# whcorkran/mamba-TTS-project

Measured on AMD Instinct MI355X. Metric: audio tokens/sec (teacher-forced fwd+bwd) per GPU; decode_step p50 latency, higher is better.
Workload: dtype bf16; 1 GPU; C2: MambaTTSDecoder 12L d_model=1024 fwd+bwd+clip+Adam, B=8/GPU T_audio=2048 T_text=128; model=MambaTTSDecoder-12L-d1024, global_batch=8, seq_len=2048, parallelism=dp1

## Files before the change

### include/mtts.h

```cpp
#ifndef MTTS_H
#define MTTS_H

#include <stdint.h>

#ifdef __cplusplus
extern "C" {
#endif

#define MTTS_ABI_VERSION 15

enum { MTTS_F32 = 0, MTTS_BF16 = 1 };
enum {
  MTTS_OK = 0,
  MTTS_EINVAL = -22,
  MTTS_EUNSUPPORTED = -95,
  MTTS_ELAUNCH = -5
};

int mtts_abi_version(void);
const char* mtts_last_error(void);

enum {
  MTTS_OVR_AUTO = -1,
  MTTS_OVR_SCAN_PATH = 0,
// ... 14 lines not shown

typedef struct {
  int batch, dim, seqlen, dstate;
  int dtype_io, dtype_bc;
  int delta_softplus;
  int ckpt_chunk;
  int a_is_log;
  int reserved_;
  int64_t u_bs, u_ls;
  int64_t delta_bs, delta_ls;
  int64_t z_bs, z_ls;
  int64_t out_bs, out_ls;
  int64_t B_bs, B_ls;
  int64_t C_bs, C_ls;
  const void* u;
  const void* delta;
  const float* A;
  const void* Bm;
  const void* Cm;
  const float* D;
  const void* z;
  const float* delta_bias;
  const float* h0;
  void* out;
  float* last_state;
  float* ckpt;
  void* workspace;
  const int* seqlens;
} MttsScanFwdArgs;

int64_t mtts_selective_scan_fwd_workspace(int batch, int dim, int seqlen, int dstate);
int mtts_selective_scan_fwd(const MttsScanFwdArgs* a, void* stream);

typedef struct {
  MttsScanFwdArgs f;
  const void* dout;
  int64_t dout_bs, dout_ls;
  void* du;      int64_t du_bs, du_ls;
  void* ddelta;  int64_t ddelta_bs, ddelta_ls;
  void* dz;      int64_t dz_bs, dz_ls;
  float* dB;     int64_t dB_bs, dB_ls;
  float* dC;     int64_t dC_bs, dC_ls;
  float* dA;
  float* dD;
  float* ddelta_bias;
  float* dh0;
  void* workspace;
} MttsScanBwdArgs;

int64_t mtts_selective_scan_bwd_workspace(int batch, int dim, int seqlen, int dstate);
int mtts_selective_scan_bwd(const MttsScanBwdArgs* a, void* stream);

typedef struct {
  int batch, dim, seqlen, width;
  int dtype;
  int silu;
  int64_t x_bs, x_ls, out_bs, out_ls;
  const void* x;
  const float* w;
  const float* bias;
  const float* conv_state_in;
  void* out;
  float* conv_state_out;
  const int* seqlens;
} MttsConvFwdArgs;

int mtts_causal_conv1d_fwd(const MttsConvFwdArgs* a, void* stream);

typedef struct {
  MttsConvFwdArgs f;
  const void* dout; int64_t dout_bs, dout_ls;
  void* dx;         int64_t dx_bs, dx_ls;
  float* dw;
  float* dbias;
  void* workspace;
} MttsConvBwdArgs;

int64_t mtts_causal_conv1d_bwd_workspace(int batch, int dim, int seqlen, int width);
int mtts_causal_conv1d_bwd(const MttsConvBwdArgs* a, void* stream);

typedef struct {
  int batch, dim, width, dtype, silu;
  int64_t x_bs, out_bs;
  const void* x;
  float* conv_state;
  const float* w;
  const float* bias;
  void* out;
} MttsConvUpdateArgs;

int mtts_causal_conv1d_update(const MttsConvUpdateArgs* a, void* stream);

typedef struct {
  int batch, dim, dstate, dtype_io, dtype_bc, dt_softplus;
  int64_t x_bs, dt_bs, z_bs, out_bs, B_bs, C_bs;
  float* state;
  const void* x;
  const void* dt;
  const float* A;
  const void* Bm;
  const void* Cm;
  const float* D;
  const void* z;
  const float* dt_bias;
  void* out;
  int dt_rank;
  const void* dt_w;
  void* out_packed;
} MttsStateUpdateArgs;

int mtts_selective_state_update(const MttsStateUpdateArgs* a, void* stream);


typedef struct {
  int rows, cols, dtype, rows_per_group;
  float eps;
  int64_t x_rs, res_rs, xsum_rs, y_rs, gb_rs;
  const void* x;
  const void* res;
  void* x_sum;
  const float* w;
  const float* b;
  const void* gamma;
  const void* beta;
  int gb_dtype;
  void* y;
  float* mean;
  float* rstd;
} MttsLNArgs;

int mtts_layernorm_fwd(const MttsLNArgs* a, void* stream);

int mtts_layernorm_rows_packed(const MttsLNArgs* a, void* y_packed, void* stream);

typedef struct {
  MttsLNArgs f;
  const void* dy;   int64_t dy_rs;
  const void* dx_acc; int64_t dxacc_rs;
  void* dx;         int64_t dx_rs;
  float* dw;
  float* db;
  float* dgamma;
  float* dbeta;
  void* workspace;
  float* dx_colsum;
  int64_t dgb_rs;
} MttsLNBwdArgs;

int64_t mtts_layernorm_bwd_workspace(int rows, int cols, int rows_per_group);
int mtts_layernorm_bwd(const MttsLNBwdArgs* a, void* stream);

int64_t mtts_colsum_workspace(int rows, int cols, int rows_per_group);
int mtts_colsum(const void* in, int dtype, int rows, int cols, int64_t row_stride, int rows_per_group, float* out,
                int64_t out_gstride, void* workspace, void* stream);

typedef struct {
  int batch, heads, head_dim, q_len, kv_len;
  int dtype;
  float scale;
  int64_t q_bs, q_ls, k_bs, k_ls, v_bs, v_ls, o_bs, o_ls;
  int64_t mask_bs;
  const void* q;
  const void* k;
  const void* v;
  const uint8_t* key_padding_mask;
  void* out;
  float* lse;
  void* out_packed;
  int64_t kv_hs;
} MttsAttnFwdArgs;

int mtts_attention_fwd(const MttsAttnFwdArgs* a, void* stream);

typedef struct {
  MttsAttnFwdArgs f;
  const void* x;
  int64_t x_rs;
  const void* wq;
  const void* bq;
  const float* ln_w;
  const float* ln_b;
  float eps;
  int d_model;
} MttsAttnQProjArgs;
int mtts_attention_decode_qproj(const MttsAttnQProjArgs* a, void* stream);

typedef struct {
  MttsAttnFwdArgs f;
  const void* dout; int64_t do_bs, do_ls;
  void* dq;         int64_t dq_bs, dq_ls;
  void* dk;         int64_t dk_bs, dk_ls;
  void* dv;         int64_t dv_bs, dv_ls;
  void* workspace;
} MttsAttnBwdArgs;

int64_t mtts_attention_bwd_workspace(int batch, int heads, int head_dim, int q_len, int kv_len, int dtype);
int mtts_attention_bwd(const MttsAttnBwdArgs* a, void* stream);

int mtts_length_regulate_lengths(const float* durations, int64_t dur_bs, int batch, int T, int64_t* lengths,
                                 void* stream);
int mtts_length_regulate_fwd(const void* hidden, int dtype, int batch, int T, int D, int64_t h_bs, int64_t h_ls,
                             const float* durations, int64_t dur_bs, int max_len, void* out, int64_t o_bs,
                             int64_t o_ls, void* stream);
int mtts_length_regulate_bwd(const void* dout, int dtype, int batch, int T, int D, int64_t do_bs, int64_t do_ls,
                             const float* durations, int64_t dur_bs, int max_len, void* dhidden, int64_t dh_bs,
                             int64_t dh_ls, void* stream);

// ... 58 lines not shown
  int kgroups;
  float* splitk_slab;
  int* splitk_count;
  int w_packed;
  int x_packed;
  void* y_packed;
  void* u_packed;
} MttsRowsArgs;

int mtts_gemm_rows(const MttsRowsArgs* a, void* stream);

typedef struct {
  int64_t rows;
  int vocab;
  int dtype;
  int64_t ld;
  const void* logits;
  const int64_t* targets;
  int ignore_index;
  float* loss;
  float* lse;
  float* workspace;
} MttsCrossEntropyArgs;

int64_t mtts_cross_entropy_workspace(int64_t rows);
int mtts_cross_entropy_fwd(const MttsCrossEntropyArgs* a, void* stream);
int mtts_cross_entropy_bwd(const MttsCrossEntropyArgs* a, const float* grad_loss, void* dlogits, int64_t ld_dlogits,
                           void* stream);

int64_t mtts_pack_rows_bytes(int N, int K);
int mtts_pack_rows_weight(const void* W, int64_t ldw, int N, int K, void* out, void* stream);


#define MTTS_GEMM_NT 0
#define MTTS_GEMM_TN 1
#define MTTS_GEMM_EPI_BIAS 1
#define MTTS_GEMM_EPI_GELU 2
#define MTTS_GEMM_EPI_DGELU 4
typedef struct {
  int m, n, k;
  int layout;
  int splits;
  int epilogue;
  int out_dtype;
  int bias_dtype;
  int64_t lda, ldb, ldc, ld_aux;
  const void* a;
  const void* b;
  void* c;
  const void* bias;
  void* aux;
  void* workspace;
  float beta;
} MttsGemmArgs;

int64_t mtts_gemm_workspace(const MttsGemmArgs* a);
int mtts_gemm(const MttsGemmArgs* a, void* stream);

int mtts_gemm_grouped(const MttsGemmArgs* probs, int n, void* stream);

int mtts_gemm_grouped_rounds(const MttsGemmArgs* probs, int n, void* stream);

#define MTTS_CONVGEMM_NN 2
#define MTTS_CONVGEMM_BIAS 1
#define MTTS_CONVGEMM_RELU 2
#define MTTS_CONVGEMM_DRELU 4
typedef struct {
  const void* ptr;
  int64_t seg_rows, seg_stride, row_stride;
  int32_t halo_c, halo_p;
} MttsRowMap;
typedef struct {
  int layout;
  int m, n, k;
  MttsRowMap a, b, c, aux;
  const float* bias;
  int epilogue;
  float beta;
  int splits;
  void* workspace;
  float* colsum_a;
} MttsConvGemmArgs;
int64_t mtts_convgemm_workspace(const MttsConvGemmArgs* a);
int mtts_convgemm(const MttsConvGemmArgs* a, void* stream);

#define MTTS_SKINNY_N 0
#define MTTS_SKINNY_SMALL_K 1
#define MTTS_SKINNY_TN 2
typedef struct {
  int mode;
  int m, n, k;
  int c_dtype;
  float beta;
  int64_t lda, ldb, ldc;
  const void* a;
  const void* b;
  void* c;
  void* workspace;
  int trans_c;
  int reserved_;
} MttsSkinnyArgs;

int64_t mtts_gemm_skinny_workspace(const MttsSkinnyArgs* a);
int mtts_gemm_skinny(const MttsSkinnyArgs* a, void* stream);

typedef struct {
// ... 52 lines not shown
```

### mamba-tts-project_amd/mtts/_lib.py

```python
from __future__ import annotations

import contextlib
import ctypes as C
import os

import torch

_HERE = os.path.dirname(os.path.abspath(__file__))
LIB_PATH = os.environ.get("MTTS_LIB", os.path.join(_HERE, "libmtts.so"))
ABI_VERSION = 15

F32, BF16 = 0, 1
i32, i64, f32, vp = C.c_int, C.c_int64, C.c_float, C.c_void_p


class ScanFwdArgs(C.Structure):
    _fields_ = [("batch", i32), ("dim", i32), ("seqlen", i32), ("dstate", i32),
                ("dtype_io", i32), ("dtype_bc", i32), ("delta_softplus", i32), ("ckpt_chunk", i32),
                ("a_is_log", i32), ("reserved_", i32), ("u_bs", i64), ("u_ls", i64), ("delta_bs", i64), ("delta_ls", i64),
                ("z_bs", i64), ("z_ls", i64), ("out_bs", i64), ("out_ls", i64),
                ("B_bs", i64), ("B_ls", i64), ("C_bs", i64), ("C_ls", i64),
                ("u", vp), ("delta", vp), ("A", vp), ("Bm", vp), ("Cm", vp), ("D", vp), ("z", vp),
                ("delta_bias", vp), ("h0", vp), ("out", vp), ("last_state", vp), ("ckpt", vp),
                ("workspace", vp), ("seqlens", vp)]


class ScanBwdArgs(C.Structure):
    _fields_ = [("f", ScanFwdArgs), ("dout", vp), ("dout_bs", i64), ("dout_ls", i64),
                ("du", vp), ("du_bs", i64), ("du_ls", i64),
                ("ddelta", vp), ("ddelta_bs", i64), ("ddelta_ls", i64),
                ("dz", vp), ("dz_bs", i64), ("dz_ls", i64),
                ("dB", vp), ("dB_bs", i64), ("dB_ls", i64),
                ("dC", vp), ("dC_bs", i64), ("dC_ls", i64),
                ("dA", vp), ("dD", vp), ("ddelta_bias", vp), ("dh0", vp), ("workspace", vp)]


class ConvFwdArgs(C.Structure):
    _fields_ = [("batch", i32), ("dim", i32), ("seqlen", i32), ("width", i32), ("dtype", i32), ("silu", i32),
                ("x_bs", i64), ("x_ls", i64), ("out_bs", i64), ("out_ls", i64),
                ("x", vp), ("w", vp), ("bias", vp), ("conv_state_in", vp), ("out", vp), ("conv_state_out", vp),
                ("seqlens", vp)]


class ConvBwdArgs(C.Structure):
    _fields_ = [("f", ConvFwdArgs), ("dout", vp), ("dout_bs", i64), ("dout_ls", i64),
                ("dx", vp), ("dx_bs", i64), ("dx_ls", i64), ("dw", vp), ("dbias", vp), ("workspace", vp)]


class ConvUpdateArgs(C.Structure):
    _fields_ = [("batch", i32), ("dim", i32), ("width", i32), ("dtype", i32), ("silu", i32),
                ("x_bs", i64), ("out_bs", i64), ("x", vp), ("conv_state", vp), ("w", vp), ("bias", vp),
                ("out", vp)]


class StateUpdateArgs(C.Structure):
    _fields_ = [("batch", i32), ("dim", i32), ("dstate", i32), ("dtype_io", i32), ("dtype_bc", i32),
                ("dt_softplus", i32),
                ("x_bs", i64), ("dt_bs", i64), ("z_bs", i64), ("out_bs", i64), ("B_bs", i64), ("C_bs", i64),
                ("state", vp), ("x", vp), ("dt", vp), ("A", vp), ("Bm", vp), ("Cm", vp), ("D", vp), ("z", vp),
                ("dt_bias", vp), ("out", vp), ("dt_rank", i32), ("dt_w", vp), ("out_packed", vp)]


class RowsArgs(C.Structure):
    _fields_ = [("M", i32), ("N", i32), ("K", i32), ("act", i32), ("ldx", i64), ("ldw", i64), ("ldy", i64),
                ("x", vp), ("W", vp), ("bias", vp), ("y", vp),
                ("conv_dim", i32), ("conv_state", vp), ("conv_w", vp), ("conv_b", vp), ("u", vp), ("ldu", i64),
                ("ln_w", vp), ("ln_b", vp), ("ln_eps", f32), ("gamma", vp), ("beta", vp), ("ld_gb", i64),
                ("res", vp), ("ld_res", i64), ("kgroups", i32), ("splitk_slab", vp), ("splitk_count", vp),
                ("w_packed", i32), ("x_packed", i32), ("y_packed", vp), ("u_packed", vp)]


class CrossEntropyArgs(C.Structure):
    _fields_ = [("rows", i64), ("vocab", i32), ("dtype", i32), ("ld", i64), ("logits", vp), ("targets", vp),
                ("ignore_index", i32), ("loss", vp), ("lse", vp), ("workspace", vp)]


class GemmArgs(C.Structure):
    _fields_ = [("m", i32), ("n", i32), ("k", i32), ("layout", i32), ("splits", i32), ("epilogue", i32),
                ("out_dtype", i32), ("bias_dtype", i32), ("lda", i64), ("ldb", i64), ("ldc", i64), ("ld_aux", i64),
                ("a", vp), ("b", vp), ("c", vp), ("bias", vp), ("aux", vp), ("workspace", vp), ("beta", f32)]


class DropoutArgs(C.Structure):
    _fields_ = [("n", i64), ("dtype", i32), ("p", f32), ("seed", C.c_uint64), ("x", vp), ("y", vp), ("pre", vp),
                ("group", i32), ("x_rep", i32), ("x_inner", i32), ("reserved_", i32), ("seed_in", vp),
                ("seed_out", vp)]


class SampleArgs(C.Structure):
    _fields_ = [("rows", i32), ("vocab", i32), ("dtype", i32), ("top_k", i32), ("ld", i64), ("logits", vp),
                ("bias", vp), ("bias_ld", i64), ("temperature", f32), ("top_p", f32), ("seed", vp), ("step", vp),
                ("advance", i32), ("step0", i32), ("pos", vp), ("tokens", vp), ("tok_stride", i64),
                ("history", vp), ("hist_ld", i64), ("hist_cols", i32), ("eos_id", i32), ("pad_id", i32),
                ("pos_rows", i32), ("finished", vp), ("length", vp), ("unfinished", vp)]


class RowMap(C.Structure):
    _fields_ = [("ptr", vp), ("seg_rows", i64), ("seg_stride", i64), ("row_stride", i64), ("halo_c", i32),
                ("halo_p", i32)]


class ConvGemmArgs(C.Structure):
    _fields_ = [("layout", i32), ("m", i32), ("n", i32), ("k", i32), ("a", RowMap), ("b", RowMap), ("c", RowMap),
                ("aux", RowMap), ("bias", vp), ("epilogue", i32), ("beta", f32), ("splits", i32),
                ("workspace", vp), ("colsum_a", vp)]


class SkinnyArgs(C.Structure):
    _fields_ = [("mode", i32), ("m", i32), ("n", i32), ("k", i32), ("c_dtype", i32), ("beta", f32),
                ("lda", i64), ("ldb", i64), ("ldc", i64), ("a", vp), ("b", vp), ("c", vp), ("workspace", vp),
                ("trans_c", i32), ("reserved_", i32)]


class LNArgs(C.Structure):
    _fields_ = [("rows", i32), ("cols", i32), ("dtype", i32), ("rows_per_group", i32), ("eps", f32),
                ("x_rs", i64), ("res_rs", i64), ("xsum_rs", i64), ("y_rs", i64), ("gb_rs", i64),
                ("x", vp), ("res", vp), ("x_sum", vp), ("w", vp), ("b", vp), ("gamma", vp), ("beta", vp),
                ("gb_dtype", i32), ("y", vp), ("mean", vp), ("rstd", vp)]


class LNBwdArgs(C.Structure):
    _fields_ = [("f", LNArgs), ("dy", vp), ("dy_rs", i64), ("dx_acc", vp), ("dxacc_rs", i64),
                ("dx", vp), ("dx_rs", i64), ("dw", vp), ("db", vp), ("dgamma", vp), ("dbeta", vp),
                ("workspace", vp), ("dx_colsum", vp), ("dgb_rs", i64)]


class AttnFwdArgs(C.Structure):
    _fields_ = [("batch", i32), ("heads", i32), ("head_dim", i32), ("q_len", i32), ("kv_len", i32),
                ("dtype", i32), ("scale", f32),
                ("q_bs", i64), ("q_ls", i64), ("k_bs", i64), ("k_ls", i64), ("v_bs", i64), ("v_ls", i64),
                ("o_bs", i64), ("o_ls", i64), ("mask_bs", i64),
                ("q", vp), ("k", vp), ("v", vp), ("key_padding_mask", vp), ("out", vp), ("lse", vp),
                ("out_packed", vp), ("kv_hs", i64)]


class AttnQProjArgs(C.Structure):
    _fields_ = [("f", AttnFwdArgs), ("x", vp), ("x_rs", i64), ("wq", vp), ("bq", vp), ("ln_w", vp), ("ln_b", vp),
                ("eps", f32), ("d_model", i32)]


class AttnBwdArgs(C.Structure):
    _fields_ = [("f", AttnFwdArgs), ("dout", vp), ("do_bs", i64), ("do_ls", i64),
                ("dq", vp), ("dq_bs", i64), ("dq_ls", i64), ("dk", vp), ("dk_bs", i64), ("dk_ls", i64),
                ("dv", vp), ("dv_bs", i64), ("dv_ls", i64), ("workspace", vp)]


class CastDesc(C.Structure):
    _fields_ = [("src", vp), ("dst", vp), ("dstT", vp), ("rows", i32), ("cols", i32), ("tile0", i64)]


class AdamTensor(C.Structure):
    _fields_ = [("p", vp), ("g", vp), ("m", vp), ("v", vp), ("n", i64), ("chunk0", i64)]


_SIGS = {
    "mtts_abi_version": ([], i32),
    "mtts_last_error": ([], C.c_char_p),
    "mtts_set_override": ([i32, i32], i32),
    "mtts_get_override": ([i32], i32),
    "mtts_selective_scan_fwd_workspace": ([i32, i32, i32, i32], i64),
    "mtts_selective_scan_fwd": ([C.POINTER(ScanFwdArgs), vp], i32),
    "mtts_selective_scan_bwd_workspace": ([i32, i32, i32, i32], i64),
    "mtts_selective_scan_bwd": ([C.POINTER(ScanBwdArgs), vp], i32),
    "mtts_causal_conv1d_fwd": ([C.POINTER(ConvFwdArgs), vp], i32),
    "mtts_causal_conv1d_bwd_workspace": ([i32, i32, i32, i32], i64),
    "mtts_causal_conv1d_bwd": ([C.POINTER(ConvBwdArgs), vp], i32),
    "mtts_causal_conv1d_update": ([C.POINTER(ConvUpdateArgs), vp], i32),
    "mtts_selective_state_update": ([C.POINTER(StateUpdateArgs), vp], i32),
    "mtts_layernorm_fwd": ([C.POINTER(LNArgs), vp], i32),
    "mtts_gemm_rows": ([C.POINTER(RowsArgs), vp], i32),
    "mtts_pack_rows_bytes": ([i32, i32], i64),
    "mtts_cross_entropy_workspace": ([i64], i64),
    "mtts_cross_entropy_fwd": ([C.POINTER(CrossEntropyArgs), vp], i32),
    "mtts_cross_entropy_bwd": ([C.POINTER(CrossEntropyArgs), vp, vp, i64, vp], i32),
    "mtts_layernorm_rows_packed": ([C.POINTER(LNArgs), vp, vp], i32),
    "mtts_pack_rows_weight": ([vp, i64, i32, i32, vp, vp], i32),
    "mtts_gemm_workspace": ([C.POINTER(GemmArgs)], i64),
    "mtts_gemm": ([C.POINTER(GemmArgs), vp], i32),
    "mtts_gemm_grouped": ([C.POINTER(GemmArgs), i32, vp], i32),
    "mtts_gemm_grouped_rounds": ([C.POINTER(GemmArgs), i32, vp], i32),
    "mtts_convgemm": ([C.POINTER(ConvGemmArgs), vp], i32),
    "mtts_convgemm_workspace": ([C.POINTER(ConvGemmArgs)], i64),
    "mtts_gemm_skinny": ([C.POINTER(SkinnyArgs), vp], i32),
    "mtts_gemm_skinny_workspace": ([C.POINTER(SkinnyArgs)], i64),
    "mtts_layernorm_bwd_workspace": ([i32, i32, i32], i64),
    "mtts_layernorm_bwd": ([C.POINTER(LNBwdArgs), vp], i32),
    "mtts_colsum_workspace": ([i32, i32, i32], i64),
    "mtts_colsum": ([vp, i32, i32, i32, i64, i32, vp, i64, vp, vp], i32),
    "mtts_attention_fwd": ([C.POINTER(AttnFwdArgs), vp], i32),
    "mtts_attention_decode_qproj": ([C.POINTER(AttnQProjArgs), vp], i32),
    "mtts_attention_bwd_workspace": ([i32, i32, i32, i32, i32, i32], i64),
    "mtts_attention_bwd": ([C.POINTER(AttnBwdArgs), vp], i32),
    "mtts_adam_chunks": ([i64], i64),
    "mtts_adam_workspace": ([i64], i64),
    "mtts_clip_adam": ([vp, i32, i64, vp, f32, f32, f32, f32, f32, f32, vp, vp, vp], i32),
    "mtts_embed_sum": ([vp, i64, vp, vp, vp, vp, vp, i32, i32, i32, i32, vp, i32, i64, vp, vp], i32),
    "mtts_embed_sum_at": ([vp, i64, vp, vp, vp, vp, vp, i32, i32, i32, i32, vp, i32, i64, vp, i64, i32, vp], i32),
    "mtts_embed_table_grad_workspace": ([i64, i32, i32], i64),
    "mtts_embed_table_grad": ([vp, i64, vp, i32, i64, i32, i32, vp, vp, vp], i32),
    "mtts_cast_tiles": ([i32, i32], i64),
    "mtts_cast_bf16_multi": ([vp, i32, i64, vp], i32),
    "mtts_length_regulate_lengths": ([vp, i64, i32, i32, vp, vp], i32),
    "mtts_length_regulate_fwd": ([vp, i32, i32, i32, i32, i64, i64, vp, i64, i32, vp, i64, i64, vp], i32),
    "mtts_length_regulate_bwd": ([vp, i32, i32, i32, i32, i64, i64, vp, i64, i32, vp, i64, i64, vp], i32),
    "mtts_dropout": ([C.POINTER(DropoutArgs), vp], i32),
    "mtts_sample_tokens": ([C.POINTER(SampleArgs), vp], i32),
}

_lib = None


def lib():
    global _lib
    if _lib is None:
        if not os.path.exists(LIB_PATH):
            raise RuntimeError(f"libmtts.so not found at {LIB_PATH}; run __graft_entry__.build() "
                               "(make -C mamba-tts-project_amd/mtts/csrc)")
        L = C.CDLL(LIB_PATH)
        for sym, what in (("mtts_embed_sum_at", "ragged prompts"),
                          ("mtts_gemm_grouped_rounds", "round-filling weight gradients")):
            if not hasattr(L, sym):
                raise RuntimeError(f"{LIB_PATH} is stale: it was built before {sym} ({what}) was "
                                   "added; rebuild it with __graft_entry__.build() "
                                   "(make -C mamba-tts-project_amd/mtts/csrc)")
        for name, (argt, rest) in _SIGS.items():
            fn = getattr(L, name)
            fn.argtypes = argt
            fn.restype = rest
        v = L.mtts_abi_version()
        if v != ABI_VERSION:
            raise RuntimeError(f"libmtts ABI {v} != expected {ABI_VERSION}")
        _lib = L
    return _lib


def exported_symbols():
    return list(_SIGS)


def call(name, args):
    L = lib()
    stream = torch.cuda.current_stream().cuda_stream
    rc = getattr(L, name)(C.byref(args), C.c_void_p(stream))
    if rc != 0:
        raise RuntimeError(f"{name} failed ({rc}): {L.mtts_last_error().decode()}")


def call_raw(name, *args):
    L = lib()
    rc = getattr(L, name)(*args, C.c_void_p(torch.cuda.current_stream().cuda_stream))
    if rc != 0:
        raise RuntimeError(f"{name} failed ({rc}): {L.mtts_last_error().decode()}")


OVERRIDES = {"scan_path": 0, "scan_p": 1, "scan_segs": 2, "scan_bwd_segs": 3, "gemm_narrow": 4,
             "attn_chunks": 5, "attn_bwd": 6, "attn_generic": 7, "conv_untiled": 8, "gemm_tile": 9,
             "attn_dq_dma": 10}
SCAN_C1, SCAN_W2, SCAN_NARROW = 1, 2, 3
ATTN_BWD_FUSED, ATTN_BWD_SPLIT = 1, 2


@contextlib.contextmanager
def override(**paths):
    L = lib()
    old = {}
    try:
        for k, v in paths.items():
            old[k] = L.mtts_set_override(OVERRIDES[k], -1 if v is None else int(v))
        yield
    finally:
        for k, v in old.items():
            L.mtts_set_override(OVERRIDES[k], v)

# ... 12 lines not shown
```

### mamba-tts-project_amd/mtts/attention.py

```python
from __future__ import annotations

import math

import torch
import torch.nn as nn
import torch.nn.functional as F

from . import attn_kernels
from . import wgrad as WG
from .linear import _want_t, cast_scope, cast_weight, cast_weight_t, colsum, linear, proj, wgrad


class InProjFn(torch.autograd.Function):

    @staticmethod
    def forward(ctx, query, key, weight, bias):
        cd = query.dtype
        d = query.shape[-1]
        Wc, bc = cast_weight(weight, cd), cast_weight(bias, cd)
        x2, k2 = query.reshape(-1, d), key.reshape(-1, d)
        q = proj(x2, Wc[:d], bc[:d])
        kv = proj(k2, Wc[d:], bc[d:])
        ctx.save_for_backward(x2, k2, Wc)
        ctx.weight = weight
        ctx.meta = (query.shape, key.shape, weight.dtype, bias.dtype)
        return q.view(*query.shape[:-1], d), kv.view(*key.shape[:-1], 2 * d)

    @staticmethod
    def backward(ctx, dq, dkv):
        x2, k2, Wc = ctx.saved_tensors
        qshape, kshape, wdt, bdt = ctx.meta
        d = x2.shape[1]
        dq2 = dq.reshape(-1, d).to(Wc.dtype)
        dkv2 = dkv.reshape(-1, 2 * d).to(Wc.dtype)
        if Wc.dtype == torch.bfloat16 and _want_t(ctx.weight):
            Wt = cast_weight_t(ctx.weight, Wc.dtype)
            dquery = proj(dq2, Wt[:, :d]).view(qshape) if ctx.needs_input_grad[0] else None
            dkey = proj(dkv2, Wt[:, d:]).view(kshape) if ctx.needs_input_grad[1] else None
        else:
            dquery = (dq2 @ Wc[:d]).view(qshape) if ctx.needs_input_grad[0] else None
            dkey = (dkv2 @ Wc[d:]).view(kshape) if ctx.needs_input_grad[1] else None
        dW = db = None
        if ctx.needs_input_grad[2] and not WG.submit([(dq2, x2, ctx.weight, (0, d)),
                                                      (dkv2, k2, ctx.weight, (d, 3 * d))]):
            dW = torch.empty(3 * d, d, device=x2.device, dtype=torch.float32)
            wgrad(dq2, x2, out=dW[:d])
            wgrad(dkv2, k2, out=dW[d:])
            dW = dW.to(wdt)
        if ctx.needs_input_grad[3]:
            db = torch.empty(3 * d, device=x2.device, dtype=torch.float32)
            colsum(dq2, out=db[:d])
            colsum(dkv2, out=db[d:])
            db = db.to(bdt)
        return dquery, dkey, dW, db


class DkvSink:

    def __init__(self, rows, n_layers, width, shape, device, dtype):
        self.rows, self.L, self.width, self.shape = rows, n_layers, width, shape
        self.device, self.dtype = device, dtype
        self.buf = None
        self.key2 = None
        self.written = [False] * n_layers
        self.taken = [False] * n_layers

    def view(self, layer):
        if self.buf is None:
            self.buf = torch.empty(self.rows, self.L * self.width, device=self.device, dtype=self.dtype)
        self.written[layer] = True
        return self.buf[:, layer * self.width:(layer + 1) * self.width].view(*self.shape, self.width)

    def partner(self, layer):
        sink = self

        class _P:
            @staticmethod
            def take():
                if not sink.written[layer] or sink.buf is None or sink.key2 is None:
                    return None
                sink.taken[layer] = True
                d = sink.width // 2
                return (sink.buf[:, layer * sink.width:(layer + 1) * sink.width], sink.key2, (d, 3 * d))
        return _P()


class KVAllFn(torch.autograd.Function):

    @staticmethod
    def forward(ctx, key, sink, *params):
        cd = key.dtype
        d = key.shape[-1]
        Ws, bs = params[0::2], params[1::2]
        k2 = key.reshape(-1, d)
        Wst = torch.cat([cast_weight(W, cd)[d:] for W in Ws])
        bst = torch.cat([cast_weight(b, cd)[d:] for b in bs])
        kv = proj(k2, Wst, bst)
        ctx.save_for_backward(k2)
        ctx.Ws, ctx.bs, ctx.kshape, ctx.sink = Ws, bs, key.shape, sink
        sink.key2 = k2
        return tuple(kv[:, l * 2 * d:(l + 1) * 2 * d].view(*key.shape[:-1], 2 * d) for l in range(len(Ws)))

    @staticmethod
    def backward(ctx, *dkvs):
        (k2,) = ctx.saved_tensors
        Ws, bs, sink = ctx.Ws, ctx.bs, ctx.sink
        nl, d = len(Ws), k2.shape[1]
        w2 = 2 * d
        cd = k2.dtype
        in_sink = sink.buf is not None and all(
            g is not None and g.data_ptr() == sink.buf.data_ptr() + l * w2 * sink.buf.element_size()
            and g.stride()[-2] == nl * w2 for l, g in enumerate(dkvs))
        if in_sink:
            dkv = sink.buf
        else:
            dkv = torch.zeros(k2.shape[0], nl * w2, device=k2.device, dtype=cd)
            for l, g in enumerate(dkvs):
                if g is not None:
                    dkv[:, l * w2:(l + 1) * w2] = g.reshape(-1, w2)
        sink.buf = None
        dkey = None
        if ctx.needs_input_grad[0]:
            if cd == torch.bfloat16:
                WstT = torch.cat([cast_weight_t(W, cd)[:, d:] for W in Ws], dim=1)
                dkey = proj(dkv, WstT).view(ctx.kshape)
            else:
                dkey = (dkv @ torch.cat([cast_weight(W, cd)[d:] for W in Ws])).view(ctx.kshape)
        grads = [dkey, None]
        for l in range(nl):
            W, b = Ws[l], bs[l]
            dW = db = None
            if not sink.taken[l]:
                dy = dkv[:, l * w2:(l + 1) * w2]
                if ctx.needs_input_grad[2 + 2 * l] and not WG.submit([(dy, k2, W, (d, 3 * d))]):
                    dW = torch.zeros(W.shape, device=W.device, dtype=W.dtype)
                    dW[d:] = wgrad(dy.contiguous(), k2).to(W.dtype)
                if ctx.needs_input_grad[3 + 2 * l]:
                    db = torch.zeros(b.shape, device=b.device, dtype=b.dtype)
                    db[d:] = colsum(dy).to(b.dtype)
            grads += [dW, db]
        sink.written = [False] * nl
        sink.taken = [False] * nl
        return tuple(grads)


def kv_all(key: torch.Tensor, attns) -> list:
    params = []
    for a in attns:
        params += [a.in_proj_weight, a.in_proj_bias]
    d = attns[0].embed_dim
    sink = DkvSink(key.numel() // d, len(attns), 2 * d, tuple(key.shape[:-1]), key.device, key.dtype)
    outs = list(KVAllFn.apply(key, sink, *params))
    for l, o in enumerate(outs):
        o._mtts_dkv_sink = (sink, l)
    return outs


def kv_all_ok(key: torch.Tensor, attns) -> bool:
    a0 = attns[0]
    d = a0.embed_dim
    return (len(attns) >= 2 and key.dim() == 3 and key.shape[-1] == d and key.shape[1] > 1 and key.is_cuda
            and all(a.embed_dim == d and a.in_proj_bias is not None and a.in_proj_weight.dtype == torch.float32
                    and a.in_proj_bias.dtype == torch.float32 and a.in_proj_weight.is_contiguous()
                    and a.dropout == 0.0 for a in attns))


class _KeyTie(torch.autograd.Function):

    @staticmethod
    def forward(ctx, o, key):
        ctx.kmeta = (key.shape, key.dtype, key.device)
        return o.view_as(o)

    @staticmethod
    def backward(ctx, do):
        shape, dt, dev = ctx.kmeta
        return do, torch.zeros(shape, dtype=dt, device=dev)


class CrossAttention(nn.Module):
    def __init__(self, embed_dim, num_heads, dropout=0.0, batch_first=True, bias=True, device=None, dtype=None):
        super().__init__()
        if not batch_first:
            raise ValueError("only batch_first=True is supported (reference usage)")
        fk = {"device": device, "dtype": dtype}
        self.embed_dim = embed_dim
        self.num_heads = num_heads
        self.head_dim = embed_dim // num_heads
        self.dropout = dropout
        self.batch_first = True
# ... 47 lines not shown
```

### mamba-tts-project_amd/mtts/csrc/common.h

```cpp
#pragma once
#include <hip/hip_runtime.h>
#include <stdint.h>
#include <stdio.h>
#include <stdarg.h>

#include "mtts.h"

namespace mtts {

void set_error(const char* fmt, ...);
int override_of(int key);

void colsum(const float* part, int nparts, int ppg, int64_t pstride, int ncols, float* out, int64_t out_gstride,
            hipStream_t st);
struct ColsumJob {
  const float* part;
  float* out;
  int nparts, ppg;
  int64_t out_gstride;
};
void colsum_multi(const ColsumJob* jobs, int n, int ncols, int64_t pstride, hipStream_t st);

#define MTTS_CHECK(cond, ...)                                                 \
  do {                                                                        \
    if (!(cond)) {                                                            \
      ::mtts::set_error(__VA_ARGS__);                                         \
      return MTTS_EINVAL;                                                     \
    }                                                                         \
  } while (0)

#define MTTS_LAUNCH_CHECK(name)                                               \
  do {                                                                        \
    hipError_t e_ = hipGetLastError();                                        \
    if (e_ != hipSuccess) {                                                   \
      ::mtts::set_error("%s: launch failed: %s", name, hipGetErrorString(e_)); \
      return MTTS_ELAUNCH;                                                    \
    }                                                                         \
  } while (0)

int launch_gemv_packed(const MttsRowsArgs* a, hipStream_t st);

__host__ __device__ __forceinline__ int64_t xpk_index(int m, int k) {
  return ((int64_t)((k >> 5) * 2 + (m >> 4)) * 64 + ((k >> 3) & 3) * 16 + (m & 15)) * 8 + (k & 7);
}

typedef uint16_t bf16_t;

__device__ __forceinline__ float bf2f(bf16_t v) { return __uint_as_float(((uint32_t)v) << 16); }
__device__ __forceinline__ bf16_t f2bf(float f) {
  __bf16 h = (__bf16)f;
  return *reinterpret_cast<bf16_t*>(&h);
}

template <typename T> struct IO;
template <> struct IO<float> {
  static __device__ __forceinline__ float ld(const float* p) { return *p; }
  static __device__ __forceinline__ void st(float* p, float v) { *p = v; }
};
template <> struct IO<bf16_t> {
  static __device__ __forceinline__ float ld(const bf16_t* p) { return bf2f(*p); }
  static __device__ __forceinline__ void st(bf16_t* p, float v) { *p = f2bf(v); }
};
template <typename T> __device__ __forceinline__ float ldf(const T* p) { return IO<T>::ld(p); }
template <typename T> __device__ __forceinline__ void stf(T* p, float v) { IO<T>::st(p, v); }

constexpr float kLog2e = 1.4426950408889634f;
constexpr float kLn2 = 0.6931471805599453f;

__device__ __forceinline__ float fast_exp(float x) { return __builtin_amdgcn_exp2f(x * kLog2e); }
__device__ __forceinline__ float fast_rcp(float x) { return __builtin_amdgcn_rcpf(x); }

__device__ __forceinline__ float softplus_f(float x) {
  float e = __builtin_amdgcn_exp2f(fminf(x, 20.f) * kLog2e);
  float lg = __builtin_amdgcn_logf(1.f + e) * kLn2;
// ... 106 lines not shown
```

### mamba-tts-project_amd/mtts/csrc/conv.hip

```cpp
#include "common.h"

#include <type_traits>

namespace mtts {

constexpr int kK = 4;
constexpr int kTT = 32;

template <typename T, int CPT>
__device__ __forceinline__ void ldv(const T* p, float (&o)[CPT]) {
  if constexpr (sizeof(T) * CPT == 16) {
    uint4 v = *reinterpret_cast<const uint4*>(p);
    if constexpr (sizeof(T) == 4) {
      o[0] = __uint_as_float(v.x); o[1] = __uint_as_float(v.y); o[2] = __uint_as_float(v.z); o[3] = __uint_as_float(v.w);
    } else {
      const uint32_t w[4] = {v.x, v.y, v.z, v.w};
#pragma unroll
      for (int q = 0; q < 4; ++q) { o[2 * q] = __uint_as_float(w[q] << 16); o[2 * q + 1] = __uint_as_float(w[q] & 0xffff0000u); }
    }
  } else {
#pragma unroll
    for (int q = 0; q < CPT; ++q) o[q] = ldf(p + q);
  }
}
// ... 425 lines not shown
}

}

using namespace mtts;

extern "C" int mtts_causal_conv1d_fwd(const MttsConvFwdArgs* a, void* stream) {
  int rc = check_conv(a);
  if (rc) return rc;
  hipStream_t st = (hipStream_t)stream;
  if (a->seqlen > 0) {
    if (a->dtype == MTTS_F32) {
      if (vec_ok<float>(a, 4) && (uintptr_t)a->w % 16 == 0) launch_fwd<float, 4>(a, st);
      else launch_fwd<float, 1>(a, st);
    } else {
      if (vec_ok<bf16_t>(a, 8) && (uintptr_t)a->w % 16 == 0) launch_fwd<bf16_t, 8>(a, st);
      else launch_fwd<bf16_t, 1>(a, st);
    }
    MTTS_LAUNCH_CHECK("causal_conv1d_fwd");
  }
  if (a->conv_state_out) {
    const int64_t n = (int64_t)a->batch * a->dim * kK;
    if (a->dtype == MTTS_F32) hipLaunchKernelGGL(conv_state_kernel<float>, dim3((n + 255) / 256), dim3(256), 0, st, *a);
    else hipLaunchKernelGGL(conv_state_kernel<bf16_t>, dim3((n + 255) / 256), dim3(256), 0, st, *a);
    MTTS_LAUNCH_CHECK("causal_conv1d_state");
  }
  return MTTS_OK;
}

extern "C" int64_t mtts_causal_conv1d_bwd_workspace(int batch, int dim, int seqlen, int width) {
  (void)width;
  const int64_t ntile = (seqlen + kTT - 1) / kTT;
  return ((int64_t)batch * ntile + 1) * dim * (kK + 1) * 4 + 256;
}

template <typename T, int CPT>
static int launch_bwd(const MttsConvBwdArgs* a, hipStream_t st, float* part, bool tiled) {
  if constexpr (sizeof(T) * CPT >= 8) {
   if (tiled) {
    dim3 grid((a->f.dim / CPT + 63) / 64, (a->f.seqlen + 8 * kBwdTT - 1) / (8 * kBwdTT), a->f.batch);
    hipLaunchKernelGGL((conv_bwd_tile_kernel<T, CPT, kBwdTT>), grid, dim3(512), 0, st, *a, part);
    return (int)(grid.y * grid.z);
   }
  }
  dim3 grid((a->f.dim / CPT + 255) / 256, (a->f.seqlen + kTT - 1) / kTT, a->f.batch);
  hipLaunchKernelGGL((conv_bwd_kernel<T, CPT>), grid, dim3(256), 0, st, *a, part);
  return (int)(grid.y * grid.z);
}

extern "C" int mtts_causal_conv1d_bwd(const MttsConvBwdArgs* a, void* stream) {
  MTTS_CHECK(a, "conv1d_bwd: null args");
  int rc = check_conv(&a->f);
  if (rc) return rc;
  MTTS_CHECK(a->dout && a->dx && a->dw && a->workspace, "conv1d_bwd: null tensor");
  MTTS_CHECK(!a->f.seqlens, "conv1d_bwd: seqlens is inference only");
  const MttsConvFwdArgs& f = a->f;
  if (f.seqlen == 0) return MTTS_OK;
  hipStream_t st = (hipStream_t)stream;
  float* part = (float*)a->workspace;
  const int es = f.dtype == MTTS_F32 ? 4 : 2;
  const int cpt = f.dtype == MTTS_F32 ? 4 : 8;
  const bool vec = f.dim % cpt == 0 && (uintptr_t)f.x % 16 == 0 && (uintptr_t)a->dout % 16 == 0 &&
                   (uintptr_t)a->dx % 16 == 0 && (f.x_ls * es) % 16 == 0 && (f.x_bs * es) % 16 == 0 &&
                   (a->dout_ls * es) % 16 == 0 && (a->dout_bs * es) % 16 == 0 && (a->dx_ls * es) % 16 == 0 &&
                   (a->dx_bs * es) % 16 == 0;
  auto fits = [&](int64_t ls) { return (int64_t)(f.seqlen + 16) * ls * es < (1ll << 31); };
  const bool tiled = vec && (uintptr_t)f.w % 16 == 0 && !tiled_off() && fits(f.x_ls) && fits(a->dout_ls);
  int nparts;
  if (f.dtype == MTTS_F32) {
    if (vec) nparts = launch_bwd<float, 4>(a, st, part, tiled);
    else nparts = launch_bwd<float, 1>(a, st, part, false);
  } else {
    if (tiled) nparts = launch_bwd<bf16_t, 4>(a, st, part, true);
    else if (vec) nparts = launch_bwd<bf16_t, 8>(a, st, part, false);
    else nparts = launch_bwd<bf16_t, 1>(a, st, part, false);
  }
  MTTS_LAUNCH_CHECK("causal_conv1d_bwd");
  float* sums = part + (int64_t)nparts * f.dim * (kK + 1);
  colsum(part, nparts, nparts, (int64_t)f.dim * (kK + 1), f.dim * (kK + 1), sums, 0, st);
  hipLaunchKernelGGL(conv_bwd_split, dim3((f.dim * (kK + 1) + 255) / 256), dim3(256), 0, st, sums, f.dim, a->dw,
                     a->dbias);
  MTTS_LAUNCH_CHECK("causal_conv1d_bwd_reduce");
  return MTTS_OK;
}
```

### mamba-tts-project_amd/mtts/csrc/gemm.hip

```cpp
#include "common.h"

#include <algorithm>
#include <cstddef>
#include <type_traits>

namespace mtts {
namespace {

typedef short s16x8 __attribute__((ext_vector_type(8)));
typedef short s16x4 __attribute__((ext_vector_type(4)));
typedef __bf16 bf16x8 __attribute__((ext_vector_type(8)));
typedef float f32x4 __attribute__((ext_vector_type(4)));
typedef __attribute__((address_space(3))) s16x4 lds_s16x4;
typedef __attribute__((address_space(3))) s16x8 lds_s16x8;

constexpr int kThreads = 512;
constexpr int kTile = 256;
constexpr int kBK = 64;
constexpr int kRegion = 16384;
constexpr int kBuf = 4 * kRegion;
constexpr int kLds = 2 * kBuf;

enum { R_A0 = 0, R_A1 = 1, R_B0 = 2, R_B1 = 3 };

struct GemmParams {
  const bf16_t* a;
  const bf16_t* b;
  void* c;
  const void* bias;
  void* aux;
  int64_t lda, ldb, ldc, ld_aux;
  int64_t split_stride;
  int m, n, k;
  int tiles_m, tiles_n, splits;
  int group;
  int epi;
  int bias_bf16;
  int wide_out;
  float beta;
};

__device__ __forceinline__ int a_map(int rr, int s) { return (rr >> 6) * 128 + s * 64 + (rr & 63); }
__device__ __forceinline__ int b_map(int rr, int s) { return (rr >> 5) * 64 + s * 32 + (rr & 31); }
template <bool IS_A>
__device__ __forceinline__ int rmap(int rr, int s) { return IS_A ? a_map(rr, s) : b_map(rr, s); }

__device__ __forceinline__ void glds16(const void* base, uint32_t voff, uint32_t lds_base) {
#if defined(__HIP_DEVICE_COMPILE__)
  asm volatile("s_mov_b32 m0, %2\n\ts_nop 0\n\tglobal_load_lds_dwordx4 %0, %1" ::"v"(voff), "s"(base), "s"(lds_base)
               : "memory", "m0");
#endif
}
template <int N>
__device__ __forceinline__ void wait_vm() {
#if defined(__HIP_DEVICE_COMPILE__)
  static_assert(N >= 0 && N < 64, "vmcnt range");
  __builtin_amdgcn_s_waitcnt((N & 15) | (7 << 4) | (15 << 8) | ((N >> 4) << 14));
#endif
}
__device__ __forceinline__ void barrier() {
#if defined(__HIP_DEVICE_COMPILE__)
  __builtin_amdgcn_s_waitcnt(0xC07F);
#ifndef MTTS_GEMM_DIAG_NOBAR
  __builtin_amdgcn_s_barrier();
#endif
  asm volatile("" ::: "memory");
#endif
}

__device__ __forceinline__ f32x4 mfma(s16x8 a, s16x8 b, f32x4 c) {
  return __builtin_amdgcn_mfma_f32_16x16x32_bf16(__builtin_bit_cast(bf16x8, a), __builtin_bit_cast(bf16x8, b), c, 0,
                                                 0, 0);
}

__device__ __forceinline__ float gelu_tail_s(float a) {
  float s = -1.7774024116e-08f;
  s = fmaf(s, a, 5.6194854933e-07f);
  s = fmaf(s, a, -7.6223902631e-06f);
  s = fmaf(s, a, 5.5893204013e-05f);
  s = fmaf(s, a, -2.0454518331e-04f);
  s = fmaf(s, a, -1.6655060660e-04f);
  s = fmaf(s, a, 7.1668288485e-03f);
  s = fmaf(s, a, -5.2604280745e-02f);
  s = fmaf(s, a, 2.6218665810e-01f);
  s = fmaf(s, a, -1.1511125488e+00f);
  s = fmaf(s, a, -9.9999981719e-01f);
  return s;
}
__device__ __forceinline__ float gelu_f(float x) {
  const float a = fminf(fabsf(x), 5.5f);
  const float h = __builtin_amdgcn_exp2f(fmaf(x * (-0.5f * kLog2e), x, gelu_tail_s(a)));
  return x * (x >= 0.f ? 1.f - h : h);
// ... 397 lines not shown
  static_assert(N >= 0 && N < 64, "vmcnt range");
  wait_vm<N>();
}
template <int BASE>
__device__ __forceinline__ void wait_ops_rt(int n) {
  if (n == BASE) { wait_ops<BASE>(); return; }
  switch (n) {
#define W_(k) case k: wait_ops<k>(); break;
    W_(0) W_(1) W_(2) W_(3) W_(4) W_(5) W_(6) W_(7) W_(8) W_(9) W_(10) W_(11) W_(12) W_(13) W_(14) W_(15)
    W_(16) W_(17) W_(18) W_(19) W_(20) W_(21) W_(22) W_(23) W_(24) W_(25) W_(26) W_(27) W_(28) W_(29) W_(30)
    W_(31) W_(32) W_(33) W_(34) W_(35) W_(36) W_(37) W_(38) W_(39) W_(40) W_(41) W_(42) W_(43) W_(44) W_(45)
    W_(46) W_(47) W_(48) W_(49) W_(50) W_(51) W_(52) W_(53) W_(54) W_(55) W_(56) W_(57) W_(58) W_(59) W_(60)
    W_(61) W_(62)
#undef W_
    default: wait_ops<0>(); break;
  }
}
__device__ __forceinline__ void sbar() {
#if defined(__HIP_DEVICE_COMPILE__)
  __builtin_amdgcn_s_barrier();
  asm volatile("" ::: "memory");
#endif
}

typedef int i32x4 __attribute__((ext_vector_type(4)));
typedef int i32x2 __attribute__((ext_vector_type(2)));
constexpr uint32_t kOOB = 0xFFFFFFF0u;

__device__ __forceinline__ __amdgpu_buffer_rsrc_t brsrc(const void* p, uint32_t bytes) {
  return __builtin_amdgcn_make_buffer_rsrc(const_cast<void*>(p), 0, (int)bytes, 0x00020000);
}

template <int EPI>
__device__ __forceinline__ void load_bias(const GemmParams& p, int n0, int wc, int lane, f32x4 (&bias)[4]) {
  if constexpr ((EPI & MTTS_GEMM_EPI_BIAS) != 0) {
    const int cl = 4 * (lane >> 4);
    const int es = p.bias_bf16 ? 2 : 4;
    const __amdgpu_buffer_rsrc_t r = brsrc(p.bias, (uint32_t)p.n * es);
#pragma unroll
    for (int NB = 0; NB < 4; ++NB) {
      const int col = n0 + wc * 64 + NB * 16 + cl;
      const uint32_t off = col < p.n ? (uint32_t)col * es : kOOB;
      if (p.bias_bf16) {
        const i32x2 raw = __builtin_amdgcn_raw_buffer_load_b64(r, off, 0, 0);
        bias[NB] = f32x4{__uint_as_float((uint32_t)raw.x << 16), __uint_as_float((uint32_t)raw.x & 0xffff0000u),
                         __uint_as_float((uint32_t)raw.y << 16), __uint_as_float((uint32_t)raw.y & 0xffff0000u)};
      } else {
        bias[NB] = __builtin_bit_cast(f32x4, __builtin_amdgcn_raw_buffer_load_b128(r, off, 0, 0));
      }
    }
  }
}

template <int EPI, bool OUT_F32>
__device__ __forceinline__ void store_tile_buf(const GemmParams& p, f32x4 (&acc)[8][4], const f32x4 (&bias)[4],
                                               int m0, int n0, int wr, int wc, int lane, int split) {
  const int rl = lane & 15, cl = 4 * (lane >> 4);
  if constexpr (OUT_F32) {
    const __amdgpu_buffer_rsrc_t r = brsrc((const float*)p.c + (int64_t)split * p.split_stride,
                                           (uint32_t)((int64_t)p.m * p.ldc * 4));
    const bool acc_old = p.beta != 0.f;
#pragma unroll
    for (int MB = 0; MB < 8; ++MB) {
      const int row = m0 + wr * 128 + MB * 16 + rl;
      f32x4 old[4];
      if (acc_old) {
#pragma unroll
        for (int NB = 0; NB < 4; ++NB) {
          const int col = n0 + wc * 64 + NB * 16 + cl;
          const uint32_t off = (row < p.m && col < p.n) ? (uint32_t)((row * p.ldc + col) * 4) : kOOB;
          old[NB] = __builtin_bit_cast(f32x4, __builtin_amdgcn_raw_buffer_load_b128(r, off, 0, 0));
        }
      }
#pragma unroll
      for (int NB = 0; NB < 4; ++NB) {
        const int col = n0 + wc * 64 + NB * 16 + cl;
        const uint32_t off = (row < p.m && col < p.n) ? (uint32_t)((row * p.ldc + col) * 4) : kOOB;
        f32x4 v = acc[MB][NB];
        if (acc_old) v += p.beta * old[NB];
        __builtin_amdgcn_raw_buffer_store_b128(__builtin_bit_cast(i32x4, v), r, off, 0, 0);
      }
    }
  } else {
    const int g = lane >> 4;
    const int cw0 = n0 + wc * 64 + (g & 1) * 16 + 8 * (g >> 1);
    const __amdgpu_buffer_rsrc_t rc = brsrc(p.c, (uint32_t)((int64_t)p.m * p.ldc * 2));
    const __amdgpu_buffer_rsrc_t ra = brsrc(p.aux, (uint32_t)((int64_t)p.m * p.ld_aux * 2));
#pragma unroll
    for (int MB = 0; MB < 8; ++MB) {
      const int row = m0 + wr * 128 + MB * 16 + rl;
      const bool rok = row < p.m;
      uint32_t o2[4][2], h2[4][2];
      i32x2 auxv[4];
      if constexpr ((EPI & MTTS_GEMM_EPI_DGELU) != 0) {
#pragma unroll
        for (int NB = 0; NB < 4; ++NB) {
          const int col = n0 + wc * 64 + NB * 16 + cl;
          const uint32_t off = (rok && col < p.n) ? (uint32_t)((row * p.ld_aux + col) * 2) : kOOB;
          auxv[NB] = __builtin_amdgcn_raw_buffer_load_b64(ra, off, 0, 0);
        }
      }
#pragma unroll
      for (int NB = 0; NB < 4; ++NB) {
        f32x4 v = acc[MB][NB];
        if constexpr ((EPI & MTTS_GEMM_EPI_BIAS) != 0) v += bias[NB];
        bf16_t o[4];
        if constexpr ((EPI & MTTS_GEMM_EPI_GELU) != 0) {
          bf16_t hpre[4];
#pragma unroll
          for (int j = 0; j < 4; ++j) hpre[j] = f2bf(v[j]);
#pragma unroll
          for (int j = 0; j < 4; j += 2) {
            const f32x2 g = gelu_f2(f32x2{bf2f(hpre[j]), bf2f(hpre[j + 1])});
            o[j] = f2bf(g[0]);
            o[j + 1] = f2bf(g[1]);
          }
          h2[NB][0] = hpre[0] | ((uint32_t)hpre[1] << 16);
          h2[NB][1] = hpre[2] | ((uint32_t)hpre[3] << 16);
        } else if constexpr ((EPI & MTTS_GEMM_EPI_DGELU) != 0) {
          const uint32_t x = (uint32_t)auxv[NB].x, y = (uint32_t)auxv[NB].y;
          const float h[4] = {__uint_as_float(x << 16), __uint_as_float(x & 0xffff0000u), __uint_as_float(y << 16),
                              __uint_as_float(y & 0xffff0000u)};
#pragma unroll
          for (int j = 0; j < 4; j += 2) {
            const f32x2 gg = gelu_grad_f2(f32x2{h[j], h[j + 1]});
            o[j] = f2bf(bf2f(f2bf(v[j])) * gg[0]);
            o[j + 1] = f2bf(bf2f(f2bf(v[j + 1])) * gg[1]);
          }
        } else {
#pragma unroll
          for (int j = 0; j < 4; ++j) o[j] = f2bf(v[j]);
        }
        o2[NB][0] = o[0] | ((uint32_t)o[1] << 16);
        o2[NB][1] = o[2] | ((uint32_t)o[3] << 16);
      }
#pragma unroll
      for (int pr = 0; pr < 2; ++pr) {
        uint32_t w[4];
#pragma unroll
        for (int d = 0; d < 2; ++d) {
          const auto r = __builtin_amdgcn_permlane16_swap(o2[2 * pr][d], o2[2 * pr + 1][d], false, false);
          w[d] = r[0];
          w[2 + d] = r[1];
        }
        const int cw = cw0 + pr * 32;
        const bool ok = rok && cw < p.n;
        __builtin_amdgcn_raw_buffer_store_b128(i32x4{(int)w[0], (int)w[1], (int)w[2], (int)w[3]}, rc,
                                               ok ? (uint32_t)((row * p.ldc + cw) * 2) : kOOB, 0, 0);
        if constexpr ((EPI & MTTS_GEMM_EPI_GELU) != 0) {
#pragma unroll
          for (int d = 0; d < 2; ++d) {
            const auto r = __builtin_amdgcn_permlane16_swap(h2[2 * pr][d], h2[2 * pr + 1][d], false, false);
            w[d] = r[0];
            w[2 + d] = r[1];
          }
          __builtin_amdgcn_raw_buffer_store_b128(i32x4{(int)w[0], (int)w[1], (int)w[2], (int)w[3]}, ra,
                                                 ok ? (uint32_t)((row * p.ld_aux + cw) * 2) : kOOB, 0, 0);
        }
      }
    }
  }
}

struct WorkItem {
  int m0, n0, split;
};
__device__ __forceinline__ WorkItem work_item(const GemmParams& p, int id) {
  const int tiles = p.tiles_m * p.tiles_n;
  const int split = id / tiles;
  const int tile = id % tiles;
  const int gsz = p.group * p.tiles_n;
  const int g0 = (tile / gsz) * p.group;
  const int gr = min(p.group, p.tiles_m - g0);
  const int tm = g0 + (tile % gsz) % gr, tn = (tile % gsz) / gr;
  return WorkItem{tm * kTile, tn * kTile, split};
}

template <bool KMAJ, bool IS_A>
struct PLoader {
  uint32_t fixed[2];
  int rm[2][2];
  __device__ void init(int tid, int64_t ld) {
#pragma unroll
    for (int i = 0; i < 2; ++i) {
      if constexpr (KMAJ) {
        const int rr = i * 64 + (tid >> 3), pp = tid & 7;
        fixed[i] = (uint32_t)(((pp ^ ((rr >> 1) & 7)) * 8) * 2);
#pragma unroll
        for (int s = 0; s < 2; ++s) rm[s][i] = rmap<IS_A>(rr, s);
      } else {
        const int kr = i * 32 + (tid >> 4), pp = tid & 15;
        const int f = (kr & 3) | (((kr >> 3) & 1) << 2);
        const int c = pp ^ (f << 1);
        fixed[i] = (uint32_t)(kr * ld * 2);
#pragma unroll
        for (int s = 0; s < 2; ++s) rm[s][i] = rmap<IS_A>(c * 8, s);
      }
    }
  }
  __device__ __forceinline__ uint32_t off(int row0, int nrows, int64_t ld, int s, int i) const {
    if constexpr (KMAJ) {
      int row = row0 + rm[s][i];
      row = row < nrows ? row : nrows - 1;
      return (uint32_t)(row * ld * 2) + fixed[i];
    } else {
      int col = row0 + rm[s][i];
      col = col + 8 <= nrows ? col : ((nrows - 8) & ~7);
      return fixed[i] + (uint32_t)col * 2;
    }
  }
};

__device__ __forceinline__ int xcd_work_id() {
  const int nwg = gridDim.x;
  const int bid = blockIdx.x;
  const int q8 = nwg / 8, r8 = nwg % 8, xcd = bid % 8;
  return (xcd < r8 ? xcd * (q8 + 1) : r8 * (q8 + 1) + (xcd - r8) * q8) + bid / 8;
}

template <bool AK, bool BKM, int EPI, bool OUT_F32>
__device__ __forceinline__ void gemm_pp_body(const GemmParams& p, const int wid) {
  __shared__ __attribute__((aligned(16))) char lds[kLds];
  const int tid = threadIdx.x, lane = tid & 63, wave = __builtin_amdgcn_readfirstlane(tid >> 6);
  const int wr = wave >> 2, wc = wave & 3;
  const int nk = p.k / kBK;
  const int G = nk;

  PLoader<AK, true> la;
  PLoader<BKM, false> lb;
  la.init(tid, p.lda);
  lb.init(tid, p.ldb);
  const int64_t astep = AK ? kBK * 2 : kBK * p.lda * 2;
  const int64_t bstep = BKM ? kBK * 2 : kBK * p.ldb * 2;
  const uint32_t lds0 = (uint32_t)(uintptr_t)(__attribute__((address_space(3))) char*)lds;

  struct Src {
    const char* a;
    const char* b;
    uint32_t o[8];
  };
  auto source = [&](const WorkItem& it, Src& sr) {
    const int64_t k0 = (int64_t)it.split * p.k;
    sr.a = (const char*)(AK ? p.a + k0 : p.a + k0 * p.lda);
    sr.b = (const char*)(BKM ? p.b + k0 : p.b + k0 * p.ldb);
#pragma unroll
    for (int s = 0; s < 2; ++s)
#pragma unroll
      for (int i = 0; i < 2; ++i) {
        sr.o[s * 2 + i] = la.off(it.m0, p.m, p.lda, s, i);
        sr.o[4 + s * 2 + i] = lb.off(it.n0, p.n, p.ldb, s, i);
      }
  };
  const WorkItem cur = work_item(p, wid);
  Src scur;
  source(cur, scur);
  auto stage = [&](int kt, int r) {
    const uint32_t reg = lds0 + (kt & 1) * kBuf + r * kRegion;
    const int oi = (r == R_A0 ? 0 : r == R_A1 ? 2 : r == R_B0 ? 4 : 6);
    const bool isa = r == R_A0 || r == R_A1;
    const char* base = isa ? scur.a + kt * astep : scur.b + kt * bstep;
    glds16(base, scur.o[oi], reg + wave * 1024);
    glds16(base, scur.o[oi + 1], reg + 8192 + wave * 1024);
  };

  f32x4 bias[4] = {};
  load_bias<EPI>(p, cur.n0, wc, lane, bias);

  f32x4 acc[8][4];
#pragma unroll
  for (int i = 0; i < 8; ++i)
#pragma unroll
    for (int j = 0; j < 4; ++j) acc[i][j] = f32x4{0.f, 0.f, 0.f, 0.f};

// ... 7 lines not shown
  s16x8 af[2][4], b0f[2][2], b1f[2][2];
#define PP_MFMA(BF, MO, NO)                                                                   \
  __builtin_amdgcn_sched_barrier(0);                                                        \
  __builtin_amdgcn_s_waitcnt(0xC07F);                                                        \
  __builtin_amdgcn_sched_barrier(0);                                                        \
  __builtin_amdgcn_s_setprio(1);                                                            \
  _Pragma("unroll") for (int ks_ = 0; ks_ < 2; ++ks_)                                        \
  _Pragma("unroll") for (int mb_ = 0; mb_ < 4; ++mb_)                                        \
  _Pragma("unroll") for (int nb_ = 0; nb_ < 2; ++nb_)                                        \
      acc[(MO) + mb_][(NO) + nb_] = mfma(BF[ks_][nb_], af[ks_][mb_], acc[(MO) + mb_][(NO) + nb_]); \
  __builtin_amdgcn_s_setprio(0);                                                            \
  __builtin_amdgcn_sched_barrier(0);                                                        \
  sbar();
  for (int g = 0; g < G; ++g) {
    const bool steady = g > 0 && g + 2 < G;
    const bool n1 = g + 1 < G, n2 = g + 2 < G;
    const char* bufp = lbase + (g & 1) * kBuf;
#pragma unroll
    for (int ks = 0; ks < 2; ++ks) {
#pragma unroll
      for (int nb = 0; nb < 2; ++nb) b0f[ks][nb] = frag<BKM>(bufp + R_B0 * kRegion, wc * 32 + nb * 16, ks, lane);
#pragma unroll
      for (int mb = 0; mb < 4; ++mb) af[ks][mb] = frag<AK>(bufp + R_A0 * kRegion, wr * 64 + mb * 16, ks, lane);
    }
    if (n1) stage(g + 1, R_A1);
    if (steady) wait_ops<6>();
    else wait_ops_rt<6>(g == 0 ? (n1 ? 8 : 2) : (n1 ? 6 : 0));
    sbar();
    PP_MFMA(b0f, 0, 0)
#pragma unroll
    for (int ks = 0; ks < 2; ++ks)
#pragma unroll
      for (int nb = 0; nb < 2; ++nb) b1f[ks][nb] = frag<BKM>(bufp + R_B1 * kRegion, wc * 32 + nb * 16, ks, lane);
    if (n1) stage(g + 1, R_B1);
    if (steady) wait_ops<10>();
    else wait_ops_rt<10>(g == 0 ? (n1 ? 8 : 0) : (n1 ? 10 : 2));
    sbar();
    PP_MFMA(b1f, 0, 2)
#pragma unroll
    for (int ks = 0; ks < 2; ++ks)
#pragma unroll
      for (int mb = 0; mb < 4; ++mb) af[ks][mb] = frag<AK>(bufp + R_A1 * kRegion, wr * 64 + mb * 16, ks, lane);
    if (n2) stage(g + 2, R_A0);
    sbar();
    PP_MFMA(b1f, 4, 2)
    if (n2) stage(g + 2, R_B0);
    if (steady) wait_ops<8>();
    else if (n1) wait_ops_rt<8>((n2 ? 8 : 4));
    sbar();
    PP_MFMA(b0f, 4, 0)
  }
#undef PP_MFMA
  if (wr == 0) sbar();
  store_tile_buf<EPI, OUT_F32>(p, acc, bias, cur.m0, cur.n0, wr, wc, lane, cur.split);
}

template <bool AK, bool BKM, int EPI, bool OUT_F32>
__global__ __launch_bounds__(kThreads, 1) void gemm_pp_kernel(GemmParams p) {
  gemm_pp_body<AK, BKM, EPI, OUT_F32>(p, xcd_work_id());
}

constexpr int kGroupMax = 24;
struct GroupParams {
  GemmParams p[kGroupMax];
  int tile_end[kGroupMax];
  int n;
};

template <bool AK, bool BKM, int EPI, bool OUT_F32>
__global__ __launch_bounds__(kThreads, 1) void gemm_pp_grouped_kernel(const GroupParams G) {
  const int wid = xcd_work_id();
  int i = 0, t0 = 0;
#pragma unroll
  for (int j = 0; j + 1 < kGroupMax; ++j)
    if (j + 1 < G.n && wid >= G.tile_end[j]) { i = j + 1; t0 = G.tile_end[j]; }
  GemmParams q = G.p[0];
#pragma unroll
  for (int j = 1; j < kGroupMax; ++j)
    if (i == j) q = G.p[j];
  gemm_pp_body<AK, BKM, EPI, OUT_F32>(q, wid - t0);
}

constexpr int kRoundsMax = 64;
struct RoundProb {
  const bf16_t* a;
  const bf16_t* b;
  void* c;
  int lda, ldb, ldc;
  int m, n, k;
  float beta;
  int pad_;
};
struct RoundParams {
  RoundProb p[kRoundsMax];
  int tile_end[kRoundsMax];
  int n;
  int round;
};
static_assert(sizeof(RoundProb) == 56 && offsetof(RoundParams, p) == 0 && sizeof(RoundParams) <= 4096,
              "round-filling problem table must fit the kernel arguments");
static_assert(offsetof(RoundProb, lda) == 24 && offsetof(RoundProb, ldc) == 32 && offsetof(RoundProb, n) == 40 &&
              offsetof(RoundProb, beta) == 48, "gemm_pp_rounds_kernel reads RoundProb as qwords");

__device__ __forceinline__ int round_work_id(int round) {
  const int bid = blockIdx.x;
  const int b = bid % round, r0 = bid - b;
  const int nwg = min(round, (int)gridDim.x - r0);
  const int q8 = nwg / 8, r8 = nwg % 8, xcd = b % 8;
  return r0 + (xcd < r8 ? xcd * (q8 + 1) : r8 * (q8 + 1) + (xcd - r8) * q8) + b / 8;
}

__global__ __launch_bounds__(kThreads, 1) void gemm_pp_rounds_kernel(const RoundParams G) {
// ... 100 lines not shown
    __builtin_amdgcn_sched_barrier(0);
  };
  for (int g = 0; g < nk; g += 2) {
    step(g, std::integral_constant<int, 0>{});
    step(g + 1, std::integral_constant<int, 1>{});
  }
  wait_ops<0>();
#pragma unroll
  for (int h = 0; h < 2; ++h)
#pragma unroll
    for (int i = 0; i < 8; ++i)
#pragma unroll
      for (int j = 0; j < 4; ++j) asm volatile("" : "+a"(acc[h][i][j]));
#pragma unroll
  for (int h = 0; h < 2; ++h) {
    f32x4 bias[4] = {};
    load_bias<EPI>(p, it.n0, 2 * wc + h, lane, bias);
    store_tile_buf<EPI, false>(p, acc[h], bias, it.m0, it.n0, wr, 2 * wc + h, lane, 0);
  }
}

__global__ __launch_bounds__(256) void split_reduce_kernel(const float* __restrict__ slabs, int64_t sstride, int splits,
                                                           int rows, int cols, int64_t lds_, float* out, int64_t ldo,
                                                           float beta) {
  const int c4 = cols / 4;
  const int64_t total = (int64_t)rows * c4;
  for (int64_t i = (int64_t)blockIdx.x * blockDim.x + threadIdx.x; i < total; i += (int64_t)gridDim.x * blockDim.x) {
    const int r = (int)(i / c4), c = (int)(i % c4) * 4;
    f32x4 s = *(const f32x4*)(slabs + (int64_t)r * lds_ + c);
    for (int k = 1; k < splits; ++k) s += *(const f32x4*)(slabs + k * sstride + (int64_t)r * lds_ + c);
    float* op = out + (int64_t)r * ldo + c;
    if (beta != 0.f) s += beta * *(const f32x4*)op;
    *(f32x4*)op = s;
  }
}

template <bool AK, bool BKM, int EPI, bool F32>
void launch(const GemmParams& p, int nwg, hipStream_t st) {
  const int64_t cbytes = F32 ? (int64_t)p.m * p.ldc * 4 : (int64_t)p.m * p.ldc * 2;
  const int64_t abytes = (EPI & (MTTS_GEMM_EPI_GELU | MTTS_GEMM_EPI_DGELU)) ? (int64_t)p.m * p.ld_aux * 2 : 0;
  const bool pp_ok = (F32 || p.wide_out) && cbytes < (1ll << 31) && abytes < (1ll << 31) &&
                     (!F32 || p.beta == 0.f || p.splits == 1) && override_of(MTTS_OVR_GEMM_NARROW) != 1;
  if (!pp_ok) {
    hipLaunchKernelGGL((gemm_kernel<AK, BKM, EPI, F32>), dim3(nwg), dim3(kThreads), 0, st, p);
    return;
  }
  if constexpr (AK && BKM && !F32) {
    if (override_of(MTTS_OVR_GEMM_TILE) == 2) {
      hipLaunchKernelGGL((gemm_w4_kernel<EPI>), dim3(nwg), dim3(kW4Threads), 0, st, p);
      return;
    }
  }
  hipLaunchKernelGGL((gemm_pp_kernel<AK, BKM, EPI, F32>), dim3(nwg), dim3(kThreads), 0, st, p);
}

}
}

using namespace mtts;

extern "C" int64_t mtts_gemm_workspace(const MttsGemmArgs* a) {
  if (!a || a->layout != MTTS_GEMM_TN || a->splits <= 1) return 0;
  return (int64_t)a->splits * a->m * a->n * 4;
}

extern "C" int mtts_gemm(const MttsGemmArgs* a, void* stream) {
  MTTS_CHECK(a && a->a && a->b && a->c, "gemm: null pointer");
  const int M = a->m, N = a->n, K = a->k;
  MTTS_CHECK(M > 0 && N > 0 && K > 0, "gemm: m=%d n=%d k=%d must be positive", M, N, K);
  MTTS_CHECK(a->layout == MTTS_GEMM_NT || a->layout == MTTS_GEMM_TN, "gemm: layout must be NT (0) or TN (1)");
  const bool nt = a->layout == MTTS_GEMM_NT;
  const int splits = a->splits > 0 ? a->splits : 1;
  MTTS_CHECK(K % (kBK * splits) == 0, "gemm: k=%d must be a multiple of 64*splits (splits=%d)", K, splits);
  MTTS_CHECK(N % 8 == 0, "gemm: n=%d must be a multiple of 8", N);
  MTTS_CHECK(nt || M % 8 == 0, "gemm: TN needs m=%d a multiple of 8", M);
  MTTS_CHECK(((uintptr_t)a->a | (uintptr_t)a->b) % 16 == 0 && a->lda % 8 == 0 && a->ldb % 8 == 0,
             "gemm: A / B must be 16-byte aligned with row strides a multiple of 8 elements");
  MTTS_CHECK(a->ldc % 4 == 0 && (uintptr_t)a->c % 16 == 0, "gemm: C must be 16-byte aligned, ldc a multiple of 4");
  MTTS_CHECK(nt ? (a->lda >= K && a->ldb >= K) : (a->lda >= M && a->ldb >= N), "gemm: leading dimension too small");
  const int64_t aspan = nt ? (int64_t)(M - 1) * a->lda + K : (int64_t)(kBK - 1) * a->lda + M;
  const int64_t bspan = nt ? (int64_t)(N - 1) * a->ldb + K : (int64_t)(kBK - 1) * a->ldb + N;
  MTTS_CHECK(aspan * 2 < (1ll << 32) && bspan * 2 < (1ll << 32), "gemm: operand span exceeds 4 GiB");
  const int epi = a->epilogue;
  const bool f32out = a->out_dtype == 0;
  MTTS_CHECK(a->out_dtype == 0 || a->out_dtype == 1, "gemm: out_dtype must be 0 (f32) or 1 (bf16)");
  MTTS_CHECK(!f32out || epi == 0, "gemm: epilogues apply to bf16 output only");
  MTTS_CHECK(f32out || splits == 1, "gemm: split-K needs fp32 output");
  MTTS_CHECK(!(epi & MTTS_GEMM_EPI_BIAS) || a->bias, "gemm: bias epilogue without bias");
  MTTS_CHECK(!(epi & MTTS_GEMM_EPI_BIAS) || (uintptr_t)a->bias % (a->bias_dtype == 1 ? 8 : 16) == 0,
             "gemm: bias must be %d-byte aligned", a->bias_dtype == 1 ? 8 : 16);
  MTTS_CHECK(!(epi & (MTTS_GEMM_EPI_GELU | MTTS_GEMM_EPI_DGELU)) || (uintptr_t)a->aux % 8 == 0,
             "gemm: aux must be 8-byte aligned");
  MTTS_CHECK(!(epi & (MTTS_GEMM_EPI_GELU | MTTS_GEMM_EPI_DGELU)) || (a->aux && a->ld_aux % 4 == 0),
             "gemm: GELU epilogues need aux (ld_aux multiple of 4)");
  MTTS_CHECK((epi & (MTTS_GEMM_EPI_GELU | MTTS_GEMM_EPI_DGELU)) != (MTTS_GEMM_EPI_GELU | MTTS_GEMM_EPI_DGELU),
             "gemm: GELU and DGELU are exclusive");
  MTTS_CHECK(nt || (epi == 0 && f32out), "gemm: TN (weight gradient) runs fp32 out, no epilogue");
  MTTS_CHECK(splits == 1 || a->workspace, "gemm: split-K needs the workspace (mtts_gemm_workspace bytes)");

  GemmParams p{};
  p.a = (const bf16_t*)a->a; p.b = (const bf16_t*)a->b;
  p.bias = a->bias; p.aux = a->aux; p.bias_bf16 = a->bias_dtype == 1;
  p.lda = a->lda; p.ldb = a->ldb; p.ld_aux = a->ld_aux;
  p.m = M; p.n = N; p.k = K / splits;
  p.tiles_m = (M + kTile - 1) / kTile; p.tiles_n = (N + kTile - 1) / kTile;
  p.splits = splits; p.epi = epi;
  p.group = std::min(p.tiles_m, 4);
  if (splits > 1) {
    p.c = a->workspace; p.ldc = N; p.split_stride = (int64_t)M * N; p.beta = 0.f;
  } else {
    p.c = a->c; p.ldc = a->ldc; p.split_stride = 0; p.beta = a->beta;
  }
  p.wide_out = !f32out && a->ldc % 8 == 0 && (!(epi & (MTTS_GEMM_EPI_GELU | MTTS_GEMM_EPI_DGELU)) || a->ld_aux % 8 == 0) &&
               (!a->aux || (uintptr_t)a->aux % 16 == 0) && override_of(MTTS_OVR_GEMM_NARROW) != 1;
  const int nwg = p.tiles_m * p.tiles_n * splits;
  hipStream_t st = (hipStream_t)stream;
  if (!nt) {
    launch<false, false, 0, true>(p, nwg, st);
  } else if (f32out) {
    launch<true, true, 0, true>(p, nwg, st);
  } else {
    switch (epi) {
      case 0: launch<true, true, 0, false>(p, nwg, st); break;
      case MTTS_GEMM_EPI_BIAS: launch<true, true, MTTS_GEMM_EPI_BIAS, false>(p, nwg, st); break;
      case MTTS_GEMM_EPI_GELU: launch<true, true, MTTS_GEMM_EPI_GELU, false>(p, nwg, st); break;
      case MTTS_GEMM_EPI_BIAS | MTTS_GEMM_EPI_GELU:
        launch<true, true, MTTS_GEMM_EPI_BIAS | MTTS_GEMM_EPI_GELU, false>(p, nwg, st); break;
      case MTTS_GEMM_EPI_DGELU: launch<true, true, MTTS_GEMM_EPI_DGELU, false>(p, nwg, st); break;
      default: MTTS_CHECK(false, "gemm: unsupported epilogue combination %d", epi);
    }
  }
  MTTS_LAUNCH_CHECK("gemm");
  if (splits > 1) {
    const int64_t total = (int64_t)M * (N / 4);
    const int blocks = (int)std::min<int64_t>((total + 255) / 256, 2048);
    hipLaunchKernelGGL(split_reduce_kernel, dim3(blocks), dim3(256), 0, st, (const float*)a->workspace,
                       (int64_t)M * N, splits, M, N, (int64_t)N, (float*)a->c, a->ldc, a->beta);
    MTTS_LAUNCH_CHECK("gemm split reduce");
  }
  return MTTS_OK;
}

extern "C" int mtts_gemm_grouped(const MttsGemmArgs* probs, int n, void* stream) {
  using namespace mtts;
  MTTS_CHECK(probs && n >= 1 && n <= kGroupMax, "gemm_grouped: 1 <= n <= %d problems", kGroupMax);
  GroupParams G{};
  int tiles = 0;
  for (int i = 0; i < n; ++i) {
    const MttsGemmArgs* a = probs + i;
    MTTS_CHECK(a->a && a->b && a->c, "gemm_grouped[%d]: null pointer", i);
    const int M = a->m, N = a->n, K = a->k;
    MTTS_CHECK(a->layout == MTTS_GEMM_TN && a->out_dtype == 0 && a->epilogue == 0 && a->splits <= 1,
               "gemm_grouped[%d]: TN, fp32 out, no epilogue, no split-K only", i);
    MTTS_CHECK(M > 0 && N > 0 && K > 0 && K % kBK == 0, "gemm_grouped[%d]: m=%d n=%d k=%d (k %% 64 == 0)", i, M, N, K);
    MTTS_CHECK(N % 8 == 0 && M % 8 == 0, "gemm_grouped[%d]: m, n must be multiples of 8", i);
    MTTS_CHECK(((uintptr_t)a->a | (uintptr_t)a->b) % 16 == 0 && a->lda % 8 == 0 && a->ldb % 8 == 0 &&
               a->lda >= M && a->ldb >= N, "gemm_grouped[%d]: A / B alignment or leading dimension", i);
    MTTS_CHECK(a->ldc % 4 == 0 && (uintptr_t)a->c % 16 == 0 && a->ldc >= N, "gemm_grouped[%d]: C alignment / ldc", i);
    MTTS_CHECK(a->beta == 0.f || a->beta == 1.f, "gemm_grouped[%d]: beta must be 0 or 1", i);
    MTTS_CHECK((int64_t)(kBK - 1) * a->lda + M < (1ll << 31) && (int64_t)(kBK - 1) * a->ldb + N < (1ll << 31) &&
               (int64_t)M * a->ldc * 4 < (1ll << 31), "gemm_grouped[%d]: operand / C span exceeds the 32-bit offsets", i);
    GemmParams& p = G.p[i];
    p.a = (const bf16_t*)a->a; p.b = (const bf16_t*)a->b; p.c = a->c;
    p.lda = a->lda; p.ldb = a->ldb; p.ldc = a->ldc;
    p.m = M; p.n = N; p.k = K;
    p.tiles_m = (M + kTile - 1) / kTile; p.tiles_n = (N + kTile - 1) / kTile;
    p.splits = 1; p.split_stride = 0; p.beta = a->beta;
    p.group = std::min(p.tiles_m, 4);
    tiles += p.tiles_m * p.tiles_n;
// ... 53 lines not shown
```

### mamba-tts-project_amd/mtts/csrc/ln.hip

```cpp
#include "common.h"

namespace mtts {

constexpr int kLnWaves = 4;
constexpr int kMaxVec = 8;


template <typename T, typename TG, int VEC, int NV>
__global__ __launch_bounds__(64 * kLnWaves) void ln_fwd_kernel(const MttsLNArgs a) {
  const int lane = threadIdx.x & 63;
  const int row = blockIdx.x * kLnWaves + (threadIdx.x >> 6);
  if (row >= a.rows) return;
  const int n = a.cols;
  float v[NV][VEC];
  const T* x = (const T*)a.x + (int64_t)row * a.x_rs;
#pragma unroll
  for (int k = 0; k < NV; ++k) ld_vec<T, VEC>(x + (k * 64 + lane) * VEC, v[k]);
  if (a.res) {
    const T* r = (const T*)a.res + (int64_t)row * a.res_rs;
#pragma unroll
    for (int k = 0; k < NV; ++k) {
      float t[VEC];
      ld_vec<T, VEC>(r + (k * 64 + lane) * VEC, t);
#pragma unroll
// ... 249 lines not shown
  const bool gf = !a->gamma || a->gb_dtype == MTTS_F32;
  if (a->dtype == MTTS_F32) return gf ? go(F32{}, F32{}) : go(F32{}, BF{});
  return gf ? go(BF{}, F32{}) : go(BF{}, BF{});
}

template <typename T, typename TG, int VEC, int NV>
struct FwdRunner {
  static void run(const MttsLNArgs* a, hipStream_t st) { launch_fwd<T, TG, VEC, NV>(a, st); }
};
template <typename T, typename TG, int VEC, int NV>
struct BwdRunner {
  static void run(const MttsLNArgs* a, const MttsLNBwdArgs* b, int rb, float* part, hipStream_t st) {
    (void)a;
    launch_bwd<T, TG, VEC, NV>(b, rb, part, st);
  }
};

static int check_ln(const MttsLNArgs* a) {
  MTTS_CHECK(a && a->x && a->w && a->b && a->y && a->mean && a->rstd, "layernorm: null tensor");
  MTTS_CHECK(a->rows >= 0 && a->cols > 0, "layernorm: bad sizes");
  MTTS_CHECK(a->dtype == MTTS_F32 || a->dtype == MTTS_BF16, "layernorm: bad dtype");
  MTTS_CHECK(!a->gamma || (a->beta && a->rows_per_group > 0), "layernorm: FiLM needs beta and rows_per_group");
  return MTTS_OK;
}

}

using namespace mtts;

extern "C" int mtts_layernorm_fwd(const MttsLNArgs* a, void* stream) {
  int rc = check_ln(a);
  if (rc) return rc;
  if (a->rows == 0) return MTTS_OK;
  rc = dispatch_ln<FwdRunner>(a, (hipStream_t)stream);
  if (rc) return rc;
  MTTS_LAUNCH_CHECK("layernorm_fwd");
  return MTTS_OK;
}

extern "C" int64_t mtts_layernorm_bwd_workspace(int rows, int cols, int rows_per_group) {
  MttsLNArgs t{};
  t.gamma = rows_per_group > 0 ? (const void*)1 : nullptr;
  t.rows_per_group = rows_per_group;
  t.rows = rows;
  const int rb = ln_rb(&t);
  const int64_t nblk = (rows + rb - 1) / rb;
  return 5 * nblk * cols * 4 + 256;
}

extern "C" int mtts_layernorm_bwd(const MttsLNBwdArgs* a, void* stream) {
  MTTS_CHECK(a, "layernorm_bwd: null args");
  int rc = check_ln(&a->f);
  if (rc) return rc;
  MTTS_CHECK(a->dy && a->dx && a->dw && a->db && a->workspace, "layernorm_bwd: null tensor");
  MTTS_CHECK(!a->f.gamma || (a->dgamma && a->dbeta), "layernorm_bwd: FiLM needs dgamma/dbeta");
  const MttsLNArgs& f = a->f;
  hipStream_t st = (hipStream_t)stream;
  MTTS_CHECK(a->dgb_rs == 0 || a->dgb_rs >= f.cols, "layernorm_bwd: dgb_rs < cols");
  if (f.rows == 0) {
    (void)hipMemsetAsync(a->dw, 0, f.cols * 4, st);
    (void)hipMemsetAsync(a->db, 0, f.cols * 4, st);
    if (a->dx_colsum) (void)hipMemsetAsync(a->dx_colsum, 0, f.cols * 4, st);
    return MTTS_OK;
  }
  const int rb = ln_rb(&f);
  float* part = (float*)a->workspace;
  rc = dispatch_ln<BwdRunner>(&f, a, rb, part, st);
  if (rc) return rc;
  MTTS_LAUNCH_CHECK("layernorm_bwd");
  const int nblk = (f.rows + rb - 1) / rb;
  const int64_t slab = (int64_t)nblk * f.cols;
  ColsumJob jobs[5] = {{part, a->dw, nblk, nblk, 0}, {part + slab, a->db, nblk, nblk, 0}};
  int nj = 2;
  if (f.gamma) {
    const int bpg = f.rows_per_group / rb;
    const int64_t gs = a->dgb_rs > 0 ? a->dgb_rs : (int64_t)f.cols;
    jobs[nj++] = {part + 2 * slab, a->dgamma, nblk, bpg, gs};
    jobs[nj++] = {part + 3 * slab, a->dbeta, nblk, bpg, gs};
  }
  if (a->dx_colsum) jobs[nj++] = {part + 4 * slab, a->dx_colsum, nblk, nblk, 0};
  colsum_multi(jobs, nj, f.cols, f.cols, st);
  MTTS_LAUNCH_CHECK("layernorm_bwd_reduce");
  return MTTS_OK;
}
```

### mamba-tts-project_amd/mtts/csrc/reduce.hip

```cpp
#include "common.h"

namespace mtts {

template <typename T, int W = 4>
__global__ __launch_bounds__(64 * W) void colsum_kernel(const T* __restrict__ part, int nparts, int ppg,
                                                        int64_t pstride, int ncols, float* __restrict__ out,
                                                        int64_t out_gstride, int outer = 0) {
  __shared__ float red[W][64];
  const int lane = threadIdx.x & 63, w = threadIdx.x >> 6;
  const int c = blockIdx.x * 64 + lane;
  const int g = blockIdx.y;
  int p0 = g * ppg, p1 = min(nparts, p0 + ppg);
  if (outer > 0) {
    const int cpg = (outer + ppg - 1) / ppg;
    const int og = g / cpg;
    p0 = og * outer + (g % cpg) * ppg;
    p1 = min(min(nparts, p0 + ppg), (og + 1) * outer);
  }
  float acc[8];
#pragma unroll
  for (int q = 0; q < 8; ++q) acc[q] = 0.f;
  if (c < ncols) {
    int p = p0 + w;
    for (; p + 7 * W < p1; p += 8 * W) {
#pragma unroll
      for (int q = 0; q < 8; ++q) acc[q] += ldf(part + (int64_t)(p + W * q) * pstride + c);
    }
    for (; p < p1; p += W) acc[0] += ldf(part + (int64_t)p * pstride + c);
  }
  float s = ((acc[0] + acc[1]) + (acc[2] + acc[3])) + ((acc[4] + acc[5]) + (acc[6] + acc[7]));
  red[w][lane] = s;
  block_sync();
  if (w == 0 && c < ncols) {
    float t = 0.f;
#pragma unroll
    for (int i = 0; i < W; i += 4) t += (red[i][lane] + red[i + 1][lane]) + (red[i + 2][lane] + red[i + 3][lane]);
    out[(int64_t)g * out_gstride + c] = t;
  }
}

void colsum(const float* part, int nparts, int ppg, int64_t pstride, int ncols, float* out, int64_t out_gstride,
            hipStream_t st) {
  const int ngroups = (nparts + ppg - 1) / ppg;
  if (ngroups * ((ncols + 63) / 64) < 128 && ppg >= 64) {
    hipLaunchKernelGGL((colsum_kernel<float, 16>), dim3((ncols + 63) / 64, ngroups), dim3(1024), 0, st, part, nparts,
                       ppg, pstride, ncols, out, out_gstride);
    return;
  }
  hipLaunchKernelGGL((colsum_kernel<float, 4>), dim3((ncols + 63) / 64, ngroups), dim3(256), 0, st, part, nparts, ppg,
                     pstride, ncols, out, out_gstride);
}

struct ColsumJobs {
  ColsumJob j[5];
  int ncols;
  int64_t pstride;
};
template <int W>
__global__ __launch_bounds__(64 * W) void colsum_multi_kernel(const ColsumJobs J) {
  const ColsumJob& jb = J.j[blockIdx.z];
  const int g = blockIdx.y;
  const int p0 = g * jb.ppg;
  if (p0 >= jb.nparts) return;
  __shared__ float red[W][64];
  const int lane = threadIdx.x & 63, w = threadIdx.x >> 6;
  const int c = blockIdx.x * 64 + lane;
  const int p1 = min(jb.nparts, p0 + jb.ppg);
  float acc[8];
#pragma unroll
  for (int q = 0; q < 8; ++q) acc[q] = 0.f;
  if (c < J.ncols) {
    int p = p0 + w;
    for (; p + 7 * W < p1; p += 8 * W) {
#pragma unroll
      for (int q = 0; q < 8; ++q) acc[q] += jb.part[(int64_t)(p + W * q) * J.pstride + c];
    }
    for (; p < p1; p += W) acc[0] += jb.part[(int64_t)p * J.pstride + c];
  }
  const float s = ((acc[0] + acc[1]) + (acc[2] + acc[3])) + ((acc[4] + acc[5]) + (acc[6] + acc[7]));
  red[w][lane] = s;
  block_sync();
  if (w == 0 && c < J.ncols) {
    float t = 0.f;
#pragma unroll
    for (int i = 0; i < W; i += 4) t += (red[i][lane] + red[i + 1][lane]) + (red[i + 2][lane] + red[i + 3][lane]);
    jb.out[(int64_t)g * jb.out_gstride + c] = t;
  }
}

void colsum_multi(const ColsumJob* jobs, int n, int ncols, int64_t pstride, hipStream_t st) {
  ColsumJobs J{};
  int gmax = 1, pmax = 0;
  for (int i = 0; i < n; ++i) {
    J.j[i] = jobs[i];
    gmax = std::max(gmax, (jobs[i].nparts + jobs[i].ppg - 1) / jobs[i].ppg);
    pmax = std::max(pmax, std::min(jobs[i].ppg, jobs[i].nparts));
  }
  J.ncols = ncols;
  J.pstride = pstride;
  const dim3 grid((ncols + 63) / 64, gmax, n);
  if ((int)(grid.x * grid.y * grid.z) < 128 && pmax >= 64)
    hipLaunchKernelGGL(colsum_multi_kernel<16>, grid, dim3(1024), 0, st, J);
  else
    hipLaunchKernelGGL(colsum_multi_kernel<4>, grid, dim3(256), 0, st, J);
}

template <typename T>
__global__ __launch_bounds__(256) void colsum_rows_kernel(const T* __restrict__ in, int rows, int cols,
                                                          int64_t ld, int rchunk, float* __restrict__ part) {
  constexpr int EPL = 16 / (int)sizeof(T);
  constexpr int CB = 64 * EPL;
  __shared__ float red[4][CB];
  const int lane = threadIdx.x & 63, w = threadIdx.x >> 6;
  const int c = blockIdx.x * CB + lane * EPL;
  const int r0 = blockIdx.y * rchunk, r1 = min(rows, r0 + rchunk);
  float acc[EPL];
#pragma unroll
  for (int e = 0; e < EPL; ++e) acc[e] = 0.f;
  auto add = [&](const uint4 v) {
    if constexpr (sizeof(T) == 2) {
      const uint32_t x[4] = {v.x, v.y, v.z, v.w};
#pragma unroll
      for (int q = 0; q < 4; ++q) {
        acc[2 * q] += __uint_as_float(x[q] << 16);
        acc[2 * q + 1] += __uint_as_float(x[q] & 0xffff0000u);
      }
    } else {
      acc[0] += __uint_as_float(v.x); acc[1] += __uint_as_float(v.y);
      acc[2] += __uint_as_float(v.z); acc[3] += __uint_as_float(v.w);
    }
  };
  if (c < cols) {
    int r = r0 + w;
    for (; r + 60 < r1; r += 64) {
      uint4 v[16];
#pragma unroll
      for (int q = 0; q < 16; ++q) v[q] = *reinterpret_cast<const uint4*>(in + (int64_t)(r + 4 * q) * ld + c);
#pragma unroll
      for (int q = 0; q < 16; ++q) add(v[q]);
    }
    for (; r + 12 < r1; r += 16) {
      uint4 v[4];
#pragma unroll
      for (int q = 0; q < 4; ++q) v[q] = *reinterpret_cast<const uint4*>(in + (int64_t)(r + 4 * q) * ld + c);
#pragma unroll
      for (int q = 0; q < 4; ++q) add(v[q]);
    }
    for (; r < r1; r += 4) add(*reinterpret_cast<const uint4*>(in + (int64_t)r * ld + c));
  }
#pragma unroll
  for (int e = 0; e < EPL; ++e) red[w][lane * EPL + e] = acc[e];
  block_sync();
  for (int q = threadIdx.x; q < CB; q += 256) {
    const int cc = blockIdx.x * CB + q;
    if (cc < cols) part[(int64_t)blockIdx.y * cols + cc] = (red[0][q] + red[1][q]) + (red[2][q] + red[3][q]);
  }
}

}

extern "C" int64_t mtts_colsum_workspace(int rows, int cols, int rows_per_group) {
  if (rows_per_group <= 1024 && !(rows_per_group >= rows && rows >= 256)) return 0;
  const int64_t chunks = (int64_t)(rows + 15) / 16;
  return chunks * cols * 4 + 256;
}

extern "C" int mtts_colsum(const void* in, int dtype, int rows, int cols, int64_t row_stride, int rows_per_group,
                           float* out, int64_t out_gstride, void* workspace, void* stream) {
  using namespace mtts;
  MTTS_CHECK(in && out && rows >= 0 && cols > 0 && rows_per_group > 0, "colsum: bad args");
  MTTS_CHECK(dtype == MTTS_F32 || dtype == MTTS_BF16, "colsum: bad dtype");
  hipStream_t st = (hipStream_t)stream;
  if (rows == 0) {
    (void)hipMemsetAsync(out, 0, (size_t)cols * 4, st);
    return MTTS_OK;
  }
  const int es = dtype == MTTS_F32 ? 4 : 2;
  if (rows_per_group >= rows && rows >= 256 && cols % (16 / es) == 0 && row_stride % (16 / es) == 0 &&
      (uintptr_t)in % 16 == 0) {
    MTTS_CHECK(workspace, "colsum: workspace required (mtts_colsum_workspace)");
    int rchunk = 128;
    if (rows <= 1024) {
      const int cblocks = (cols + 64 * (16 / es) - 1) / (64 * (16 / es));
      const int want = (256 + cblocks - 1) / cblocks;
      rchunk = std::min(128, std::max(16, ((rows + want - 1) / want + 15) / 16 * 16));
    }
    const int chunks = (rows + rchunk - 1) / rchunk;
    float* part = (float*)workspace;
    if (dtype == MTTS_F32)
      hipLaunchKernelGGL(colsum_rows_kernel<float>, dim3((cols + 255) / 256, chunks), dim3(256), 0, st,
                         (const float*)in, rows, cols, row_stride, rchunk, part);
    else
      hipLaunchKernelGGL(colsum_rows_kernel<bf16_t>, dim3((cols + 511) / 512, chunks), dim3(256), 0, st,
                         (const bf16_t*)in, rows, cols, row_stride, rchunk, part);
    MTTS_LAUNCH_CHECK("colsum rows");
    colsum(part, chunks, chunks, cols, cols, out, out_gstride, st);
    MTTS_LAUNCH_CHECK("colsum chunks");
    return MTTS_OK;
  }
  if (rows_per_group > 1024) {
    MTTS_CHECK(workspace, "colsum: workspace required (mtts_colsum_workspace)");
    const int rpg = std::min(rows_per_group, rows);
    const bool ragged = rpg % 256 != 0 && rpg < rows;
    const int cpg = (rpg + 255) / 256;
    const int chunks = ragged ? ((rows + rpg - 1) / rpg) * cpg : (rows + 255) / 256;
    float* part = (float*)workspace;
    dim3 g1((cols + 63) / 64, chunks);
    if (dtype == MTTS_F32)
      hipLaunchKernelGGL((colsum_kernel<float, 4>), g1, dim3(256), 0, st, (const float*)in, rows, 256, row_stride, cols,
                         part, (int64_t)cols, ragged ? rpg : 0);
    else
      hipLaunchKernelGGL((colsum_kernel<bf16_t, 4>), g1, dim3(256), 0, st, (const bf16_t*)in, rows, 256, row_stride,
                         cols, part, (int64_t)cols, ragged ? rpg : 0);
    MTTS_LAUNCH_CHECK("colsum stage 1");
    colsum(part, chunks, rows_per_group >= rows ? chunks : cpg, cols, cols, out, out_gstride, st);
    MTTS_LAUNCH_CHECK("colsum stage 2");
    return MTTS_OK;
  }
  const int ngroups = (rows + rows_per_group - 1) / rows_per_group;
  dim3 grid((cols + 63) / 64, ngroups);
  if (dtype == MTTS_F32)
    hipLaunchKernelGGL((colsum_kernel<float, 4>), grid, dim3(256), 0, st, (const float*)in, rows, rows_per_group,
                       row_stride, cols, out, out_gstride);
  else
    hipLaunchKernelGGL((colsum_kernel<bf16_t, 4>), grid, dim3(256), 0, st, (const bf16_t*)in, rows, rows_per_group,
                       row_stride, cols, out, out_gstride);
  MTTS_LAUNCH_CHECK("colsum");
  return MTTS_OK;
}

namespace mtts {

}
```

### mamba-tts-project_amd/mtts/dp.py

```python
from __future__ import annotations

import torch
import torch.distributed as dist

from . import wgrad

DEFER_LISTENER_LAUNCH = True


class GradAllReduce:
    def __init__(self, params, bucket_mb: float = 128.0, group=None, first_bucket_mb: float = 8.0,
                 comm_dtype: torch.dtype = None):
        self.group = group
        self.world = dist.get_world_size(group)
        self.bucket_mb, self.first_bucket_mb = bucket_mb, first_bucket_mb
        self.params = [p for p in params if p.requires_grad]
        order = list(reversed(self.params))
        dev = order[0].device
        dtype = order[0].dtype
        al = max(1, 256 // torch.empty(0, dtype=dtype).element_size())
        pad = lambda n: -(-n // al) * al
        total = sum(pad(p.numel()) for p in order)
        self.flat = torch.zeros(total, device=dev, dtype=dtype)
        cap_rest = max(1, int(bucket_mb * 1024 * 1024 // self.flat.element_size()))
        cap = max(1, int(min(first_bucket_mb, bucket_mb) * 1024 * 1024 // self.flat.element_size()))
        if comm_dtype is not None and comm_dtype not in (torch.bfloat16, dtype):
            raise TypeError("GradAllReduce: comm_dtype must be None, the parameter dtype or torch.bfloat16")
        self.comm_dtype = None if comm_dtype in (None, dtype) else comm_dtype
        self.buckets = []
        self.bucket_of = {}
        off, start, count = 0, 0, 0
        self.views = {}
        for p in order:
            if p.dtype != dtype or dtype not in (torch.float32, torch.float64):
                raise TypeError("GradAllReduce expects fp32 (or, for tests, fp64) master parameters of one dtype")
            n = p.numel()
            self.views[p] = self.flat[off:off + n].as_strided(p.shape, p.stride())
            p.grad = self.views[p]
            self.bucket_of[p] = len(self.buckets)
            off += pad(n)
            count += 1
            if off - start >= cap:
                self.buckets.append([start, off, count])
                start, count = off, 0
                cap = cap_rest
        if count:
            self.buckets.append([start, off, count])
        self.cbuf = None if self.comm_dtype is None else torch.empty(total, device=dev, dtype=self.comm_dtype)
        self.pending = [0] * len(self.buckets)
        self.handles = [None] * len(self.buckets)
        self.counted = set()
        self.ready = []
        self.hooks = [p.register_post_accumulate_grad_hook(self._hook) for p in self.params]
        for p, v in self.views.items():
            p._mtts_grad_view = v
        wgrad.add_listener(self._deferred_ready)

    def _deferred_ready(self, p):
        if p in self.views:
            self._hook(p, from_listener=True)

    def zero_grad(self):
        for p in self.views:
            p.grad = None
        self.pending = [0] * len(self.buckets)
        self.handles = [None] * len(self.buckets)
        self.counted = set()

    def _hook(self, p, from_listener=False):
        if p.grad is None:
            return
        if not from_listener and wgrad.owns(p):
            return
        if id(p) in self.counted:
            return
        self.counted.add(id(p))
        v = self.views[p]
        if p.grad is not v and p.grad.data_ptr() != v.data_ptr():
            v.copy_(p.grad)
            p.grad = v
        b = self.bucket_of[p]
        self.pending[b] += 1
        if self.pending[b] == self.buckets[b][2]:
            if from_listener and DEFER_LISTENER_LAUNCH:
                self.ready.append(b)
            else:
                self._launch_ready()
                self._launch(b)
        elif not from_listener:
            self._launch_ready()

    def _launch_ready(self):
        while self.ready:
            self._launch(self.ready.pop(0))

    def _avg_op(self):
        if not hasattr(self, "_avg"):
            self._avg = dist.get_backend(self.group) == "nccl"
        return self._avg

    def _launch(self, b):
        s, e, _ = self.buckets[b]
        buf = self.flat[s:e]
        if self.cbuf is not None:
            self.cbuf[s:e].copy_(buf)
            buf = self.cbuf[s:e]
        if self._avg_op():
            try:
                self.handles[b] = dist.all_reduce(buf, op=dist.ReduceOp.AVG, group=self.group, async_op=True)
# ... 47 lines not shown
```

### mamba-tts-project_amd/mtts/gemm.py

```python
from __future__ import annotations

import torch

from . import _lib as L

EPI_BIAS, EPI_GELU, EPI_DGELU = 1, 2, 4
NT, TN = 0, 1
TILE = 256
ENABLED = True
FFN_FUSED = True


def _rowmajor(t):
    return t.dim() == 2 and t.stride(1) == 1 and t.stride(0) % 8 == 0 and t.data_ptr() % 16 == 0


def nt_ok(a: torch.Tensor, b: torch.Tensor) -> bool:
    return (ENABLED and a.dtype == torch.bfloat16 and b.dtype == torch.bfloat16 and a.is_cuda
            and _rowmajor(a) and _rowmajor(b)
            and a.shape[1] == b.shape[1] and a.shape[1] % 64 == 0 and b.shape[0] % 8 == 0 and a.shape[0] > 0)


def epi_ok(bias: torch.Tensor = None, aux: torch.Tensor = None) -> bool:
    if bias is not None and bias.data_ptr() % (16 if bias.dtype == torch.float32 else 8) != 0:
        return False
    if aux is not None and (aux.data_ptr() % 8 != 0 or aux.stride(0) % 4 != 0 or aux.stride(-1) != 1):
        return False
    return True


def tn_ok(a: torch.Tensor, b: torch.Tensor) -> bool:
    return (ENABLED and a.dtype == torch.bfloat16 and b.dtype == torch.bfloat16 and a.is_cuda
            and _rowmajor(a) and _rowmajor(b)
            and a.shape[0] == b.shape[0] and a.shape[0] % 64 == 0 and a.shape[1] % 8 == 0 and b.shape[1] % 8 == 0)


def mm_nt(a: torch.Tensor, b: torch.Tensor, bias: torch.Tensor = None, gelu_aux: torch.Tensor = None,
          dgelu_aux: torch.Tensor = None, out: torch.Tensor = None) -> torch.Tensor:
    m, k = a.shape
    n = b.shape[0]
    if not epi_ok(bias, gelu_aux if gelu_aux is not None else dgelu_aux):
        raise ValueError("mm_nt: bias / aux not aligned for the epilogue's vector accesses (gemm.epi_ok)")
    if out is None:
        out = torch.empty(m, n, device=a.device, dtype=torch.bfloat16)
    args = L.GemmArgs()
    args.m, args.n, args.k, args.layout, args.splits, args.out_dtype = m, n, k, NT, 1, 1
    epi = 0
    if bias is not None:
        epi |= EPI_BIAS
        args.bias, args.bias_dtype = bias.data_ptr(), L.dtype_code(bias)
    aux = gelu_aux if gelu_aux is not None else dgelu_aux
    if gelu_aux is not None:
        epi |= EPI_GELU
    if dgelu_aux is not None:
        epi |= EPI_DGELU
    if aux is not None:
        args.aux, args.ld_aux = aux.data_ptr(), aux.stride(0)
    args.epilogue = epi
    args.lda, args.ldb, args.ldc = a.stride(0), b.stride(0), out.stride(0)
    args.a, args.b, args.c = a.data_ptr(), b.data_ptr(), out.data_ptr()
    L.call("mtts_gemm", args)
    return out


def tn_splits(m: int, n: int, k: int) -> int:
    tiles = -(-m // TILE) * -(-n // TILE)
    min_k = 1024 if tiles >= 64 else 256
    s = 1
    while tiles * s < 256 and k % (64 * s * 2) == 0 and k // (s * 2) >= min_k:
        s *= 2
    return s


def mm_tn(a: torch.Tensor, b: torch.Tensor, out: torch.Tensor = None, beta: float = 0.0,
          splits: int = None) -> torch.Tensor:
    k, m = a.shape
    n = b.shape[1]
    if out is None:
        out = torch.empty(m, n, device=a.device, dtype=torch.float32)
    args = L.GemmArgs()
    s = tn_splits(m, n, k) if splits is None else splits
    args.m, args.n, args.k, args.layout, args.splits, args.out_dtype = m, n, k, TN, s, 0
    args.lda, args.ldb, args.ldc = a.stride(0), b.stride(0), out.stride(0)
    args.a, args.b, args.c = a.data_ptr(), b.data_ptr(), out.data_ptr()
    args.beta = beta
    ws = None
    if s > 1:
        ws = torch.empty(L.lib().mtts_gemm_workspace(args), device=a.device, dtype=torch.uint8)
        args.workspace = ws.data_ptr()
    L.call("mtts_gemm", args)
    return out


SKINNY_N, SKINNY_SMALL_K = 0, 1
SKINNY = True
SKINNY_TN_KERNEL = True
WGRAD_SKINNY_ON_TN = False
SKINNY_XPROJ = False
SKINNY_DTPROJ = True
SKINNY_DU = True


def _skinny_operand(t):
    return (t.dim() == 2 and t.dtype == torch.bfloat16 and t.is_cuda and t.stride(1) == 1 and t.stride(0) % 8 == 0
            and t.data_ptr() % 16 == 0)


def skinny_ok(a: torch.Tensor, b: torch.Tensor, out_dtype=torch.bfloat16, out: torch.Tensor = None) -> bool:
    if not (SKINNY and _skinny_operand(a) and _skinny_operand(b) and a.shape[1] == b.shape[1]):
        return False
    m, k = a.shape
    n = b.shape[0]
    if m == 0 or k % 32 or n % 4 or not (n <= 128 or k <= 128):
        return False
    if out is not None:
# ... 50 lines not shown
```

### mamba-tts-project_amd/mtts/linear.py

```python
from __future__ import annotations

import contextlib

import torch

from . import _lib as L
from . import gemm as G
from . import wgrad as WG

_scope = {"token": 0, "depth": 0}
_cast_plans = {}
TRANSPOSE_MIN = 512


def _want_t(p):
    return p.dim() == 2 and (min(p.shape) >= TRANSPOSE_MIN or getattr(p, "_mtts_want_t", False))


def _cast_multi_bf16(params):
    key = tuple((p.data_ptr(), tuple(p.shape)) for p in params)
    plan = _cast_plans.get(key)
    if plan is None:
        descs = (L.CastDesc * len(params))()
        bufs = []
# ... 43 lines not shown
                    torch.empty(p.shape, device=p.device, dtype=dtype)
                dst.append(buf)
            if src:
                with torch.no_grad():
                    torch._foreach_copy_(dst, [p.detach() for p in src])
                for p, b in zip(src, dst):
                    p._mtts_cast = (_scope["token"], b)
    _scope["depth"] += 1
    try:
        yield
    finally:
        _scope["depth"] -= 1


def cast_weight(w: torch.Tensor, dtype: torch.dtype) -> torch.Tensor:
    if w.dtype == dtype:
        return w.detach()
    ent = getattr(w, "_mtts_cast", None)
    if ent is not None and ent[0] == _scope["token"] and ent[1].dtype == dtype and ent[1].device == w.device:
        return ent[1]
    if ent is not None and ent[1].dtype == dtype and ent[1].shape == w.shape:
        t = ent[1]
        with torch.no_grad():
            t.copy_(w.detach())
    else:
        t = w.detach().to(dtype)
    w._mtts_cast = (_scope["token"], t)
    return t


def cast_weight_t(w: torch.Tensor, dtype: torch.dtype) -> torch.Tensor:
    ent = getattr(w, "_mtts_castT", None)
    if ent is not None and ent[0] == _scope["token"] and ent[1].dtype == dtype:
        return ent[1]
    t = cast_weight(w, dtype).t().contiguous()
    w._mtts_castT = (_scope["token"], t)
    return t


def colsum(x2d: torch.Tensor, out: torch.Tensor = None) -> torch.Tensor:
    if x2d.stride(-1) != 1:
        x2d = x2d.contiguous()
    rows, cols = x2d.shape
    if out is None:
        out = torch.empty(cols, device=x2d.device, dtype=torch.float32)
    rpg = max(rows, 1)
    wsz = L.lib().mtts_colsum_workspace(rows, cols, rpg)
    ws = torch.empty(wsz, device=x2d.device, dtype=torch.uint8) if wsz > 0 else None
    L.call_raw("mtts_colsum", x2d.data_ptr(), L.dtype_code(x2d), rows, cols, x2d.stride(0), rpg,
               out.data_ptr(), 0, L.ptr(ws))
    return out


def colsum_groups(x2d: torch.Tensor, rows_per_group: int) -> torch.Tensor:
    if x2d.stride(-1) != 1:
        x2d = x2d.contiguous()
    rows, cols = x2d.shape
    if rows % rows_per_group:
        raise ValueError(f"colsum_groups: rows={rows} not a multiple of {rows_per_group}")
    out = torch.empty(rows // rows_per_group, cols, device=x2d.device, dtype=torch.float32)
    wsz = L.lib().mtts_colsum_workspace(rows, cols, rows_per_group)
    ws = torch.empty(wsz, device=x2d.device, dtype=torch.uint8) if wsz > 0 else None
    L.call_raw("mtts_colsum", x2d.data_ptr(), L.dtype_code(x2d), rows, cols, x2d.stride(0), rows_per_group,
               out.data_ptr(), cols, L.ptr(ws))
    return out


HIP_WGRAD_MIN = 256


NT_MIN = 256
NT_MIN_TILES = 128


def _nt_route(x2, w, bias=None):
    m, k = x2.shape
    n = w.shape[0]
    return (n >= NT_MIN and k >= NT_MIN and -(-m // G.TILE) * -(-n // G.TILE) >= NT_MIN_TILES and G.nt_ok(x2, w)
            and (bias is None or (bias.dtype in (torch.float32, torch.bfloat16) and bias.stride(-1) == 1
                                  and G.epi_ok(bias))))


def proj(x2: torch.Tensor, w: torch.Tensor, bias: torch.Tensor = None) -> torch.Tensor:
    if _nt_route(x2, w, bias):
        return G.mm_nt(x2, w, bias=bias)
    return torch.addmm(bias, x2, w.t()) if bias is not None else x2 @ w.t()


def wgrad(dy: torch.Tensor, x: torch.Tensor, splits: int = 4, out: torch.Tensor = None) -> torch.Tensor:
    M = dy.shape[0]
    if dy.dtype == torch.float32:
        return torch.mm(dy.t(), x, out=out) if out is not None else dy.t() @ x
    big = dy.shape[1] >= HIP_WGRAD_MIN and x.shape[1] >= HIP_WGRAD_MIN
    skinny = G.WGRAD_SKINNY_ON_TN and min(dy.shape[1], x.shape[1]) >= 64 and max(dy.shape[1], x.shape[1]) >= HIP_WGRAD_MIN
    out_ok = out is None or (out.stride(1) == 1 and out.stride(0) % 4 == 0 and out.data_ptr() % 16 == 0)
    if (big or skinny) and G.tn_ok(dy, x) and out_ok:
        return G.mm_tn(dy, x, out=out)
    M64 = M // 64 * 64
    if (big or skinny) and M64 >= 1024 and M != M64 and out_ok and G.tn_ok(dy[:M64], x[:M64]):
        tail = torch.mm(dy[M64:].t(), x[M64:], out_dtype=torch.float32)
        if out is None:
            out = tail
        else:
            out.copy_(tail)
        return G.mm_tn(dy[:M64], x[:M64], out=out, beta=1.0)
    if splits > 1 and M % splits == 0 and M >= 2048:
        m = M // splits
        part = torch.bmm(dy.reshape(splits, m, -1).transpose(1, 2), x.reshape(splits, m, -1),
                         out_dtype=torch.float32)
        return torch.sum(part, 0, out=out) if out is not None else part.sum(0)
    r = torch.mm(dy.t(), x, out_dtype=torch.float32)
    if out is not None:
        out.copy_(r)
        return out
    return r


class BiasGradSlot:
    __slots__ = ("value",)

    def __init__(self):
        self.value = None

    def take(self, n):
        v, self.value = self.value, None
        return v if (v is not None and v.numel() == n) else None


class LinearFn(torch.autograd.Function):

    @staticmethod
    def forward(ctx, x, weight, bias, r0, r1, slot=None, partner=None):
        cd = x.dtype
        ctx.slot = slot
        ctx.partner = partner
        w = cast_weight(weight, cd)
        if r0 is not None:
            w = w[r0:r1]
        x2 = x.reshape(-1, x.shape[-1])
        b = None
        if bias is not None:
            b = cast_weight(bias, cd)
            if r0 is not None:
                b = b[r0:r1]
        y = proj(x2, w, b)
        ctx.save_for_backward(x2, w)
        ctx.weight = weight
        ctx.meta = (x.shape, weight.shape, weight.dtype, None if bias is None else bias.dtype, r0, r1)
        return y.view(*x.shape[:-1], w.shape[0])

    @staticmethod
    def backward(ctx, dy):
        x2, w = ctx.saved_tensors
        xshape, wshape, wdt, bdt, r0, r1 = ctx.meta
        dy2 = dy.reshape(-1, dy.shape[-1])
        if dy2.dtype != w.dtype:
            dy2 = dy2.to(w.dtype)
        dx = None
        if ctx.needs_input_grad[0]:
            if w.dtype == torch.bfloat16 and _want_t(ctx.weight):
                wt = cast_weight_t(ctx.weight, w.dtype)
                if r0 is not None:
                    wt = wt[:, r0:r1]
                dx = proj(dy2, wt).view(xshape)
            else:
                dx = (dy2 @ w).view(xshape)
        dW = db = None
        rest = ctx.partner.take() if ctx.partner is not None else None
        if rest is not None and r0 is not None:
            dyr, xr, (q0, q1) = rest
            if ctx.needs_input_grad[1] and not WG.submit([(dy2, x2, ctx.weight, (r0, r1)),
                                                          (dyr, xr, ctx.weight, (q0, q1))]):
                dW = torch.empty(wshape, device=dy2.device, dtype=torch.float32)
                wgrad(dy2, x2, out=dW[r0:r1])
                wgrad(dyr.contiguous(), xr, out=dW[q0:q1])
                if r1 - r0 + q1 - q0 < wshape[0]:
                    for a, b in ((0, min(r0, q0)), (max(r1, q1), wshape[0])):
                        if b > a:
                            dW[a:b].zero_()
                dW = dW.to(wdt)
            if bdt is not None and ctx.needs_input_grad[2]:
                db = torch.empty(wshape[0], device=dy2.device, dtype=torch.float32)
                colsum(dy2, out=db[r0:r1])
                colsum(dyr, out=db[q0:q1])
                if r1 - r0 + q1 - q0 < wshape[0]:
                    for a, b in ((0, min(r0, q0)), (max(r1, q1), wshape[0])):
                        if b > a:
                            db[a:b].zero_()
                db = db.to(bdt)
            return dx, dW, db, None, None, None, None
        if ctx.needs_input_grad[1] and not WG.submit([(dy2, x2, ctx.weight, None if r0 is None else (r0, r1))]):
            g = wgrad(dy2, x2).to(wdt)
            if r0 is not None:
                full = torch.zeros(wshape, device=g.device, dtype=wdt)
                full[r0:r1] = g
                g = full
            dW = g
        if bdt is not None and ctx.needs_input_grad[2]:
            gb = ctx.slot.take(dy2.shape[1]) if ctx.slot is not None else None
            gb = (gb if gb is not None else colsum(dy2)).to(bdt)
            if r0 is not None:
                full = torch.zeros(wshape[0], device=gb.device, dtype=bdt)
                full[r0:r1] = gb
                gb = full
            db = gb
        return dx, dW, db, None, None, None, None


def linear(x, weight, bias=None, rows=None, dbias_slot=None, partner=None):
    r0, r1 = (None, None) if rows is None else rows
    return LinearFn.apply(x, weight, bias, r0, r1, dbias_slot, partner)


class FFNFn(torch.autograd.Function):

    @staticmethod
    def forward(ctx, h, w1, b1, w2, b2, slot=None, p=0.0):
        from . import dropout as DO
        cd = h.dtype
        ctx.slot = slot
        W1, B1, W2, B2 = cast_weight(w1, cd), cast_weight(b1, cd), cast_weight(w2, cd), cast_weight(b2, cd)
        h2 = h.reshape(-1, h.shape[-1])
        pre = torch.empty(h2.shape[0], W1.shape[0], device=h.device, dtype=cd)
        a = G.mm_nt(h2, W1, bias=B1, gelu_aux=pre)
        ctx.p, ctx.seed = p, None
        if p > 0.0:
            ctx.seed = DO.new_seed()
            base, ctx.used = DO._slot(a)
            a = DO.apply_mask(a, p, ctx.seed, seed_in=base, seed_out=ctx.used)
        y = proj(a, W2, B2)
        ctx.save_for_backward(h2, pre, a, W1, W2)
        ctx.ws = (w1, w2)
        ctx.meta = (h.shape, w1.dtype, b1.dtype, w2.dtype, b2.dtype)
        return y.view(*h.shape[:-1], W2.shape[0])

    @staticmethod
    def backward(ctx, dy):
        h2, pre, a, W1, W2 = ctx.saved_tensors
        hshape, w1dt, b1dt, w2dt, b2dt = ctx.meta
        w1, w2 = ctx.ws
        dy2 = dy.reshape(-1, dy.shape[-1]).to(W2.dtype)
        W2t = cast_weight_t(w2, W2.dtype) if _want_t(w2) else W2.t().contiguous()
        if ctx.p > 0.0:
            from . import dropout as DO
            dpre = DO.apply_mask(G.mm_nt(dy2, W2t), ctx.p, ctx.seed, pre=pre, seed_in=ctx.used)
        else:
            dpre = G.mm_nt(dy2, W2t, dgelu_aux=pre)
        dh = None
        if ctx.needs_input_grad[0]:
            if _want_t(w1):
                dh = proj(dpre, cast_weight_t(w1, W1.dtype))
            else:
                dh = dpre @ W1
            dh = dh.view(hshape)
        dW1 = dW2 = None
        if ctx.needs_input_grad[1] and not WG.submit([(dpre, h2, w1, None)]):
            dW1 = wgrad(dpre, h2).to(w1dt)
        db1 = colsum(dpre).to(b1dt) if ctx.needs_input_grad[2] else None
        if ctx.needs_input_grad[3] and not WG.submit([(dy2, a, w2, None)]):
            dW2 = wgrad(dy2, a).to(w2dt)
        db2 = None
        if ctx.needs_input_grad[4]:
            db2 = ctx.slot.take(dy2.shape[1]) if ctx.slot is not None else None
            db2 = (db2 if db2 is not None else colsum(dy2)).to(b2dt)
        return dh, dW1, db1, dW2, db2, None, None


def ffn(h, w1, b1, w2, b2, dbias_slot=None, p=0.0):
    if (G.ENABLED and G.FFN_FUSED and h.dtype == torch.bfloat16 and h.is_cuda and h.shape[-1] % 64 == 0 and w1.shape[0] % 64 == 0
            and h.stride(-1) == 1 and h.is_contiguous()):
        return FFNFn.apply(h, w1, b1, w2, b2, dbias_slot, p)
    from . import dropout as DO
    a = DO.dropout(torch.nn.functional.gelu(linear(h, w1, b1)), p, p > 0.0)
    return linear(a, w2, b2, dbias_slot=dbias_slot)
```

### mamba-tts-project_amd/mtts/mamba.py

```python
from __future__ import annotations

import math

import torch
import torch.nn as nn
import torch.nn.functional as F

from . import gemm as G
from . import ops
from . import wgrad as WG
from .linear import cast_scope, cast_weight, cast_weight_t, linear, wgrad


class MambaInnerFn(torch.autograd.Function):

    @staticmethod
    def forward(ctx, xz, conv_w, conv_b, W_x, W_dt, A_log, D, dt_bias, conv_state_in, h0, seq_lens=None):
        ctx.ragged = seq_lens is not None
        need = any(ctx.needs_input_grad) and not ctx.ragged
        cd = xz.dtype
        di = xz.shape[-1] // 2
        N = A_log.shape[1]
        r = W_dt.shape[1]
        Wx, Wdt = cast_weight(W_x, cd), cast_weight(W_dt, cd)
# ... 12 lines not shown
        y, last, ckpt = ops.scan_fwd(u, delta, A_log32, Bm, Cm, D, z, dt_bias, True, h0, want_last=True,
                                     want_ckpt=need, out=y0, a_is_log=True, seq_lens=seq_lens)
        if need:
            ctx.save_for_backward(xz, conv_w, conv_b, W_x, W_dt, A_log, D, dt_bias, u, x_dbl, delta, ckpt,
                                  conv_state_in, h0, A_log32)
        ctx.mark_non_differentiable(conv_state, last)
        ctx.set_materialize_grads(False)
        return y, conv_state, last

    @staticmethod
    def backward(ctx, dy, _dconv, _dlast):
        if ctx.ragged:
            raise RuntimeError("Mamba: seq_lens (a ragged batch) is inference only: there is no backward")
        (xz, conv_w, conv_b, W_x, W_dt, A_log, D, dt_bias, u, x_dbl, delta, ckpt,
         conv_state_in, h0, A_log32) = ctx.saved_tensors
        if dy is None:
            dy = torch.zeros(xz.shape[:-1] + (xz.shape[-1] // 2,), device=xz.device, dtype=xz.dtype)
        cd = u.dtype
        Wx, Wdt = cast_weight(W_x, cd), cast_weight(W_dt, cd)
        di = xz.shape[-1] // 2
        N = A_log.shape[1]
        r = W_dt.shape[1]
        Bsz, Ln, _ = xz.shape
        x, z = xz[..., :di], xz[..., di:]
        dt, Bm, Cm = x_dbl[..., :r], x_dbl[..., r:r + N], x_dbl[..., r + N:]
        dxz = torch.empty_like(xz)
        dx_dbl = torch.empty(Bsz, Ln, r + 2 * N, device=xz.device, dtype=torch.float32)
        need_dh0 = h0 is not None and ctx.needs_input_grad[9]
        du, ddelta, _, _, _, dA_log, dD, dbias, dh0 = ops.scan_bwd(
            u, delta, A_log32, Bm, Cm, D, z, dt_bias, True, h0, ckpt, dy,
            dz=dxz[..., di:], dB=dx_dbl[..., r:r + N], dC=dx_dbl[..., r + N:], need_dh0=need_dh0, a_is_log=True)
        dd2 = ddelta.reshape(-1, di)
        dxd2 = dx_dbl.view(-1, r + 2 * N)
        WdtT = cast_weight_t(W_dt, cd) if cd == torch.bfloat16 else None
        if WdtT is not None and G.skinny_ok(dd2, WdtT, out_dtype=torch.float32, out=dxd2[:, :r]):
            G.mm_skinny(dd2, WdtT, out=dxd2[:, :r])
        else:
            dx_dbl[..., :r] = (ddelta @ Wdt).float()
        dt2 = x_dbl.view(-1, r + 2 * N)[:, :r]
        dW_dt = None
        if not WG.submit([(dd2, dt2, W_dt, None)], narrow=True):
            dW_dt = G.mm_skinny_tn(dd2, dt2) if G.skinny_tn_ok(dd2, dt2) else wgrad(dd2, dt2)
        gx = dx_dbl.to(cd).view(-1, r + 2 * N)
        du2 = du.view(-1, di)
        WxT = cast_weight_t(W_x, cd) if cd == torch.bfloat16 else None
        if WxT is not None and G.SKINNY_DU and G.skinny_ok(gx, WxT, out=du2):
            G.mm_skinny(gx, WxT, out=du2, beta=1.0)
        else:
            du2.addmm_(gx, Wx)
        u2 = u.reshape(-1, di)
        dW_x = None
        if not WG.submit([(gx, u2, W_x, None)], narrow=True):
            dW_x = G.mm_skinny_tn(u2, gx, trans_c=True) if G.skinny_tn_ok(u2, gx) else wgrad(gx, u2)
        _, dw, db = ops.conv_bwd(x, conv_w, conv_b, du, True, dx=dxz[..., :di], state_in=conv_state_in)
        dstate = None
        if conv_state_in is not None and ctx.needs_input_grad[8]:
            dstate = _conv_state_grad(x, conv_w, conv_b, conv_state_in, du)
        dA_log = dA_log.to(A_log.dtype)
        return (dxz, dw.reshape(conv_w.shape).to(conv_w.dtype), db.to(conv_b.dtype),
                None if dW_x is None else dW_x.to(W_x.dtype), None if dW_dt is None else dW_dt.to(W_dt.dtype),
                dA_log, dD.to(D.dtype), dbias.to(dt_bias.dtype), dstate,
                None if dh0 is None else dh0.to(h0.dtype), None)


def _conv_state_grad(x, conv_w, conv_b, state, du):
    K = state.shape[-1]
    di = state.shape[1]
    w = conv_w.reshape(di, K).float()
    L = x.shape[1]
    n = min(K - 1, L)
    full = torch.cat([state.float(), x[:, :n].transpose(1, 2).float()], dim=-1)
    pre = torch.stack([(full[:, :, 1 + t:1 + t + K] * w).sum(-1) for t in range(n)], dim=-1)
    if conv_b is not None:
        pre = pre + conv_b.float()[None, :, None]
    s = torch.sigmoid(pre)
    g = du[:, :n].transpose(1, 2).float() * s * (1 + pre * (1 - s))
    ds = torch.zeros_like(state, dtype=torch.float32)
    for j in range(1, K):
        for t in range(min(j, n)):
            ds[:, :, j] += w[:, j - 1 - t] * g[:, :, t]
    return ds.to(state.dtype)


class Mamba(nn.Module):
    def __init__(self, d_model, d_state=16, d_conv=4, expand=2, dt_rank="auto", dt_min=0.001, dt_max=0.1,
                 dt_init="random", dt_scale=1.0, dt_init_floor=1e-4, conv_bias=True, bias=False,
                 device=None, dtype=None):
        super().__init__()
        fk = {"device": device, "dtype": dtype}
        self.d_model = d_model
        self.d_state = d_state
        self.d_conv = d_conv
        self.expand = expand
        self.d_inner = int(expand * d_model)
        self.dt_rank = math.ceil(d_model / 16) if dt_rank == "auto" else dt_rank
        di = self.d_inner
        self.in_proj = nn.Linear(d_model, di * 2, bias=bias, **fk)
        self.conv1d = nn.Conv1d(di, di, kernel_size=d_conv, groups=di, padding=d_conv - 1, bias=conv_bias, **fk)
        self.x_proj = nn.Linear(di, self.dt_rank + d_state * 2, bias=False, **fk)
        self.dt_proj = nn.Linear(self.dt_rank, di, bias=True, **fk)
        self.x_proj.weight._mtts_want_t = True
        self.dt_proj.weight._mtts_want_t = True
        dt_init_std = self.dt_rank ** -0.5 * dt_scale
        with torch.no_grad():
            if dt_init == "constant":
                self.dt_proj.weight.fill_(dt_init_std)
            else:
                self.dt_proj.weight.uniform_(-dt_init_std, dt_init_std)
            dt = torch.exp(torch.rand(di, **fk) * (math.log(dt_max) - math.log(dt_min)) + math.log(dt_min))
            dt = dt.clamp(min=dt_init_floor)
            self.dt_proj.bias.copy_(dt + torch.log(-torch.expm1(-dt)))
        self.dt_proj.bias._no_reinit = True
# ... 53 lines not shown
```

### mamba-tts-project_amd/mtts/ops.py

```python
from __future__ import annotations

import ctypes as C

import torch

from . import _lib as L

SCAN_CKPT = 16


def _check_cuda(*ts):
    for t in ts:
        if t is not None and not t.is_cuda:
            raise RuntimeError("libmtts ops need CUDA (HIP) tensors; there is no CPU path")


def _f32c(t):
    return None if t is None else t.detach().to(torch.float32).contiguous()


def _bc_ok(t):
    es = t.element_size()
    return (t.stride(-1) == 1 and t.data_ptr() % 16 == 0 and (t.stride(0) * es) % 16 == 0
            and (t.stride(1) * es) % 16 == 0)


def _bc(t):
    return t if _bc_ok(t) else t.contiguous()


def _seq_lens(seq_lens, batch, dev, what):
    if seq_lens is None:
        return None
    t = torch.as_tensor(seq_lens)
    if t.dim() != 1 or t.shape[0] != batch or t.dtype.is_floating_point or t.dtype == torch.bool:
        raise ValueError(f"{what}: seq_lens must be {batch} integers, one per batch row")
    return t.to(device=dev, dtype=torch.int32).contiguous()


def _scan_args(u, delta, A, Bm, Cm, D, z, delta_bias, softplus, h0, out, last, ckpt, a_is_log=False):
    Bsz, Ln, Dm = u.shape
    for t in (u, delta, out) + ((z,) if z is not None else ()):
        if t.stride(-1) != 1:
            raise ValueError("scan: channel stride must be 1")
    a = L.ScanFwdArgs()
    a.batch, a.seqlen, a.dim, a.dstate = Bsz, Ln, Dm, A.shape[1]
    a.dtype_io, a.dtype_bc = L.dtype_code(u), L.dtype_code(Bm)
    a.delta_softplus = int(bool(softplus))
    a.ckpt_chunk = SCAN_CKPT if ckpt is not None else 0
    a.a_is_log = int(bool(a_is_log))
    a.u_bs, a.u_ls = u.stride(0), u.stride(1)
    a.delta_bs, a.delta_ls = delta.stride(0), delta.stride(1)
    if z is not None:
        a.z_bs, a.z_ls = z.stride(0), z.stride(1)
    a.out_bs, a.out_ls = out.stride(0), out.stride(1)
    a.B_bs, a.B_ls = Bm.stride(0), Bm.stride(1)
    a.C_bs, a.C_ls = Cm.stride(0), Cm.stride(1)
    a.u, a.delta, a.A, a.Bm, a.Cm = u.data_ptr(), delta.data_ptr(), A.data_ptr(), Bm.data_ptr(), Cm.data_ptr()
    a.D, a.z, a.delta_bias, a.h0 = L.ptr(D), L.ptr(z), L.ptr(delta_bias), L.ptr(h0)
# ... 74 lines not shown
        out, last, ckpt = scan_fwd(u, delta, A, Bm, Cm, D, z, delta_bias, softplus, want_last=True, want_ckpt=True)
        ctx.softplus = softplus
        ctx.has = (D is not None, z is not None, delta_bias is not None)
        ctx.bc_dtype = Bm.dtype
        ctx.save_for_backward(u, delta, A, Bm, Cm, D, z, delta_bias, ckpt)
        ctx.mark_non_differentiable(last)
        return out, last

    @staticmethod
    def backward(ctx, dout, dlast):
        u, delta, A, Bm, Cm, D, z, delta_bias, ckpt = ctx.saved_tensors
        du, ddelta, dz, dB, dC, dA, dD, dbias, _ = scan_bwd(u, delta, A, Bm, Cm, D, z, delta_bias, ctx.softplus,
                                                            None, ckpt, dout)
        hasD, hasz, hasb = ctx.has
        return (du, ddelta, dA.to(A.dtype), dB.to(Bm.dtype), dC.to(Cm.dtype), dD.to(D.dtype) if hasD else None,
                dz if hasz else None, dbias.to(delta_bias.dtype) if hasb else None, None, None)


def selective_scan_fn(u, delta, A, B, C, D=None, z=None, delta_bias=None, delta_softplus=False,
                      return_last_state=False):
    cl = lambda t: None if t is None else t.transpose(1, 2).contiguous()
    out, last = SelectiveScanFn.apply(cl(u), cl(delta), A, cl(B), cl(C), D, cl(z), delta_bias, delta_softplus,
                                      return_last_state)
    out = out.transpose(1, 2)
    return (out, last) if return_last_state else out


def _conv_args(x, w, bias, silu, state_in, out, state_out):
    Bsz, Ln, Dm = x.shape
    a = L.ConvFwdArgs()
    a.batch, a.dim, a.seqlen, a.width, a.dtype, a.silu = Bsz, Dm, Ln, w.shape[-1], L.dtype_code(x), int(silu)
    a.x_bs, a.x_ls = x.stride(0), x.stride(1)
    a.out_bs, a.out_ls = out.stride(0), out.stride(1)
    a.x, a.w, a.bias, a.conv_state_in = x.data_ptr(), w.data_ptr(), L.ptr(bias), L.ptr(state_in)
    a.out, a.conv_state_out = out.data_ptr(), L.ptr(state_out)
    return a


def conv_fwd(x, w, bias=None, silu=True, state_in=None, want_state=False, out=None, seq_lens=None):
    _check_cuda(x, w, bias, state_in)
    if x.stride(-1) != 1:
        x = x.contiguous()
    Bsz, Ln, Dm = x.shape
    w = _f32c(w.reshape(Dm, -1))
    bias, state_in = _f32c(bias), _f32c(state_in)
    out = torch.empty(Bsz, Ln, Dm, device=x.device, dtype=x.dtype) if out is None else out
    st = torch.empty(Bsz, Dm, w.shape[1], device=x.device, dtype=torch.float32) if want_state else None
    a = _conv_args(x, w, bias, silu, state_in, out, st)
    a.seqlens = L.ptr(_seq_lens(seq_lens, Bsz, x.device, "conv"))
    L.call("mtts_causal_conv1d_fwd", a)
    return out, st


def conv_bwd(x, w, bias, dout, silu=True, dx=None, state_in=None):
    Bsz, Ln, Dm = x.shape
    w = _f32c(w.reshape(Dm, -1))
    bias, state_in = _f32c(bias), _f32c(state_in)
    dout = dout if dout.stride(-1) == 1 else dout.contiguous()
    if dout.dtype != x.dtype:
        dout = dout.to(x.dtype)
    dx = torch.empty(Bsz, Ln, Dm, device=x.device, dtype=x.dtype) if dx is None else dx
    dw = torch.empty(Dm, w.shape[1], device=x.device, dtype=torch.float32)
    db = torch.empty(Dm, device=x.device, dtype=torch.float32)
    ws = torch.empty(L.lib().mtts_causal_conv1d_bwd_workspace(Bsz, Dm, Ln, w.shape[1]), device=x.device,
                     dtype=torch.uint8)
    b = L.ConvBwdArgs()
    b.f = _conv_args(x, w, bias, silu, state_in, dout, None)
    b.dout, b.dout_bs, b.dout_ls = dout.data_ptr(), dout.stride(0), dout.stride(1)
    b.dx, b.dx_bs, b.dx_ls = dx.data_ptr(), dx.stride(0), dx.stride(1)
    b.dw, b.dbias, b.workspace = dw.data_ptr(), db.data_ptr(), ws.data_ptr()
    L.call("mtts_causal_conv1d_bwd", b)
    return dx, dw, db


class CausalConv1dFn(torch.autograd.Function):
    @staticmethod
    def forward(ctx, x, w, bias, silu):
        out, _ = conv_fwd(x, w, bias, silu)
        ctx.silu = silu
        ctx.save_for_backward(x, w, bias)
        return out

    @staticmethod
    def backward(ctx, dout):
        x, w, bias = ctx.saved_tensors
        if x.stride(-1) != 1:
            x = x.contiguous()
        dx, dw, db = conv_bwd(x, w, bias, dout, ctx.silu)
        return dx, dw.reshape(w.shape).to(w.dtype), (db.to(bias.dtype) if bias is not None else None), None


def causal_conv1d_fn(x, weight, bias=None, activation=None):
    silu = activation in ("silu", "swish")
    out = CausalConv1dFn.apply(x.transpose(1, 2), weight, bias, silu)
    return out.transpose(1, 2)


def conv_update(x, conv_state, w, bias=None, silu=True, out=None):
    _check_cuda(x, conv_state, w)
    Bsz, Dm = x.shape
    if x.stride(-1) != 1:
        x = x.contiguous()
    out = torch.empty(Bsz, Dm, device=x.device, dtype=x.dtype) if out is None else out
    a = L.ConvUpdateArgs()
    a.batch, a.dim, a.width, a.dtype, a.silu = Bsz, Dm, conv_state.shape[-1], L.dtype_code(x), int(silu)
    a.x_bs, a.out_bs = x.stride(0), out.stride(0)
    a.x, a.conv_state, a.w, a.bias, a.out = x.data_ptr(), conv_state.data_ptr(), w.data_ptr(), L.ptr(bias), out.data_ptr()
    L.call("mtts_causal_conv1d_update", a)
    return out


def state_update(state, x, dt, A, Bm, Cm, D=None, z=None, dt_bias=None, softplus=True, out=None, dt_w=None,
                 packed_out=False):
    _check_cuda(state, x, dt, A, Bm, Cm, dt_w)
    for t in (Bm, Cm, dt):
        if t.stride(-1) != 1:
            raise ValueError("state_update: B / C / dt need unit element stride")
    Bsz, Dm = x.shape
    yp = PackedAct.empty(Bsz, Dm, x.device) if packed_out else None
    if not packed_out:
        out = torch.empty(Bsz, Dm, device=x.device, dtype=x.dtype) if out is None else out
    a = L.StateUpdateArgs()
    a.batch, a.dim, a.dstate = Bsz, Dm, state.shape[-1]
# ... 36 lines not shown
        if t.shape[d] > 1 and t.stride(d) != st * _prod(t.shape[d + 1:-1]):
            raise ValueError("layernorm: leading dims must be collapsible")
    return rows, st


def _prod(s):
    p = 1
    for v in s:
        p *= v
    return p


def _ln_args(x, w, b, eps, res, x_sum, gamma, beta, rows_per_group, y, mean, rstd):
    rows, xrs = _rows(x)
    a = L.LNArgs()
    a.rows, a.cols, a.dtype, a.eps = rows, x.shape[-1], L.dtype_code(x), float(eps)
    a.rows_per_group = int(rows_per_group) if gamma is not None else 0
    a.x_rs, a.y_rs = xrs, _rows(y)[1]
    a.x, a.w, a.b, a.y, a.mean, a.rstd = x.data_ptr(), w.data_ptr(), b.data_ptr(), y.data_ptr(), mean.data_ptr(), rstd.data_ptr()
    if res is not None:
        a.res, a.res_rs = res.data_ptr(), _rows(res)[1]
        if x_sum is not None:
            a.x_sum, a.xsum_rs = x_sum.data_ptr(), _rows(x_sum)[1]
    if gamma is not None:
        a.gamma, a.beta, a.gb_rs, a.gb_dtype = gamma.data_ptr(), beta.data_ptr(), gamma.stride(0), L.dtype_code(gamma)
    return a


def layernorm_fwd(x, w, b, eps=1e-5, res=None, gamma=None, beta=None, rows_per_group=1, want_sum=True):
    _check_cuda(x, w, b, res, gamma, beta)
    if x.stride(-1) != 1:
        x = x.contiguous()
    if res is not None and (res.shape != x.shape):
        raise ValueError("layernorm: res shape mismatch")
    if res is not None and res.dtype != x.dtype:
        res = res.to(x.dtype)
    w, b = _f32c(w), _f32c(b)
    if gamma is not None:
        gamma = gamma if gamma.stride(-1) == 1 else gamma.contiguous()
        beta = beta if beta.stride(-1) == 1 else beta.contiguous()
        if beta.stride(0) != gamma.stride(0):
            beta = beta.contiguous()
            gamma = gamma.contiguous()
    rows = x.numel() // x.shape[-1]
    y = torch.empty(x.shape, device=x.device, dtype=x.dtype)
    mean = torch.empty(rows, device=x.device, dtype=torch.float32)
    rstd = torch.empty(rows, device=x.device, dtype=torch.float32)
    x_sum = torch.empty(x.shape, device=x.device, dtype=x.dtype) if (res is not None and want_sum) else None
    L.call("mtts_layernorm_fwd", _ln_args(x, w, b, eps, res, x_sum, gamma, beta, rows_per_group, y, mean, rstd))
    return y, mean, rstd, x_sum


def layernorm_bwd(xn, w, b, eps, gamma, beta, rows_per_group, mean, rstd, dy, dx_acc=None, dgb=None,
                  dx_colsum=None):
    dy = dy if dy.stride(-1) == 1 else dy.contiguous()
    if dy.dtype != xn.dtype:
        dy = dy.to(xn.dtype)
    w, b = _f32c(w), _f32c(b)
    rows, cols = mean.numel(), xn.shape[-1]
    dx = torch.empty(xn.shape, device=xn.device, dtype=xn.dtype)
    dw = torch.empty(cols, device=xn.device, dtype=torch.float32)
    db = torch.empty(cols, device=xn.device, dtype=torch.float32)
    film = gamma is not None
    G = rows // rows_per_group if film else 0
    if film and dgb is not None:
        dg, dbe = dgb[:, :cols], dgb[:, cols:]
    else:
        dg = torch.empty(G, cols, device=xn.device, dtype=torch.float32) if film else None
        dbe = torch.empty(G, cols, device=xn.device, dtype=torch.float32) if film else None
    ws = torch.empty(L.lib().mtts_layernorm_bwd_workspace(rows, cols, rows_per_group if film else 0),
                     device=xn.device, dtype=torch.uint8)
    bb = L.LNBwdArgs()
    bb.f = _ln_args(xn, w, b, eps, None, None, gamma, beta, rows_per_group, xn, mean, rstd)
    bb.dy, bb.dy_rs = dy.data_ptr(), _rows(dy)[1]
    if dx_acc is not None:
        dx_acc = dx_acc if dx_acc.stride(-1) == 1 else dx_acc.contiguous()
        if dx_acc.dtype != xn.dtype:
            dx_acc = dx_acc.to(xn.dtype)
        bb.dx_acc, bb.dxacc_rs = dx_acc.data_ptr(), _rows(dx_acc)[1]
    bb.dx, bb.dx_rs = dx.data_ptr(), _rows(dx)[1]
    bb.dw, bb.db, bb.dgamma, bb.dbeta, bb.workspace = dw.data_ptr(), db.data_ptr(), L.ptr(dg), L.ptr(dbe), ws.data_ptr()
    bb.dgb_rs = dg.stride(0) if film else 0
    bb.dx_colsum = L.ptr(dx_colsum)
    L.call("mtts_layernorm_bwd", bb)
    return dx, dw, db, dg, dbe


class LayerNormFn(torch.autograd.Function):

    @staticmethod
    def forward(ctx, x, res, w, b, gamma, beta, eps, rows_per_group, film, colsum_slot):
        if film is not None:
            n = x.shape[-1]
            gamma, beta = film[:, :n], film[:, n:]
        y, mean, rstd, x_sum = layernorm_fwd(x, w, b, eps, res, gamma, beta, rows_per_group)
        xn = x_sum if res is not None else x
        ctx.set_materialize_grads(False)
        ctx.eps, ctx.rpg = eps, rows_per_group
        ctx.has_res = res is not None
        ctx.has_film = film is not None
        ctx.slot = colsum_slot
        ctx.dtypes = (w.dtype, b.dtype, None if gamma is None else gamma.dtype)
        ctx.save_for_backward(xn, w, b, gamma, beta, mean, rstd)
        if res is None:
            x_sum = x.new_empty(0)
            ctx.mark_non_differentiable(x_sum)
        return y, x_sum

    @staticmethod
    def backward(ctx, dy, dsum):
        xn, w, b, gamma, beta, mean, rstd = ctx.saved_tensors
        if dsum is not None and dsum.numel() == 0:
            dsum = None
        if dy is None:
            dy = torch.zeros_like(xn)
        n = xn.shape[-1]
        dgb = None
        if ctx.has_film:
            dgb = torch.empty(gamma.shape[0], 2 * n, device=xn.device, dtype=torch.float32)
        csum = None
        if ctx.slot is not None:
            csum = torch.empty(n, device=xn.device, dtype=torch.float32)
        dx, dw, db, dg, dbe = layernorm_bwd(xn, w, b, ctx.eps, gamma, beta, ctx.rpg, mean, rstd, dy, dx_acc=dsum,
                                            dgb=dgb, dx_colsum=csum)
        if csum is not None:
            ctx.slot.value = csum
        wd, bd, gd = ctx.dtypes
        dres = dx if ctx.has_res else None
        if ctx.has_film:
            return (dx, dres, dw.to(wd), db.to(bd), None, None, None, None, dgb.to(gd), None)
        return (dx, dres, dw.to(wd), db.to(bd), None if dg is None else dg.to(gd),
                None if dbe is None else dbe.to(gd), None, None, None, None)


def layer_norm(x, w, b, eps=1e-5, res=None, gamma=None, beta=None, rows_per_group=1, film=None, colsum_slot=None):
    return LayerNormFn.apply(x, res, w, b, gamma, beta, eps, rows_per_group, film, colsum_slot)



def _dur_f32(durations):
    d = durations.detach()
    if d.dtype != torch.float32:
        d = d.to(torch.float32)
    return d if d.stride(-1) == 1 else d.contiguous()


def length_regulate_lengths(durations):
    _check_cuda(durations)
    d = _dur_f32(durations)
    B, T = d.shape
    out = torch.empty(B, device=d.device, dtype=torch.int64)
    L.call_raw("mtts_length_regulate_lengths", d.data_ptr(), d.stride(0), B, T, out.data_ptr())
    return out


class LengthRegulateFn(torch.autograd.Function):

    @staticmethod
    def forward(ctx, hidden, durations, max_len):
        _check_cuda(hidden, durations)
        h = hidden if hidden.stride(-1) == 1 else hidden.contiguous()
        d = _dur_f32(durations)
        B, T, D = h.shape
        out = torch.empty(B, max_len, D, device=h.device, dtype=h.dtype)
        L.call_raw("mtts_length_regulate_fwd", h.data_ptr(), L.dtype_code(h), B, T, D, h.stride(0), h.stride(1),
                   d.data_ptr(), d.stride(0), max_len, out.data_ptr(), out.stride(0), out.stride(1))
        ctx.save_for_backward(d)
        ctx.meta = (T, max_len)
        return out

    @staticmethod
    def backward(ctx, dout):
        (d,) = ctx.saved_tensors
        T, max_len = ctx.meta
        g = dout if dout.stride(-1) == 1 else dout.contiguous()
        B, _, D = g.shape
        dh = torch.empty(B, T, D, device=g.device, dtype=g.dtype)
        L.call_raw("mtts_length_regulate_bwd", g.data_ptr(), L.dtype_code(g), B, T, D, g.stride(0), g.stride(1),
                   d.data_ptr(), d.stride(0), max_len, dh.data_ptr(), dh.stride(0), dh.stride(1))
        return dh, None, None
# ... 273 lines not shown
```

### mamba-tts-project_amd/mtts/wgrad.py

```python
from __future__ import annotations

import contextlib
import ctypes as C
import heapq

import torch

from . import _lib as L
from . import gemm as G

GROUP_TILES = 192
MAX_PROBLEMS = 64
LAYER_PROBLEMS = 24
FILL_ROUNDS = True
FILL = 0.95
HOLD_BYTES = 6 << 30
_LAYER_TILES = GROUP_TILES
_BK = 64
MIN_GROUP_TILES = 128
SIDE_STREAM = False

_depth = 0


class _Job:
    __slots__ = ("dy", "x", "param", "rows")

    def __init__(self, dy, x, param, rows):
        self.dy, self.x, self.param, self.rows = dy, x, param, rows

    def tiles(self):
        m, n = self.dy.shape[1], self.x.shape[1]
        return -(-m // G.TILE) * -(-n // G.TILE)

    def nbytes(self):
        return self.dy.numel() * self.dy.element_size() + self.x.numel() * self.x.element_size()


def makespan(work, cus):
    by_k = {}
    for t, k in work:
        if t > 0 and k > 0:
            by_k[k] = by_k.get(k, 0) + t
    loads = [0] * cus
    for k in sorted(by_k, reverse=True):
        t = by_k[k]
        if loads[-1] - loads[0] > k:
            heapq.heapify(loads)
            top = max(loads)
            while t and top - loads[0] > k:
                new = loads[0] + k
                heapq.heapreplace(loads, new)
                top = max(top, new)
                t -= 1
            loads.sort()
        q, r = divmod(t, cus)
        if q:
            loads = [v + q * k for v in loads]
        if r:
            loads[:r] = [v + k for v in loads[:r]]
            loads.sort()
    return loads[-1]


def utilisation(work, cus):
    total = sum(t * k for t, k in work if t > 0 and k > 0)
    return total / (cus * makespan(work, cus)) if total else 0.0


def plan_groups(work, nbytes, cus):
    n = 1
    while n * len(work) <= MAX_PROBLEMS - 2 and n * nbytes <= HOLD_BYTES:
        if utilisation(work * n, cus) >= FILL:
            return n
        n += 1
    return 1


class RoundQueue:

    def __init__(self):
        self.clear()

    def clear(self):
        self.work = []
        self.held = 0
        self.tiles = 0
        self.jobs = 0
        self.groups = 0
        self.plan = 1

    def add(self, tiles, ktiles, nbytes):
        self.work.append((tiles, ktiles))
        self.held += nbytes
        self.tiles += tiles
        self.jobs += 1

    def full(self, cus):
        if len(self.work) >= MAX_PROBLEMS - 2:
            return True
        if self.tiles < GROUP_TILES and self.jobs < LAYER_PROBLEMS - 2:
            return False
        self.tiles = self.jobs = 0
        self.groups += 1
        if self.groups == 1:
            self.plan = plan_groups(self.work, self.held, cus)
        return self.groups >= self.plan or self.held >= HOLD_BYTES


_cus = {}


def cu_count(dev):
    i = dev.index if dev.index is not None else torch.cuda.current_device()
    if i not in _cus:
        _cus[i] = torch.cuda.get_device_properties(i).multi_processor_count
    return _cus[i]


class _Engine:
    def __init__(self):
        self.jobs = []
        self.tiles = 0
        self.queue = RoundQueue()
        self.callback_queued = False
        self.done = set()
        self.covered = {}
        self.listeners = []
        self.side = {}
        self.used_side = None

    def reset_pass(self):
        self.callback_queued = False
        self.done = set()
        self.covered = {}
        self.used_side = None


_E = _Engine()


def active() -> bool:
    return _depth > 0


@contextlib.contextmanager
def deferred(enable: bool = True):
    global _depth
    if not enable:
        yield
        return
    _depth += 1
    try:
        yield
    finally:
        _depth -= 1
        if _depth == 0 and (_E.jobs or _E.used_side is not None):
            _end_of_backward()


def owns(p) -> bool:
    if id(p) in _E.done:
        return False
    return id(p) in _E.covered or any(j.param is p for j in _E.jobs)


def add_listener(fn):
    _E.listeners.append(fn)


def remove_listener(fn):
    if fn in _E.listeners:
        _E.listeners.remove(fn)


def _eligible(dy, x, param, narrow=False):
    return (active() and param is not None and param.requires_grad and param.dtype == torch.float32
            and param.dim() == 2 and (narrow or (dy.shape[1] >= 256 and x.shape[1] >= 256)) and G.tn_ok(dy, x))


def _end_of_backward():
    flush()
    if _E.used_side is not None:
        main, side = _E.used_side
        main.wait_stream(side)
    for key, (p, _, _) in list(_E.covered.items()):
        if key not in _E.done:
            _announce(p)
    _E.reset_pass()


def _announce(p):
    _E.done.add(id(p))
    for fn in _E.listeners:
        fn(p)


def _cover(p, rows):
    r0, r1 = rows if rows is not None else (0, p.shape[0])
    _, ivs, overlap = _E.covered.get(id(p), (p, [], False))
    overlap = overlap or any(a < r1 and r0 < b for a, b in ivs)
    ivs = ivs + [(r0, r1)]
    _E.covered[id(p)] = (p, ivs, overlap)
    if overlap:
        return False
    return sum(b - a for a, b in ivs) >= p.shape[0]


def _side_stream(dev):
    i = dev.index if dev.index is not None else torch.cuda.current_device()
    st = _E.side.get(i)
    if st is None:
        st = _E.side[i] = torch.cuda.Stream(device=i)
    return st


def submit(jobs, narrow=False) -> bool:
    if not jobs or not all(_eligible(dy, x, p, narrow) for dy, x, p, _ in jobs):
        return False
    param = jobs[0][2]
    for dy, x, p, rows in jobs:
        r0, r1 = rows if rows is not None else (0, p.shape[0])
        if p is not param or p.shape[1] != x.shape[1] or r1 - r0 != dy.shape[1]:
            return False
    if id(param) in _E.done and _E.listeners:
        raise RuntimeError("wgrad: a parameter's weight gradient was submitted after its gradient was announced "
                           "complete to a listener (a weight used again later in the backward under GradAllReduce); "
                           "run this backward outside mtts.wgrad.deferred()")
    if any(j.param is param for j in _E.jobs):
        flush()
    if not _E.callback_queued:
        torch.autograd.Variable._execution_engine.queue_callback(_end_of_backward)
        _E.callback_queued = True
    for dy, x, p, rows in jobs:
        j = _Job(dy, x, p, rows)
        _E.jobs.append(j)
        _E.tiles += j.tiles()
        _E.queue.add(j.tiles(), dy.shape[0] // _BK, j.nbytes())
    if not FILL_ROUNDS or _E.listeners or GROUP_TILES < _LAYER_TILES:
        if _E.tiles >= GROUP_TILES or len(_E.jobs) >= LAYER_PROBLEMS - 2:
            flush()
    elif _E.queue.full(cu_count(dy.device)):
        flush()
    return True


def flush():
    jobs, _E.jobs, _E.tiles = _E.jobs, [], 0
    _E.queue.clear()
    if not jobs:
        return
    if not (SIDE_STREAM and _E.callback_queued):
        _flush(jobs)
        return
    main = torch.cuda.current_stream()
    side = _side_stream(jobs[0].dy.device)
    side.wait_stream(main)
    _E.used_side = (main, side)
    for j in jobs:
        j.dy.record_stream(side)
        j.x.record_stream(side)
    with torch.cuda.stream(side):
        _flush(jobs, side)


def _flush(jobs, side=None):
    dest, covered = {}, {}
    for j in jobs:
        covered[id(j.param)] = covered.get(id(j.param), 0) + ((j.rows[1] - j.rows[0]) if j.rows else j.param.shape[0])
    for j in jobs:
        p = j.param
        if id(p) in dest:
            continue
        if p.grad is not None:
            dest[id(p)] = (p.grad, 1.0, False)
            continue
        cover = covered[id(p)]
        view = getattr(p, "_mtts_grad_view", None)
        full = cover >= p.shape[0]
        if view is not None:
            if not full:
                view.zero_()
            g = view
        else:
            g = torch.empty(p.shape, device=p.device, dtype=torch.float32) if full else \
                torch.zeros(p.shape, device=p.device, dtype=torch.float32)
        if side is not None:
            g.record_stream(side)
        dest[id(p)] = (g, 0.0 if full else 1.0, True)
    probs, fixups = [], []
    for j in jobs:
        g, beta, _ = dest[id(j.param)]
        out = g if j.rows is None else g[j.rows[0]:j.rows[1]]
        if not _addressable(out):
            tmp = torch.empty(out.shape, device=out.device, dtype=torch.float32)
            if side is not None:
                tmp.record_stream(side)
            fixups.append((out, tmp, beta))
            out, beta = tmp, 0.0
        probs.append((j.dy, j.x, out, beta))
# ... 44 lines not shown
```

Baseline: 552,500 tokens/s.

## Defer and batch bias/LN/conv parameter-gradient reductions into one launch

Bias, LayerNorm and conv weight-gradient partial sums are no longer reduced by a separate kernel per op. Their reduce jobs are recorded and later launched together through a new mtts_reduce_batch call, which writes straight into the parameter .grad buffers (accumulating when a gradient already exists). A GEMM epilogue variant that emits per-tile column sums is also added so bias gradients can come out of the dgrad GEMM. The aim is fewer small launches and less memory traffic in backward, at the cost of holding partial buffers longer and a more complex gradient-ownership and announcement path.

```diff
diff --git a/include/mtts.h b/include/mtts.h
--- a/include/mtts.h
+++ b/include/mtts.h
@@ -90,6 +90,18 @@
 int mtts_selective_scan_bwd(const MttsScanBwdArgs* a, void* stream);
 
 typedef struct {
+  const float* part;
+  float* out;
+  float* out2;
+  int64_t pstride, out_gstride;
+  int nparts, ppg, ncols, split;
+  int waves;
+  float beta;
+} MttsReduceJob;
+
+int mtts_reduce_batch(const MttsReduceJob* jobs, int n, void* stream);
+
+typedef struct {
   int batch, dim, seqlen, width;
   int dtype;
   int silu;
@@ -112,6 +124,7 @@
   float* dw;
   float* dbias;
   void* workspace;
+  MttsReduceJob* defer_job;
 } MttsConvBwdArgs;
 
 int64_t mtts_causal_conv1d_bwd_workspace(int batch, int dim, int seqlen, int width);
@@ -183,6 +196,7 @@
   void* workspace;
   float* dx_colsum;
   int64_t dgb_rs;
+  MttsReduceJob* defer_jobs;
 } MttsLNBwdArgs;
 
 int64_t mtts_layernorm_bwd_workspace(int rows, int cols, int rows_per_group);
@@ -191,6 +205,8 @@
 int64_t mtts_colsum_workspace(int rows, int cols, int rows_per_group);
 int mtts_colsum(const void* in, int dtype, int rows, int cols, int64_t row_stride, int rows_per_group, float* out,
                 int64_t out_gstride, void* workspace, void* stream);
+int mtts_colsum_partials(const void* in, int dtype, int rows, int cols, int64_t row_stride, void* workspace,
+                         MttsReduceJob* job, void* stream);
 
 typedef struct {
   int batch, heads, head_dim, q_len, kv_len;
@@ -355,6 +371,7 @@
   void* aux;
   void* workspace;
   float beta;
+  float* colsum_c;
 } MttsGemmArgs;
 
 int64_t mtts_gemm_workspace(const MttsGemmArgs* a);
diff --git a/mamba-tts-project_amd/mtts/_lib.py b/mamba-tts-project_amd/mtts/_lib.py
--- a/mamba-tts-project_amd/mtts/_lib.py
+++ b/mamba-tts-project_amd/mtts/_lib.py
@@ -44,7 +44,8 @@
 
 class ConvBwdArgs(C.Structure):
     _fields_ = [("f", ConvFwdArgs), ("dout", vp), ("dout_bs", i64), ("dout_ls", i64),
-                ("dx", vp), ("dx_bs", i64), ("dx_ls", i64), ("dw", vp), ("dbias", vp), ("workspace", vp)]
+                ("dx", vp), ("dx_bs", i64), ("dx_ls", i64), ("dw", vp), ("dbias", vp), ("workspace", vp),
+                ("defer_job", vp)]
 
 
 class ConvUpdateArgs(C.Structure):
@@ -78,7 +79,8 @@
 class GemmArgs(C.Structure):
     _fields_ = [("m", i32), ("n", i32), ("k", i32), ("layout", i32), ("splits", i32), ("epilogue", i32),
                 ("out_dtype", i32), ("bias_dtype", i32), ("lda", i64), ("ldb", i64), ("ldc", i64), ("ld_aux", i64),
-                ("a", vp), ("b", vp), ("c", vp), ("bias", vp), ("aux", vp), ("workspace", vp), ("beta", f32)]
+                ("a", vp), ("b", vp), ("c", vp), ("bias", vp), ("aux", vp), ("workspace", vp), ("beta", f32),
+                ("colsum_c", vp)]
 
 
 class DropoutArgs(C.Structure):
@@ -122,7 +124,7 @@
 class LNBwdArgs(C.Structure):
     _fields_ = [("f", LNArgs), ("dy", vp), ("dy_rs", i64), ("dx_acc", vp), ("dxacc_rs", i64),
                 ("dx", vp), ("dx_rs", i64), ("dw", vp), ("db", vp), ("dgamma", vp), ("dbeta", vp),
-                ("workspace", vp), ("dx_colsum", vp), ("dgb_rs", i64)]
+                ("workspace", vp), ("dx_colsum", vp), ("dgb_rs", i64), ("defer_jobs", vp)]
 
 
 class AttnFwdArgs(C.Structure):
@@ -143,6 +145,11 @@
     _fields_ = [("f", AttnFwdArgs), ("dout", vp), ("do_bs", i64), ("do_ls", i64),
                 ("dq", vp), ("dq_bs", i64), ("dq_ls", i64), ("dk", vp), ("dk_bs", i64), ("dk_ls", i64),
                 ("dv", vp), ("dv_bs", i64), ("dv_ls", i64), ("workspace", vp)]
+
+
+class ReduceJob(C.Structure):
+    _fields_ = [("part", vp), ("out", vp), ("out2", vp), ("pstride", i64), ("out_gstride", i64),
+                ("nparts", i32), ("ppg", i32), ("ncols", i32), ("split", i32), ("waves", i32), ("beta", f32)]
 
 
 class CastDesc(C.Structure):
@@ -187,6 +194,8 @@
     "mtts_layernorm_bwd": ([C.POINTER(LNBwdArgs), vp], i32),
     "mtts_colsum_workspace": ([i32, i32, i32], i64),
     "mtts_colsum": ([vp, i32, i32, i32, i64, i32, vp, i64, vp, vp], i32),
+    "mtts_colsum_partials": ([vp, i32, i32, i32, i64, vp, C.POINTER(ReduceJob), vp], i32),
+    "mtts_reduce_batch": ([C.POINTER(ReduceJob), i32, vp], i32),
     "mtts_attention_fwd": ([C.POINTER(AttnFwdArgs), vp], i32),
     "mtts_attention_decode_qproj": ([C.POINTER(AttnQProjArgs), vp], i32),
     "mtts_attention_bwd_workspace": ([i32, i32, i32, i32, i32, i32], i64),
@@ -218,7 +227,8 @@
                                "(make -C mamba-tts-project_amd/mtts/csrc)")
         L = C.CDLL(LIB_PATH)
         for sym, what in (("mtts_embed_sum_at", "ragged prompts"),
-                          ("mtts_gemm_grouped_rounds", "round-filling weight gradients")):
+                          ("mtts_gemm_grouped_rounds", "round-filling weight gradients"),
+                          ("mtts_reduce_batch", "batched parameter-gradient reductions")):
             if not hasattr(L, sym):
                 raise RuntimeError(f"{LIB_PATH} is stale: it was built before {sym} ({what}) was "
                                    "added; rebuild it with __graft_entry__.build() "
diff --git a/mamba-tts-project_amd/mtts/attention.py b/mamba-tts-project_amd/mtts/attention.py
--- a/mamba-tts-project_amd/mtts/attention.py
+++ b/mamba-tts-project_amd/mtts/attention.py
@@ -8,7 +8,7 @@
 
 from . import attn_kernels
 from . import wgrad as WG
-from .linear import _want_t, cast_scope, cast_weight, cast_weight_t, colsum, linear, proj, wgrad
+from .linear import _want_t, cast_scope, cast_weight, cast_weight_t, colsum, defer_bias, linear, proj, wgrad
 
 
 class InProjFn(torch.autograd.Function):
@@ -23,6 +23,7 @@
         kv = proj(k2, Wc[d:], bc[d:])
         ctx.save_for_backward(x2, k2, Wc)
         ctx.weight = weight
+        ctx.bias_p = bias
         ctx.meta = (query.shape, key.shape, weight.dtype, bias.dtype)
         return q.view(*query.shape[:-1], d), kv.view(*key.shape[:-1], 2 * d)
 
@@ -47,7 +48,7 @@
             wgrad(dq2, x2, out=dW[:d])
             wgrad(dkv2, k2, out=dW[d:])
             dW = dW.to(wdt)
-        if ctx.needs_input_grad[3]:
+        if ctx.needs_input_grad[3] and not defer_bias([(dq2, (0, d)), (dkv2, (d, 3 * d))], ctx.bias_p):
             db = torch.empty(3 * d, device=x2.device, dtype=torch.float32)
             colsum(dq2, out=db[:d])
             colsum(dkv2, out=db[d:])
@@ -135,7 +136,7 @@
                 if ctx.needs_input_grad[2 + 2 * l] and not WG.submit([(dy, k2, W, (d, 3 * d))]):
                     dW = torch.zeros(W.shape, device=W.device, dtype=W.dtype)
                     dW[d:] = wgrad(dy.contiguous(), k2).to(W.dtype)
-                if ctx.needs_input_grad[3 + 2 * l]:
+                if ctx.needs_input_grad[3 + 2 * l] and not defer_bias([(dy, (d, 3 * d))], b):
                     db = torch.zeros(b.shape, device=b.device, dtype=b.dtype)
                     db[d:] = colsum(dy).to(b.dtype)
             grads += [dW, db]
diff --git a/mamba-tts-project_amd/mtts/csrc/common.h b/mamba-tts-project_amd/mtts/csrc/common.h
--- a/mamba-tts-project_amd/mtts/csrc/common.h
+++ b/mamba-tts-project_amd/mtts/csrc/common.h
@@ -19,7 +19,9 @@
   int nparts, ppg;
   int64_t out_gstride;
 };
-void colsum_multi(const ColsumJob* jobs, int n, int ncols, int64_t pstride, hipStream_t st);
+void colsum_multi(const ColsumJob* jobs, int n, int ncols, int64_t pstride, hipStream_t st, int waves = 0);
+int colsum_waves(int nparts, int ppg, int ncols);
+int colsum_multi_waves(const ColsumJob* jobs, int n, int ncols);
 
 #define MTTS_CHECK(cond, ...)                                                 \
   do {                                                                        \
diff --git a/mamba-tts-project_amd/mtts/csrc/conv.hip b/mamba-tts-project_amd/mtts/csrc/conv.hip
--- a/mamba-tts-project_amd/mtts/csrc/conv.hip
+++ b/mamba-tts-project_amd/mtts/csrc/conv.hip
@@ -501,7 +501,8 @@
   MTTS_CHECK(a, "conv1d_bwd: null args");
   int rc = check_conv(&a->f);
   if (rc) return rc;
-  MTTS_CHECK(a->dout && a->dx && a->dw && a->workspace, "conv1d_bwd: null tensor");
+  MTTS_CHECK(a->dout && a->dx && (a->dw || a->defer_job) && a->workspace, "conv1d_bwd: null tensor");
+  if (a->defer_job) *a->defer_job = MttsReduceJob{};
   MTTS_CHECK(!a->f.seqlens, "conv1d_bwd: seqlens is inference only");
   const MttsConvFwdArgs& f = a->f;
   if (f.seqlen == 0) return MTTS_OK;
@@ -525,6 +526,18 @@
     else nparts = launch_bwd<bf16_t, 1>(a, st, part, false);
   }
   MTTS_LAUNCH_CHECK("causal_conv1d_bwd");
+  if (a->defer_job) {
+    MttsReduceJob& r = *a->defer_job;
+    r.part = part;
+    r.out = a->dw;
+    r.out2 = a->dbias;
+    r.pstride = (int64_t)f.dim * (kK + 1);
+    r.nparts = r.ppg = nparts;
+    r.ncols = f.dim * (kK + 1);
+    r.split = kK;
+    r.waves = colsum_waves(nparts, nparts, f.dim * (kK + 1));
+    return MTTS_OK;
+  }
   float* sums = part + (int64_t)nparts * f.dim * (kK + 1);
   colsum(part, nparts, nparts, (int64_t)f.dim * (kK + 1), f.dim * (kK + 1), sums, 0, st);
   hipLaunchKernelGGL(conv_bwd_split, dim3((f.dim * (kK + 1) + 255) / 256), dim3(256), 0, st, sums, f.dim, a->dw,
diff --git a/mamba-tts-project_amd/mtts/csrc/gemm.hip b/mamba-tts-project_amd/mtts/csrc/gemm.hip
--- a/mamba-tts-project_amd/mtts/csrc/gemm.hip
+++ b/mamba-tts-project_amd/mtts/csrc/gemm.hip
@@ -38,6 +38,7 @@
   int bias_bf16;
   int wide_out;
   float beta;
+  float* colsum;
 };
 
 __device__ __forceinline__ int a_map(int rr, int s) { return (rr >> 6) * 128 + s * 64 + (rr & 63); }
@@ -541,7 +542,7 @@
   }
 }
 
-template <int EPI, bool OUT_F32>
+template <int EPI, bool OUT_F32, bool CS = false>
 __device__ __forceinline__ void store_tile_buf(const GemmParams& p, f32x4 (&acc)[8][4], const f32x4 (&bias)[4],
                                                int m0, int n0, int wr, int wc, int lane, int split) {
   const int rl = lane & 15, cl = 4 * (lane >> 4);
@@ -575,6 +576,7 @@
     const int cw0 = n0 + wc * 64 + (g & 1) * 16 + 8 * (g >> 1);
     const __amdgpu_buffer_rsrc_t rc = brsrc(p.c, (uint32_t)((int64_t)p.m * p.ldc * 2));
     const __amdgpu_buffer_rsrc_t ra = brsrc(p.aux, (uint32_t)((int64_t)p.m * p.ld_aux * 2));
+    f32x4 cs[4] = {};
 #pragma unroll
     for (int MB = 0; MB < 8; ++MB) {
       const int row = m0 + wr * 128 + MB * 16 + rl;
@@ -622,6 +624,10 @@
         }
         o2[NB][0] = o[0] | ((uint32_t)o[1] << 16);
         o2[NB][1] = o[2] | ((uint32_t)o[3] << 16);
+        if constexpr (CS) {
+#pragma unroll
+          for (int j = 0; j < 4; ++j) cs[NB][j] += rok ? bf2f(o[j]) : 0.f;
+        }
       }
 #pragma unroll
       for (int pr = 0; pr < 2; ++pr) {
@@ -646,6 +652,26 @@
           __builtin_amdgcn_raw_buffer_store_b128(i32x4{(int)w[0], (int)w[1], (int)w[2], (int)w[3]}, ra,
                                                  ok ? (uint32_t)((row * p.ld_aux + cw) * 2) : kOOB, 0, 0);
         }
+      }
+    }
+    if constexpr (CS) {
+      const int srow = m0 / 128 + wr;
+      const __amdgpu_buffer_rsrc_t rs = brsrc(p.colsum, (uint32_t)((int64_t)2 * p.tiles_m * p.n * 4));
+#pragma unroll
+      for (int NB = 0; NB < 4; ++NB) {
+        f32x4 v = cs[NB];
+#pragma unroll
+        for (int j = 0; j < 4; ++j) {
+          float t = v[j];
+          t += dpp<kQuadXor1>(t);
+          t += dpp<kQuadXor2>(t);
+          t += xor4(t, lane);
+          t += xor8(t);
+          v[j] = t;
+        }
+        const int col = n0 + wc * 64 + NB * 16 + cl;
+        const uint32_t off = (rl == 0 && col < p.n) ? (uint32_t)((srow * p.n + col) * 4) : kOOB;
+        __builtin_amdgcn_raw_buffer_store_b128(__builtin_bit_cast(i32x4, v), rs, off, 0, 0);
       }
     }
   }
@@ -707,7 +733,7 @@
   return (xcd < r8 ? xcd * (q8 + 1) : r8 * (q8 + 1) + (xcd - r8) * q8) + bid / 8;
 }
 
-template <bool AK, bool BKM, int EPI, bool OUT_F32>
+template <bool AK, bool BKM, int EPI, bool OUT_F32, bool CS = false>
 __device__ __forceinline__ void gemm_pp_body(const GemmParams& p, const int wid) {
   __shared__ __attribute__((aligned(16))) char lds[kLds];
   const int tid = threadIdx.x, lane = tid & 63, wave = __builtin_amdgcn_readfirstlane(tid >> 6);
@@ -821,12 +847,12 @@
   }
 #undef PP_MFMA
   if (wr == 0) sbar();
-  store_tile_buf<EPI, OUT_F32>(p, acc, bias, cur.m0, cur.n0, wr, wc, lane, cur.split);
-}
-
-template <bool AK, bool BKM, int EPI, bool OUT_F32>
+  store_tile_buf<EPI, OUT_F32, CS>(p, acc, bias, cur.m0, cur.n0, wr, wc, lane, cur.split);
+}
+
+template <bool AK, bool BKM, int EPI, bool OUT_F32, bool CS = false>
 __global__ __launch_bounds__(kThreads, 1) void gemm_pp_kernel(GemmParams p) {
-  gemm_pp_body<AK, BKM, EPI, OUT_F32>(p, xcd_work_id());
+  gemm_pp_body<AK, BKM, EPI, OUT_F32, CS>(p, xcd_work_id());
 }
 
 constexpr int kGroupMax = 24;
@@ -1033,6 +1059,17 @@
     }
   }
   hipLaunchKernelGGL((gemm_pp_kernel<AK, BKM, EPI, F32>), dim3(nwg), dim3(kThreads), 0, st, p);
+}
+
+template <int EPI>
+bool launch_colsum(const GemmParams& p, int nwg, hipStream_t st) {
+  const int64_t cbytes = (int64_t)p.m * p.ldc * 2;
+  const int64_t abytes = (EPI & MTTS_GEMM_EPI_DGELU) ? (int64_t)p.m * p.ld_aux * 2 : 0;
+  if (!p.wide_out || cbytes >= (1ll << 31) || abytes >= (1ll << 31) || (int64_t)2 * p.tiles_m * p.n * 4 >= (1ll << 31) ||
+      override_of(MTTS_OVR_GEMM_NARROW) == 1 || override_of(MTTS_OVR_GEMM_TILE) == 2)
+    return false;
+  hipLaunchKernelGGL((gemm_pp_kernel<true, true, EPI, false, true>), dim3(nwg), dim3(kThreads), 0, st, p);
+  return true;
 }
 
 }
@@ -1096,6 +1133,18 @@
                (!a->aux || (uintptr_t)a->aux % 16 == 0) && override_of(MTTS_OVR_GEMM_NARROW) != 1;
   const int nwg = p.tiles_m * p.tiles_n * splits;
   hipStream_t st = (hipStream_t)stream;
+  if (a->colsum_c) {
+    MTTS_CHECK(nt && !f32out && (epi == 0 || epi == MTTS_GEMM_EPI_DGELU) && (uintptr_t)a->colsum_c % 16 == 0,
+               "gemm: colsum_c goes with NT, bf16 out, the plain or DGELU epilogue, 16-byte aligned");
+    p.colsum = a->colsum_c;
+    const bool ok = epi == 0 ? launch_colsum<0>(p, nwg, st) : launch_colsum<MTTS_GEMM_EPI_DGELU>(p, nwg, st);
+    if (!ok) {
+      set_error("gemm: colsum_c needs the ping-pong kernel (16-byte C / aux rows, spans below 2 GiB, no tile override)");
+      return MTTS_EUNSUPPORTED;
+    }
+    MTTS_LAUNCH_CHECK("gemm");
+    return MTTS_OK;
+  }
   if (!nt) {
     launch<false, false, 0, true>(p, nwg, st);
   } else if (f32out) {
diff --git a/mamba-tts-project_amd/mtts/csrc/ln.hip b/mamba-tts-project_amd/mtts/csrc/ln.hip
--- a/mamba-tts-project_amd/mtts/csrc/ln.hip
+++ b/mamba-tts-project_amd/mtts/csrc/ln.hip
@@ -325,12 +325,14 @@
   MTTS_CHECK(a, "layernorm_bwd: null args");
   int rc = check_ln(&a->f);
   if (rc) return rc;
-  MTTS_CHECK(a->dy && a->dx && a->dw && a->db && a->workspace, "layernorm_bwd: null tensor");
+  MTTS_CHECK(a->dy && a->dx && ((a->dw && a->db) || a->defer_jobs) && a->workspace, "layernorm_bwd: null tensor");
   MTTS_CHECK(!a->f.gamma || (a->dgamma && a->dbeta), "layernorm_bwd: FiLM needs dgamma/dbeta");
   const MttsLNArgs& f = a->f;
   hipStream_t st = (hipStream_t)stream;
   MTTS_CHECK(a->dgb_rs == 0 || a->dgb_rs >= f.cols, "layernorm_bwd: dgb_rs < cols");
+  if (a->defer_jobs) a->defer_jobs[0] = a->defer_jobs[1] = a->defer_jobs[2] = MttsReduceJob{};
   if (f.rows == 0) {
+    MTTS_CHECK(a->dw && a->db, "layernorm_bwd: no rows: nothing to defer, dw / db required");
     (void)hipMemsetAsync(a->dw, 0, f.cols * 4, st);
     (void)hipMemsetAsync(a->db, 0, f.cols * 4, st);
     if (a->dx_colsum) (void)hipMemsetAsync(a->dx_colsum, 0, f.cols * 4, st);
@@ -352,6 +354,27 @@
     jobs[nj++] = {part + 3 * slab, a->dbeta, nblk, bpg, gs};
   }
   if (a->dx_colsum) jobs[nj++] = {part + 4 * slab, a->dx_colsum, nblk, nblk, 0};
+  if (a->defer_jobs) {
+    const int waves = colsum_multi_waves(jobs, nj, f.cols);
+    auto defer = [&](int slot, const ColsumJob& j) {
+      MttsReduceJob& r = a->defer_jobs[slot];
+      r.part = j.part;
+      r.out = j.out;
+      r.pstride = f.cols;
+      r.nparts = j.nparts;
+      r.ppg = j.ppg;
+      r.ncols = f.cols;
+      r.waves = waves;
+    };
+    defer(0, jobs[0]);
+    defer(1, jobs[1]);
+    if (a->dx_colsum) defer(2, jobs[nj - 1]);
+    if (f.gamma) {
+      colsum_multi(jobs + 2, 2, f.cols, f.cols, st, waves);
+      MTTS_LAUNCH_CHECK("layernorm_bwd_reduce");
+    }
+    return MTTS_OK;
+  }
   colsum_multi(jobs, nj, f.cols, f.cols, st);
   MTTS_LAUNCH_CHECK("layernorm_bwd_reduce");
   return MTTS_OK;
diff --git a/mamba-tts-project_amd/mtts/csrc/reduce.hip b/mamba-tts-project_amd/mtts/csrc/reduce.hip
--- a/mamba-tts-project_amd/mtts/csrc/reduce.hip
+++ b/mamba-tts-project_amd/mtts/csrc/reduce.hip
@@ -39,10 +39,15 @@
   }
 }
 
+int colsum_waves(int nparts, int ppg, int ncols) {
+  const int ngroups = (nparts + ppg - 1) / ppg;
+  return ngroups * ((ncols + 63) / 64) < 128 && ppg >= 64 ? 16 : 4;
+}
+
 void colsum(const float* part, int nparts, int ppg, int64_t pstride, int ncols, float* out, int64_t out_gstride,
             hipStream_t st) {
   const int ngroups = (nparts + ppg - 1) / ppg;
-  if (ngroups * ((ncols + 63) / 64) < 128 && ppg >= 64) {
+  if (colsum_waves(nparts, ppg, ncols) == 16) {
     hipLaunchKernelGGL((colsum_kernel<float, 16>), dim3((ncols + 63) / 64, ngroups), dim3(1024), 0, st, part, nparts,
                        ppg, pstride, ncols, out, out_gstride);
     return;
@@ -88,21 +93,96 @@
   }
 }
 
-void colsum_multi(const ColsumJob* jobs, int n, int ncols, int64_t pstride, hipStream_t st) {
+int colsum_multi_waves(const ColsumJob* jobs, int n, int ncols) {
+  int gmax = 1, pmax = 0;
+  for (int i = 0; i < n; ++i) {
+    gmax = std::max(gmax, (jobs[i].nparts + jobs[i].ppg - 1) / jobs[i].ppg);
+    pmax = std::max(pmax, std::min(jobs[i].ppg, jobs[i].nparts));
+  }
+  return ((ncols + 63) / 64) * gmax * n < 128 && pmax >= 64 ? 16 : 4;
+}
+
+void colsum_multi(const ColsumJob* jobs, int n, int ncols, int64_t pstride, hipStream_t st, int waves) {
   ColsumJobs J{};
-  int gmax = 1, pmax = 0;
+  int gmax = 1;
   for (int i = 0; i < n; ++i) {
     J.j[i] = jobs[i];
     gmax = std::max(gmax, (jobs[i].nparts + jobs[i].ppg - 1) / jobs[i].ppg);
-    pmax = std::max(pmax, std::min(jobs[i].ppg, jobs[i].nparts));
   }
   J.ncols = ncols;
   J.pstride = pstride;
   const dim3 grid((ncols + 63) / 64, gmax, n);
-  if ((int)(grid.x * grid.y * grid.z) < 128 && pmax >= 64)
+  if (waves == 0) waves = colsum_multi_waves(jobs, n, ncols);
+  if (waves == 16)
     hipLaunchKernelGGL(colsum_multi_kernel<16>, grid, dim3(1024), 0, st, J);
   else
     hipLaunchKernelGGL(colsum_multi_kernel<4>, grid, dim3(256), 0, st, J);
+}
+
+constexpr int kBatchJobs = 56;
+struct BatchJob {
+  const float* part;
+  float* out;
+  float* out2;
+  int64_t pstride, out_gstride;
+  int nparts, ppg, ncols, split;
+  int beta, blk0;
+};
+struct BatchTable {
+  BatchJob j[kBatchJobs];
+  int n;
+};
+static_assert(sizeof(BatchTable) <= 4096 - 64 && offsetof(BatchTable, j) == 0,
+              "the job table travels in the kernel arguments, read from offset 0");
+
+template <int W>
+__global__ __launch_bounds__(64 * W) void reduce_batch_kernel(const BatchTable T) {
+  BatchJob jb{};
+#if defined(__HIP_DEVICE_COMPILE__)
+  typedef const __attribute__((address_space(4))) BatchJob* KJob;
+  const KJob tab = (KJob)__builtin_amdgcn_kernarg_segment_ptr();
+  int lo = 0, hi = T.n;
+  while (hi - lo > 1) {
+    const int mid = (lo + hi) >> 1;
+    if ((int)blockIdx.x >= tab[mid].blk0) lo = mid;
+    else hi = mid;
+  }
+  jb = tab[lo];
+#endif
+  __shared__ float red[W][64];
+  const int lane = threadIdx.x & 63, w = threadIdx.x >> 6;
+  const int cb = (jb.ncols + 63) / 64;
+  const int local = blockIdx.x - jb.blk0;
+  const int g = local / cb;
+  const int c = (local % cb) * 64 + lane;
+  const int p0 = g * jb.ppg, p1 = min(jb.nparts, p0 + jb.ppg);
+  const float* __restrict__ part = jb.part;
+  const int64_t ps = jb.pstride;
+  float acc[8];
+#pragma unroll
+  for (int q = 0; q < 8; ++q) acc[q] = 0.f;
+  if (c < jb.ncols) {
+    int p = p0 + w;
+    for (; p + 7 * W < p1; p += 8 * W) {
+#pragma unroll
+      for (int q = 0; q < 8; ++q) acc[q] += part[(int64_t)(p + W * q) * ps + c];
+    }
+    for (; p < p1; p += W) acc[0] += part[(int64_t)p * ps + c];
+  }
+  const float s = ((acc[0] + acc[1]) + (acc[2] + acc[3])) + ((acc[4] + acc[5]) + (acc[6] + acc[7]));
+  red[w][lane] = s;
+  block_sync();
+  if (w == 0 && c < jb.ncols) {
+    float t = 0.f;
+#pragma unroll
+    for (int i = 0; i < W; i += 4) t += (red[i][lane] + red[i + 1][lane]) + (red[i + 2][lane] + red[i + 3][lane]);
+    float* o = jb.out + (int64_t)g * jb.out_gstride + c;
+    if (jb.split > 0) {
+      const int ch = c / (jb.split + 1), k = c % (jb.split + 1);
+      o = k < jb.split ? jb.out + ch * jb.split + k : (jb.out2 ? jb.out2 + ch : nullptr);
+    }
+    if (o) *o = jb.beta ? *o + t : t;
+  }
 }
 
 template <typename T>
@@ -159,6 +239,35 @@
 
 }
 
+namespace mtts {
+
+static bool rows_chunked_ok(const void* in, int dtype, int rows, int cols, int64_t row_stride, int rows_per_group) {
+  const int es = dtype == MTTS_F32 ? 4 : 2;
+  return rows_per_group >= rows && rows >= 256 && cols % (16 / es) == 0 && row_stride % (16 / es) == 0 &&
+         (uintptr_t)in % 16 == 0;
+}
+
+static int launch_rows_chunks(const void* in, int dtype, int rows, int cols, int64_t row_stride, float* part,
+                              hipStream_t st) {
+  const int es = dtype == MTTS_F32 ? 4 : 2;
+  int rchunk = 128;
+  if (rows <= 1024) {
+    const int cblocks = (cols + 64 * (16 / es) - 1) / (64 * (16 / es));
+    const int want = (256 + cblocks - 1) / cblocks;
+    rchunk = std::min(128, std::max(16, ((rows + want - 1) / want + 15) / 16 * 16));
+  }
+  const int chunks = (rows + rchunk - 1) / rchunk;
+  if (dtype == MTTS_F32)
+    hipLaunchKernelGGL(colsum_rows_kernel<float>, dim3((cols + 255) / 256, chunks), dim3(256), 0, st,
+                       (const float*)in, rows, cols, row_stride, rchunk, part);
+  else
+    hipLaunchKernelGGL(colsum_rows_kernel<bf16_t>, dim3((cols + 511) / 512, chunks), dim3(256), 0, st,
+                       (const bf16_t*)in, rows, cols, row_stride, rchunk, part);
+  return chunks;
+}
+
+}
+
 extern "C" int64_t mtts_colsum_workspace(int rows, int cols, int rows_per_group) {
   if (rows_per_group <= 1024 && !(rows_per_group >= rows && rows >= 256)) return 0;
   const int64_t chunks = (int64_t)(rows + 15) / 16;
@@ -175,24 +284,10 @@
     (void)hipMemsetAsync(out, 0, (size_t)cols * 4, st);
     return MTTS_OK;
   }
-  const int es = dtype == MTTS_F32 ? 4 : 2;
-  if (rows_per_group >= rows && rows >= 256 && cols % (16 / es) == 0 && row_stride % (16 / es) == 0 &&
-      (uintptr_t)in % 16 == 0) {
+  if (rows_chunked_ok(in, dtype, rows, cols, row_stride, rows_per_group)) {
     MTTS_CHECK(workspace, "colsum: workspace required (mtts_colsum_workspace)");
-    int rchunk = 128;
-    if (rows <= 1024) {
-      const int cblocks = (cols + 64 * (16 / es) - 1) / (64 * (16 / es));
-      const int want = (256 + cblocks - 1) / cblocks;
-      rchunk = std::min(128, std::max(16, ((rows + want - 1) / want + 15) / 16 * 16));
-    }
-    const int chunks = (rows + rchunk - 1) / rchunk;
     float* part = (float*)workspace;
-    if (dtype == MTTS_F32)
-      hipLaunchKernelGGL(colsum_rows_kernel<float>, dim3((cols + 255) / 256, chunks), dim3(256), 0, st,
-                         (const float*)in, rows, cols, row_stride, rchunk, part);
-    else
-      hipLaunchKernelGGL(colsum_rows_kernel<bf16_t>, dim3((cols + 511) / 512, chunks), dim3(256), 0, st,
-                         (const bf16_t*)in, rows, cols, row_stride, rchunk, part);
+    const int chunks = launch_rows_chunks(in, dtype, rows, cols, row_stride, part, st);
     MTTS_LAUNCH_CHECK("colsum rows");
     colsum(part, chunks, chunks, cols, cols, out, out_gstride, st);
     MTTS_LAUNCH_CHECK("colsum chunks");
@@ -229,6 +324,64 @@
   return MTTS_OK;
 }
 
-namespace mtts {
-
-}
+extern "C" int mtts_colsum_partials(const void* in, int dtype, int rows, int cols, int64_t row_stride, void* workspace,
+                                    MttsReduceJob* job, void* stream) {
+  using namespace mtts;
+  MTTS_CHECK(in && job && rows >= 0 && cols > 0, "colsum_partials: bad args");
+  MTTS_CHECK(dtype == MTTS_F32 || dtype == MTTS_BF16, "colsum_partials: bad dtype");
+  *job = MttsReduceJob{};
+  if (!rows_chunked_ok(in, dtype, rows, cols, row_stride, rows)) return MTTS_OK;
+  MTTS_CHECK(workspace, "colsum_partials: workspace required (mtts_colsum_workspace)");
+  float* part = (float*)workspace;
+  const int chunks = launch_rows_chunks(in, dtype, rows, cols, row_stride, part, (hipStream_t)stream);
+  MTTS_LAUNCH_CHECK("colsum rows");
+  job->part = part;
+  job->pstride = cols;
+  job->nparts = job->ppg = chunks;
+  job->ncols = cols;
+  job->waves = colsum_waves(chunks, chunks, cols);
+  return MTTS_OK;
+}
+
+extern "C" int mtts_reduce_batch(const MttsReduceJob* jobs, int n, void* stream) {
+  using namespace mtts;
+  MTTS_CHECK(n >= 0 && (jobs || n == 0), "reduce_batch: bad args");
+  for (int i = 0; i < n; ++i) {
+    const MttsReduceJob& j = jobs[i];
+    if (j.nparts == 0) continue;
+    MTTS_CHECK(j.part && j.out && j.nparts > 0 && j.ppg > 0 && j.ncols > 0 && j.pstride >= j.ncols,
+               "reduce_batch: job %d: bad sizes or null tensor", i);
+    MTTS_CHECK(j.waves == 0 || j.waves == 4 || j.waves == 16, "reduce_batch: job %d: waves must be 0, 4 or 16", i);
+    MTTS_CHECK(j.beta == 0.f || j.beta == 1.f, "reduce_batch: job %d: beta must be 0 or 1", i);
+    MTTS_CHECK(j.split >= 0 && (j.split == 0 || (j.ppg >= j.nparts && j.ncols % (j.split + 1) == 0)),
+               "reduce_batch: job %d: split needs one group and ncols a multiple of split + 1", i);
+  }
+  hipStream_t st = (hipStream_t)stream;
+  for (int W : {16, 4}) {
+    BatchTable T{};
+    int blocks = 0;
+    auto launch = [&]() {
+      if (T.n == 0) return;
+      if (W == 16) hipLaunchKernelGGL(reduce_batch_kernel<16>, dim3(blocks), dim3(1024), 0, st, T);
+      else hipLaunchKernelGGL(reduce_batch_kernel<4>, dim3(blocks), dim3(256), 0, st, T);
+      T.n = 0;
+      blocks = 0;
+    };
+    for (int i = 0; i < n; ++i) {
+      const MttsReduceJob& j = jobs[i];
+      if (j.nparts == 0) continue;
+      if ((j.waves ? j.waves : colsum_waves(j.nparts, j.ppg, j.ncols)) != W) continue;
+      BatchJob& b = T.j[T.n++];
+      b.part = j.part; b.out = j.out; b.out2 = j.out2;
+      b.pstride = j.pstride; b.out_gstride = j.out_gstride;
+      b.nparts = j.nparts; b.ppg = j.ppg; b.ncols = j.ncols; b.split = j.split;
+      b.beta = j.beta != 0.f;
+      b.blk0 = blocks;
+      blocks += ((j.nparts + j.ppg - 1) / j.ppg) * ((j.ncols + 63) / 64);
+      if (T.n == kBatchJobs) launch();
+    }
+    launch();
+    MTTS_LAUNCH_CHECK("reduce_batch");
+  }
+  return MTTS_OK;
+}
diff --git a/mamba-tts-project_amd/mtts/dp.py b/mamba-tts-project_amd/mtts/dp.py
--- a/mamba-tts-project_amd/mtts/dp.py
+++ b/mamba-tts-project_amd/mtts/dp.py
@@ -54,7 +54,7 @@
         self.hooks = [p.register_post_accumulate_grad_hook(self._hook) for p in self.params]
         for p, v in self.views.items():
             p._mtts_grad_view = v
-        wgrad.add_listener(self._deferred_ready)
+        wgrad.add_listener(self._deferred_ready, reductions=True)
 
     def _deferred_ready(self, p):
         if p in self.views:
diff --git a/mamba-tts-project_amd/mtts/gemm.py b/mamba-tts-project_amd/mtts/gemm.py
--- a/mamba-tts-project_amd/mtts/gemm.py
+++ b/mamba-tts-project_amd/mtts/gemm.py
@@ -35,8 +35,17 @@
             and a.shape[0] == b.shape[0] and a.shape[0] % 64 == 0 and a.shape[1] % 8 == 0 and b.shape[1] % 8 == 0)
 
 
+def colsum_c_ok(m: int, n: int, aux: torch.Tensor = None) -> bool:
+    lib = L.lib()
+    if lib.mtts_get_override(L.OVERRIDES["gemm_narrow"]) == 1 or lib.mtts_get_override(L.OVERRIDES["gemm_tile"]) == 2:
+        return False
+    if n % 8 != 0 or m * n * 2 >= 1 << 31:
+        return False
+    return aux is None or (aux.stride(0) % 8 == 0 and aux.data_ptr() % 16 == 0 and m * aux.stride(0) * 2 < 1 << 31)
+
+
 def mm_nt(a: torch.Tensor, b: torch.Tensor, bias: torch.Tensor = None, gelu_aux: torch.Tensor = None,
-          dgelu_aux: torch.Tensor = None, out: torch.Tensor = None) -> torch.Tensor:
+          dgelu_aux: torch.Tensor = None, out: torch.Tensor = None, colsum_c: bool = False):
     m, k = a.shape
     n = b.shape[0]
     if not epi_ok(bias, gelu_aux if gelu_aux is not None else dgelu_aux):
@@ -59,8 +68,12 @@
     args.epilogue = epi
     args.lda, args.ldb, args.ldc = a.stride(0), b.stride(0), out.stride(0)
     args.a, args.b, args.c = a.data_ptr(), b.data_ptr(), out.data_ptr()
+    slab = None
+    if colsum_c:
+        slab = torch.empty(2 * -(-m // TILE), n, device=a.device, dtype=torch.float32)
+        args.colsum_c = slab.data_ptr()
     L.call("mtts_gemm", args)
-    return out
+    return (out, slab) if colsum_c else out
 
 
 def tn_splits(m: int, n: int, k: int) -> int:
diff --git a/mamba-tts-project_amd/mtts/linear.py b/mamba-tts-project_amd/mtts/linear.py
--- a/mamba-tts-project_amd/mtts/linear.py
+++ b/mamba-tts-project_amd/mtts/linear.py
@@ -119,6 +119,38 @@
     return out
 
 
+def colsum_deferrable(x2d: torch.Tensor) -> bool:
+    e = 16 // x2d.element_size()
+    return (x2d.dim() == 2 and x2d.dtype in (torch.float32, torch.bfloat16) and x2d.stride(1) == 1
+            and x2d.shape[0] >= 256 and x2d.shape[1] % e == 0 and x2d.stride(0) % e == 0 and x2d.data_ptr() % 16 == 0)
+
+
+def colsum_pending(x2d: torch.Tensor):
+    import ctypes as C
+    rows, cols = x2d.shape
+    ws = torch.empty(L.lib().mtts_colsum_workspace(rows, cols, rows), device=x2d.device, dtype=torch.uint8)
+    job = L.ReduceJob()
+    L.call_raw("mtts_colsum_partials", x2d.data_ptr(), L.dtype_code(x2d), rows, cols, x2d.stride(0), ws.data_ptr(),
+               C.byref(job))
+    if job.nparts == 0:
+        raise RuntimeError("colsum_pending: the shape does not take the two-stage path (colsum_deferrable)")
+    return WG.Pending(ws, job, cols)
+
+
+def defer_bias(parts, bias) -> bool:
+    if bias is None or not WG.reduce_on(bias):
+        return False
+    if not all(isinstance(s, WG.Pending) or colsum_deferrable(s) for s, _ in parts):
+        return False
+    for s, rows in parts:
+        WG.submit_reduce(s if isinstance(s, WG.Pending) else colsum_pending(s), bias, rows)
+    return True
+
+
+def _now(v):
+    return v.materialize() if isinstance(v, WG.Pending) else v
+
+
 def colsum_groups(x2d: torch.Tensor, rows_per_group: int) -> torch.Tensor:
     if x2d.stride(-1) != 1:
         x2d = x2d.contiguous()
@@ -213,6 +245,7 @@
         y = proj(x2, w, b)
         ctx.save_for_backward(x2, w)
         ctx.weight = weight
+        ctx.bias_p = bias
         ctx.meta = (x.shape, weight.shape, weight.dtype, None if bias is None else bias.dtype, r0, r1)
         return y.view(*x.shape[:-1], w.shape[0])
 
@@ -246,7 +279,8 @@
                         if b > a:
                             dW[a:b].zero_()
                 dW = dW.to(wdt)
-            if bdt is not None and ctx.needs_input_grad[2]:
+            if bdt is not None and ctx.needs_input_grad[2] and not defer_bias([(dy2, (r0, r1)), (dyr, (q0, q1))],
+                                                                              ctx.bias_p):
                 db = torch.empty(wshape[0], device=dy2.device, dtype=torch.float32)
                 colsum(dy2, out=db[r0:r1])
                 colsum(dyr, out=db[q0:q1])
@@ -265,12 +299,14 @@
             dW = g
         if bdt is not None and ctx.needs_input_grad[2]:
             gb = ctx.slot.take(dy2.shape[1]) if ctx.slot is not None else None
-            gb = (gb if gb is not None else colsum(dy2)).to(bdt)
-            if r0 is not None:
-                full = torch.zeros(wshape[0], device=gb.device, dtype=bdt)
-                full[r0:r1] = gb
-                gb = full
-            db = gb
+            if not defer_bias([(gb if gb is not None else dy2, None if r0 is None else (r0, r1))], ctx.bias_p):
+                gb = _now(gb)
+                gb = (gb if gb is not None else colsum(dy2)).to(bdt)
+                if r0 is not None:
+                    full = torch.zeros(wshape[0], device=gb.device, dtype=bdt)
+                    full[r0:r1] = gb
+                    gb = full
+                db = gb
         return dx, dW, db, None, None, None, None
 
 
@@ -298,6 +334,7 @@
         y = proj(a, W2, B2)
         ctx.save_for_backward(h2, pre, a, W1, W2)
         ctx.ws = (w1, w2)
+        ctx.bs = (b1, b2)
         ctx.meta = (h.shape, w1.dtype, b1.dtype, w2.dtype, b2.dtype)
         return y.view(*h.shape[:-1], W2.shape[0])
 
@@ -308,9 +345,18 @@
         w1, w2 = ctx.ws
         dy2 = dy.reshape(-1, dy.shape[-1]).to(W2.dtype)
         W2t = cast_weight_t(w2, W2.dtype) if _want_t(w2) else W2.t().contiguous()
+        b1, b2 = ctx.bs
+        db1_done = False
         if ctx.p > 0.0:
             from . import dropout as DO
             dpre = DO.apply_mask(G.mm_nt(dy2, W2t), ctx.p, ctx.seed, pre=pre, seed_in=ctx.used)
+        elif ctx.needs_input_grad[2] and WG.reduce_on(b1) and G.colsum_c_ok(dy2.shape[0], W2t.shape[0], pre):
+            dpre, slab = G.mm_nt(dy2, W2t, dgelu_aux=pre, colsum_c=True)
+            job = L.ReduceJob()
+            job.part, job.pstride, job.ncols = slab.data_ptr(), slab.shape[1], slab.shape[1]
+            job.nparts = job.ppg = slab.shape[0]
+            WG.submit_reduce(WG.Pending(slab, job, slab.shape[1]), b1)
+            db1_done = True
         else:
             dpre = G.mm_nt(dy2, W2t, dgelu_aux=pre)
         dh = None
@@ -323,13 +369,19 @@
         dW1 = dW2 = None
         if ctx.needs_input_grad[1] and not WG.submit([(dpre, h2, w1, None)]):
             dW1 = wgrad(dpre, h2).to(w1dt)
-        db1 = colsum(dpre).to(b1dt) if ctx.needs_input_grad[2] else None
+        db1 = None
+        if ctx.needs_input_grad[2] and not db1_done and not defer_bias([(dpre, None)], b1):
+            db1 = colsum(dpre).to(b1dt)
         if ctx.needs_input_grad[3] and not WG.submit([(dy2, a, w2, None)]):
             dW2 = wgrad(dy2, a).to(w2dt)
         db2 = None
         if ctx.needs_input_grad[4]:
             db2 = ctx.slot.take(dy2.shape[1]) if ctx.slot is not None else None
-            db2 = (db2 if db2 is not None else colsum(dy2)).to(b2dt)
+            if defer_bias([(db2 if db2 is not None else dy2, None)], b2):
+                db2 = None
+            else:
+                db2 = _now(db2)
+                db2 = (db2 if db2 is not None else colsum(dy2)).to(b2dt)
         return dh, dW1, db1, dW2, db2, None, None
 
 
diff --git a/mamba-tts-project_amd/mtts/mamba.py b/mamba-tts-project_amd/mtts/mamba.py
--- a/mamba-tts-project_amd/mtts/mamba.py
+++ b/mamba-tts-project_amd/mtts/mamba.py
@@ -88,12 +88,18 @@
         dW_x = None
         if not WG.submit([(gx, u2, W_x, None)], narrow=True):
             dW_x = G.mm_skinny_tn(u2, gx, trans_c=True) if G.skinny_tn_ok(u2, gx) else wgrad(gx, u2)
-        _, dw, db = ops.conv_bwd(x, conv_w, conv_b, du, True, dx=dxz[..., :di], state_in=conv_state_in)
+        defer = (conv_b is not None and ctx.needs_input_grad[1] and ctx.needs_input_grad[2]
+                 and WG.reduce_on(conv_w, conv_b))
+        _, dw, db = ops.conv_bwd(x, conv_w, conv_b, du, True, dx=dxz[..., :di], state_in=conv_state_in, defer=defer)
+        if isinstance(dw, WG.Pending):
+            WG.submit_reduce(dw, conv_w, param2=conv_b)
+            dw = db = None
         dstate = None
         if conv_state_in is not None and ctx.needs_input_grad[8]:
             dstate = _conv_state_grad(x, conv_w, conv_b, conv_state_in, du)
         dA_log = dA_log.to(A_log.dtype)
-        return (dxz, dw.reshape(conv_w.shape).to(conv_w.dtype), db.to(conv_b.dtype),
+        return (dxz, None if dw is None else dw.reshape(conv_w.shape).to(conv_w.dtype),
+                None if db is None else db.to(conv_b.dtype),
                 None if dW_x is None else dW_x.to(W_x.dtype), None if dW_dt is None else dW_dt.to(W_dt.dtype),
                 dA_log, dD.to(D.dtype), dbias.to(dt_bias.dtype), dstate,
                 None if dh0 is None else dh0.to(h0.dtype), None)
diff --git a/mamba-tts-project_amd/mtts/ops.py b/mamba-tts-project_amd/mtts/ops.py
--- a/mamba-tts-project_amd/mtts/ops.py
+++ b/mamba-tts-project_amd/mtts/ops.py
@@ -5,6 +5,7 @@
 import torch
 
 from . import _lib as L
+from . import wgrad as WG
 
 SCAN_CKPT = 16
 
@@ -185,7 +186,7 @@
     return out, st
 
 
-def conv_bwd(x, w, bias, dout, silu=True, dx=None, state_in=None):
+def conv_bwd(x, w, bias, dout, silu=True, dx=None, state_in=None, defer=False):
     Bsz, Ln, Dm = x.shape
     w = _f32c(w.reshape(Dm, -1))
     bias, state_in = _f32c(bias), _f32c(state_in)
@@ -193,15 +194,21 @@
     if dout.dtype != x.dtype:
         dout = dout.to(x.dtype)
     dx = torch.empty(Bsz, Ln, Dm, device=x.device, dtype=x.dtype) if dx is None else dx
-    dw = torch.empty(Dm, w.shape[1], device=x.device, dtype=torch.float32)
-    db = torch.empty(Dm, device=x.device, dtype=torch.float32)
+    defer = defer and Ln > 0
+    dw = None if defer else torch.empty(Dm, w.shape[1], device=x.device, dtype=torch.float32)
+    db = None if defer else torch.empty(Dm, device=x.device, dtype=torch.float32)
     ws = torch.empty(L.lib().mtts_causal_conv1d_bwd_workspace(Bsz, Dm, Ln, w.shape[1]), device=x.device,
                      dtype=torch.uint8)
     b = L.ConvBwdArgs()
     b.f = _conv_args(x, w, bias, silu, state_in, dout, None)
     b.dout, b.dout_bs, b.dout_ls = dout.data_ptr(), dout.stride(0), dout.stride(1)
     b.dx, b.dx_bs, b.dx_ls = dx.data_ptr(), dx.stride(0), dx.stride(1)
-    b.dw, b.dbias, b.workspace = dw.data_ptr(), db.data_ptr(), ws.data_ptr()
+    b.dw, b.dbias, b.workspace = L.ptr(dw), L.ptr(db), ws.data_ptr()
+    if defer:
+        job = L.ReduceJob()
+        b.defer_job = C.addressof(job)
+        L.call("mtts_causal_conv1d_bwd", b)
+        return dx, WG.Pending(ws, job, Dm * w.shape[1], Dm), None
     L.call("mtts_causal_conv1d_bwd", b)
     return dx, dw, db
 
@@ -344,15 +351,17 @@
 
 
 def layernorm_bwd(xn, w, b, eps, gamma, beta, rows_per_group, mean, rstd, dy, dx_acc=None, dgb=None,
-                  dx_colsum=None):
+                  dx_colsum=None, defer=None):
     dy = dy if dy.stride(-1) == 1 else dy.contiguous()
     if dy.dtype != xn.dtype:
         dy = dy.to(xn.dtype)
     w, b = _f32c(w), _f32c(b)
     rows, cols = mean.numel(), xn.shape[-1]
     dx = torch.empty(xn.shape, device=xn.device, dtype=xn.dtype)
-    dw = torch.empty(cols, device=xn.device, dtype=torch.float32)
-    db = torch.empty(cols, device=xn.device, dtype=torch.float32)
+    if defer is not None and rows == 0:
+        raise ValueError("layernorm_bwd: nothing to defer without rows")
+    dw = torch.empty(cols, device=xn.device, dtype=torch.float32) if defer is None else None
+    db = torch.empty(cols, device=xn.device, dtype=torch.float32) if defer is None else None
     film = gamma is not None
     G = rows // rows_per_group if film else 0
     if film and dgb is not None:
@@ -371,8 +380,15 @@
             dx_acc = dx_acc.to(xn.dtype)
         bb.dx_acc, bb.dxacc_rs = dx_acc.data_ptr(), _rows(dx_acc)[1]
     bb.dx, bb.dx_rs = dx.data_ptr(), _rows(dx)[1]
-    bb.dw, bb.db, bb.dgamma, bb.dbeta, bb.workspace = dw.data_ptr(), db.data_ptr(), L.ptr(dg), L.ptr(dbe), ws.data_ptr()
+    bb.dw, bb.db, bb.dgamma, bb.dbeta, bb.workspace = L.ptr(dw), L.ptr(db), L.ptr(dg), L.ptr(dbe), ws.data_ptr()
     bb.dgb_rs = dg.stride(0) if film else 0
+    if defer is not None:
+        jobs = (L.ReduceJob * 3)()
+        bb.defer_jobs = C.addressof(jobs)
+        bb.dx_colsum = ws.data_ptr() if dx_colsum else None
+        L.call("mtts_layernorm_bwd", bb)
+        defer.extend(WG.Pending(ws, jobs[i], cols) if jobs[i].nparts else None for i in range(3))
+        return dx, None, None, dg, dbe
     bb.dx_colsum = L.ptr(dx_colsum)
     L.call("mtts_layernorm_bwd", bb)
     return dx, dw, db, dg, dbe
@@ -393,6 +409,7 @@
         ctx.has_film = film is not None
         ctx.slot = colsum_slot
         ctx.dtypes = (w.dtype, b.dtype, None if gamma is None else gamma.dtype)
+        ctx.wb = (w, b)
         ctx.save_for_backward(xn, w, b, gamma, beta, mean, rstd)
         if res is None:
             x_sum = x.new_empty(0)
@@ -410,6 +427,21 @@
         dgb = None
         if ctx.has_film:
             dgb = torch.empty(gamma.shape[0], 2 * n, device=xn.device, dtype=torch.float32)
+        wd, bd, gd = ctx.dtypes
+        pw, pb = ctx.wb
+        if mean.numel() > 0 and ctx.needs_input_grad[2] and ctx.needs_input_grad[3] and WG.reduce_on(pw, pb):
+            pend = []
+            dx, _, _, dg, dbe = layernorm_bwd(xn, w, b, ctx.eps, gamma, beta, ctx.rpg, mean, rstd, dy, dx_acc=dsum,
+                                              dgb=dgb, dx_colsum=ctx.slot is not None, defer=pend)
+            WG.submit_reduce(pend[0], pw)
+            WG.submit_reduce(pend[1], pb)
+            if ctx.slot is not None:
+                ctx.slot.value = pend[2]
+            dres = dx if ctx.has_res else None
+            if ctx.has_film:
+                return (dx, dres, None, None, None, None, None, None, dgb.to(gd), None)
+            return (dx, dres, None, None, None if dg is None else dg.to(gd),
+                    None if dbe is None else dbe.to(gd), None, None, None, None)
         csum = None
         if ctx.slot is not None:
             csum = torch.empty(n, device=xn.device, dtype=torch.float32)
@@ -417,7 +449,6 @@
                                             dgb=dgb, dx_colsum=csum)
         if csum is not None:
             ctx.slot.value = csum
-        wd, bd, gd = ctx.dtypes
         dres = dx if ctx.has_res else None
         if ctx.has_film:
             return (dx, dres, dw.to(wd), db.to(bd), None, None, None, None, dgb.to(gd), None)
diff --git a/mamba-tts-project_amd/mtts/wgrad.py b/mamba-tts-project_amd/mtts/wgrad.py
--- a/mamba-tts-project_amd/mtts/wgrad.py
+++ b/mamba-tts-project_amd/mtts/wgrad.py
@@ -19,6 +19,8 @@
 _BK = 64
 MIN_GROUP_TILES = 128
 SIDE_STREAM = False
+DEFER_REDUCE = True
+REDUCE_HOLD_BYTES = 1 << 30
 
 _depth = 0
 
@@ -35,6 +37,44 @@
 
     def nbytes(self):
         return self.dy.numel() * self.dy.element_size() + self.x.numel() * self.x.element_size()
+
+
+class Pending:
+    __slots__ = ("keep", "job", "n", "n2")
+
+    def __init__(self, keep, job, n, n2=0):
+        self.keep, self.job, self.n, self.n2 = keep, job, n, n2
+
+    def numel(self):
+        return self.n
+
+    def materialize(self):
+        out = torch.empty(self.n, device=self.keep.device, dtype=torch.float32)
+        out2 = torch.empty(self.n2, device=self.keep.device, dtype=torch.float32) if self.n2 else None
+        _reduce_launch([_bind(self.job, out, out2, 0.0)])
+        return out if out2 is None else (out, out2)
+
+
+class _RJob:
+    __slots__ = ("pend", "param", "rows", "param2")
+
+    def __init__(self, pend, param, rows, param2):
+        self.pend, self.param, self.rows, self.param2 = pend, param, rows, param2
+
+
+def _bind(job, out, out2, beta):
+    j = L.ReduceJob()
+    C.memmove(C.byref(j), C.byref(job), C.sizeof(L.ReduceJob))
+    j.out, j.out2, j.beta = out.data_ptr(), (out2.data_ptr() if out2 is not None else None), beta
+    return j
+
+
+def _reduce_launch(bound):
+    arr = (L.ReduceJob * len(bound))(*bound)
+    lib = L.lib()
+    rc = lib.mtts_reduce_batch(arr, len(bound), C.c_void_p(torch.cuda.current_stream().cuda_stream))
+    if rc != 0:
+        raise RuntimeError(f"mtts_reduce_batch failed ({rc}): {lib.mtts_last_error().decode()}")
 
 
 def makespan(work, cus):
@@ -121,12 +161,16 @@
 class _Engine:
     def __init__(self):
         self.jobs = []
+        self.rjobs = []
+        self.rbytes = 0
         self.tiles = 0
         self.queue = RoundQueue()
         self.callback_queued = False
         self.done = set()
         self.covered = {}
         self.listeners = []
+        self.reduce_listeners = []
+        self.reduced = set()
         self.side = {}
         self.used_side = None
 
@@ -134,6 +178,7 @@
         self.callback_queued = False
         self.done = set()
         self.covered = {}
+        self.reduced = set()
         self.used_side = None
 
 
@@ -155,23 +200,28 @@
         yield
     finally:
         _depth -= 1
-        if _depth == 0 and (_E.jobs or _E.used_side is not None):
+        if _depth == 0 and (_E.jobs or _E.rjobs or _E.used_side is not None):
             _end_of_backward()
 
 
 def owns(p) -> bool:
     if id(p) in _E.done:
         return False
-    return id(p) in _E.covered or any(j.param is p for j in _E.jobs)
-
-
-def add_listener(fn):
+    return (id(p) in _E.covered or any(j.param is p for j in _E.jobs)
+            or any(j.param is p or j.param2 is p for j in _E.rjobs))
+
+
+def add_listener(fn, reductions=False):
     _E.listeners.append(fn)
+    if reductions:
+        _E.reduce_listeners.append(fn)
 
 
 def remove_listener(fn):
     if fn in _E.listeners:
         _E.listeners.remove(fn)
+    if fn in _E.reduce_listeners:
+        _E.reduce_listeners.remove(fn)
 
 
 def _eligible(dy, x, param, narrow=False):
@@ -192,7 +242,7 @@
 
 def _announce(p):
     _E.done.add(id(p))
-    for fn in _E.listeners:
+    for fn in (_E.reduce_listeners if id(p) in _E.reduced else _E.listeners):
         fn(p)
 
 
@@ -245,7 +295,102 @@
     return True
 
 
+def reduce_on(*params) -> bool:
+    return (active() and DEFER_REDUCE
+            and all(p is None or (p.requires_grad and p.is_leaf and p.dtype == torch.float32 and p.is_cuda)
+                    for p in params)
+            and any(p is not None for p in params))
+
+
+def _targets(param, rows, param2):
+    t = [(param, rows if rows is not None else (0, param.shape[0]))]
+    if param2 is not None:
+        t.append((param2, (0, param2.shape[0])))
+    return t
+
+
+def submit_reduce(pend, param, rows=None, param2=None):
+    for p in (param, param2):
+        if p is not None and id(p) in _E.done and _E.listeners:
+            raise RuntimeError("wgrad: a parameter's gradient sum was submitted after its gradient was announced "
+                               "complete to a listener; run this backward outside mtts.wgrad.deferred()")
+    mine = _targets(param, rows, param2)
+    if any(q is p and a < r1 and r0 < b
+           for j in _E.rjobs for q, (a, b) in _targets(j.param, j.rows, j.param2) for p, (r0, r1) in mine):
+        flush()
+    if not _E.callback_queued:
+        torch.autograd.Variable._execution_engine.queue_callback(_end_of_backward)
+        _E.callback_queued = True
+    _E.rjobs.append(_RJob(pend, param, rows, param2))
+    _E.reduced.update(id(p) for p, _ in mine)
+    _E.rbytes += pend.keep.numel() * pend.keep.element_size()
+    if _E.rbytes >= REDUCE_HOLD_BYTES:
+        _flush_reduce()
+
+
+def _flush_reduce():
+    rjobs, _E.rjobs, _E.rbytes = _E.rjobs, [], 0
+    if not rjobs:
+        return
+    pairs = [(j, p, (j.rows if p is j.param else None)) for j in rjobs for p in (j.param, j.param2) if p is not None]
+    covered = {}
+    for _, p, rows in pairs:
+        covered[id(p)] = covered.get(id(p), 0) + ((rows[1] - rows[0]) if rows else p.shape[0])
+    dest, fixups = {}, []
+    for j, p, _ in pairs:
+        if id(p) in dest:
+            continue
+        if p.grad is not None:
+            g = p.grad
+            if not g.is_contiguous() or g.dtype != torch.float32:
+                g = torch.zeros(p.shape, device=p.device, dtype=torch.float32)
+                fixups.append((p.grad, g))
+                dest[id(p)] = (g, 0.0, False)
+            else:
+                dest[id(p)] = (g, 1.0, False)
+            continue
+        view = getattr(p, "_mtts_grad_view", None)
+        full = covered[id(p)] >= p.shape[0]
+        if view is not None and view.is_contiguous():
+            if not full:
+                view.zero_()
+            g = view
+        else:
+            g = (torch.empty if full else torch.zeros)(p.shape, device=p.device, dtype=torch.float32)
+        dest[id(p)] = (g, 0.0, True)
+    bound = []
+    for j in rjobs:
+        g, beta, _ = dest[id(j.param)]
+        out = g.view(-1) if j.rows is None else g[j.rows[0]:j.rows[1]]
+        out2 = None
+        if j.param2 is not None:
+            g2, beta2, _ = dest[id(j.param2)]
+            if beta2 != beta:
+                for key in (id(j.param), id(j.param2)):
+                    gg, bb, fr = dest[key]
+                    if bb == 0.0:
+                        gg.zero_()
+                        dest[key] = (gg, 1.0, fr)
+                beta = 1.0
+            out2 = g2.view(-1)
+        bound.append(_bind(j.pend.job, out, out2, beta))
+    _reduce_launch(bound)
+    for old, g in fixups:
+        old.add_(g)
+    for _, p, _ in pairs:
+        g, _, fresh = dest[id(p)]
+        if fresh and p.grad is None:
+            p.grad = g
+    complete = {}
+    for _, p, rows in pairs:
+        if _cover(p, rows) and id(p) not in _E.done:
+            complete[id(p)] = p
+    for p in complete.values():
+        _announce(p)
+
+
 def flush():
+    _flush_reduce()
     jobs, _E.jobs, _E.tiles = _E.jobs, [], 0
     _E.queue.clear()
     if not jobs:
```

New measurement: 542,900 tokens/s. -1.7%, worse.
